# intel/QAT-ZSTD-Plugin

Measured on AMD Instinct MI355X. Metric: input MB/s via ZSTD_compress2 L1 128KiB blocks @1/2/4/8 GPU; ratio vs sw zstd, higher is better.
Workload: dtype u8

## Files before the change

### include/qzstd_hip.h

```cpp
#ifndef QZSTD_HIP_H
#define QZSTD_HIP_H

#include <stddef.h>
#include <stdint.h>

#if defined(__cplusplus)
extern "C" {
#endif

#define QZSTD_HIP_BLOCK_MAX (1u << 17)
#define QZSTD_HIP_NSEQ_ERROR 0xFFFFFFFFu
#define QZSTD_HIP_SRC_ALIGN 16u

typedef struct {
    uint32_t tableSize;
    uint32_t tileLog;
    uint32_t capLen;
    uint32_t minMatch;
    uint32_t farLog1;
    uint32_t farLog2;
    uint32_t lazy;
    uint32_t backExt;
    uint32_t nearTab;
    uint32_t window;
    uint32_t hashBytes;
    uint32_t extLog;
    uint32_t longSize;
    uint32_t repWin;
    uint32_t chainDepth;
    uint32_t subTileLog;
    uint32_t segLog;
} qzstd_hip_profile_t;

typedef struct {
    uint64_t srcOff;
    uint64_t seqOff;
    uint32_t srcLen;
    uint32_t seqCap;
    uint32_t parseFrom;
    uint32_t mark;
} qzstd_hip_block_t;

#define QZSTD_HIP_MARK_COMPACT 0x80000000u
#define QZSTD_HIP_PACK(off, lit, ml, tag) ((uint64_t)(off) | ((uint64_t)(lit) << 17) | ((uint64_t)(ml) << 35) | ((uint64_t)(tag) << 52))
#define QZSTD_HIP_PACKED_OFF(v) ((uint32_t)((v) & 0x1FFFFu))
#define QZSTD_HIP_PACKED_LIT(v) ((uint32_t)(((v) >> 17) & 0x3FFFFu))
#define QZSTD_HIP_PACKED_ML(v) ((uint32_t)(((v) >> 35) & 0x1FFFFu))
#define QZSTD_HIP_PACKED_TAG(v) ((uint32_t)((v) >> 52))

const char *qzstd_hip_last_error(void);

#define QZSTD_HIP_LEVEL_REPCODES 0x100

int qzstd_hip_profile_for_level(int level, size_t blockSize, qzstd_hip_profile_t *out);
size_t qzstd_hip_sequence_bound(size_t srcSize);
size_t qzstd_hip_lds_bytes(int level, uint32_t maxBlockLen);

#ifndef QZ_RING
#define QZ_RING 32768u
#endif
#define QZSTD_HIP_RING_MIRROR 128u
#ifndef QZ_CHAIN_TABLE
#define QZ_CHAIN_TABLE 5888u
#endif
#define QZSTD_HIP_LDS_BASE 16u
#define QZSTD_HIP_LDS_CTRL 64u
#define QZSTD_HIP_LDS_SVC 96u
#define QZSTD_HIP_LDS_MAX 163840u

int qzstd_hip_device_count(void);
int qzstd_hip_device_name(int device, char *buf, size_t bufLen);
void *qzstd_hip_malloc(int device, size_t bytes);
void qzstd_hip_free(int device, void *dptr);
void *qzstd_hip_host_alloc(size_t bytes);
void *qzstd_hip_host_device_ptr(void *hptr);
void qzstd_hip_host_free(void *hptr);
void *qzstd_hip_stream_create(int device);
void qzstd_hip_stream_destroy(int device, void *stream);
int qzstd_hip_stream_sync(int device, void *stream);
int qzstd_hip_stream_query(int device, void *stream);
int qzstd_hip_stream_wait(int device, void *stream, unsigned timeoutMs);
int qzstd_hip_memcpy_h2d(int device, void *stream, void *dst, const void *src, size_t bytes);
int qzstd_hip_copy_in(int device, void *stream, void *dst, const void *src_dev, size_t bytes);
int qzstd_hip_memcpy_d2h(int device, void *stream, void *dst, const void *src, size_t bytes);
int qzstd_hip_memset(int device, void *stream, void *dst, int value, size_t bytes);
int qzstd_hip_memcpy2d_d2h(int device, void *stream, void *dst, size_t dpitch, const void *src, size_t spitch,
                           size_t width, size_t height);

size_t qzstd_hip_workspace_bytes(int level, uint32_t nBlocks, uint32_t maxBlockLen);
int qzstd_hip_find_sequences(int device, void *stream, int level, const void *d_src,
                             const qzstd_hip_block_t *d_blocks, uint32_t nBlocks,
                             uint32_t maxBlockLen, void *d_seqs, uint32_t *d_nseq,
                             void *d_work, size_t workBytes);

int qzstd_hip_occupancy(int device, int level);

#define QZSTD_HIP_NSEQ_REJECTED 0xFFFFFFFEu
#define QZSTD_HIP_NSEQ_STAGING 0xFFFFFFFCu
int qzstd_hip_service_progressive(int device);
#define QZSTD_HIP_SVC_MAX_ITEMS 32u
#define QZSTD_HIP_SVC_MAX_SLOTS 1024u
typedef struct {
    const void *hSrc;
    void *dSrc;
    void *hSeqs;
    uint32_t *hCount;
    uint32_t srcLen, itemBytes, nItems, seqCapPerItem;
    uint32_t slot;
    uint32_t epoch;
    void *dWork;
} qzstd_hip_svc_req_t;
#ifndef QZSTD_HIP_CHAIN_ENTRY_LINKS
#define QZSTD_HIP_CHAIN_ENTRY_LINKS 4u
#endif
#define QZSTD_HIP_SVC_WORK_BYTES ((size_t)QZSTD_HIP_BLOCK_MAX * (8u * QZSTD_HIP_CHAIN_ENTRY_LINKS + 4u) + (size_t)QZSTD_HIP_SVC_MAX_ITEMS * QZ_CHAIN_TABLE * 4u)
int qzstd_hip_service_submit(int device, int level, const qzstd_hip_svc_req_t *req);
int qzstd_hip_service_stop(int device);
int qzstd_hip_service_poke(int device, int level);
void qzstd_hip_service_mark_broken(int device);
int qzstd_hip_service_info(int device, unsigned long out[8]);
int qzstd_hip_service_debug(int device, unsigned long out[8]);
void *qzstd_hip_host_alloc_coherent(size_t bytes);

int qzstd_hip_device_numa_node(int device);
void *qzstd_hip_host_alloc_on_node(size_t bytes, int node, int coherent);
int qzstd_hip_host_node_of(const void *hptr);

#if defined(__cplusplus)
}
#endif
#include "qzstd_hip_device.h"
#endif
```

### qat-zstd-plugin_amd/csrc/qzstd_hip_internal.h

```cpp
#ifndef QZSTD_HIP_INTERNAL_H
#define QZSTD_HIP_INTERNAL_H

#include <hip/hip_runtime.h>

#pragma GCC visibility push(hidden)

int fail(const char *what, hipError_t e);
int fail_msg(const char *what);

#define QZ_CHECK(call, what)                       \
    do {                                           \
        hipError_t e_ = (call);                    \
        if (e_ != hipSuccess) return fail(what, e_); \
    } while (0)

int phys(int device);
extern int g_devReplicas;

#define QZ_SET_DEVICE(device)                                            \
    do {                                                                 \
        const int pd_ = phys(device);                                    \
        if (pd_ < 0) return fail_msg("device index out of range");       \
        QZ_CHECK(hipSetDevice(pd_), "hipSetDevice");                     \
    } while (0)

int probe_lds_order(int device, int physDev);

struct SvcFreeze { SvcFreeze(); ~SvcFreeze(); };

#pragma GCC visibility pop

#endif
```

### qat-zstd-plugin_amd/csrc/qzstd_kernels.hip

```cpp
#include <hip/hip_runtime.h>

#include <stdint.h>
#include <stdio.h>
#include <stdlib.h>
#include <string.h>

#include <atomic>
#include <mutex>
#include <sched.h>
#include <time.h>

#include "qzstd_hip.h"
#include "qzstd_hip_internal.h"

#define QZ_PRIO(n) do { if (!CHAIN) __builtin_amdgcn_s_setprio(n); } while (0)

#ifndef QZ_PARSE_SPLIT
#define QZ_PARSE_SPLIT 3
#endif
#ifndef QZ_LINKS_PER_STEP
#define QZ_LINKS_PER_STEP 4
#endif
#ifndef QZ_WAVES_PER_EU
#define QZ_WAVES_PER_EU 5
#endif
#define QZ_OCCUPANCY __attribute__((amdgpu_waves_per_eu(QZ_WAVES_PER_EU)))

#ifdef QZ_DEBUG_DUMP
#define QZ_PLAP(acc) { const u64 tN = __builtin_amdgcn_s_memtime(); acc += tN - tQ; tQ = tN; }
#define QZ_LAP(acc) { const u64 tN = __builtin_amdgcn_s_memtime(); acc += tN - tP; tP = tN; }
#define QZ_CLAP(k) { const u64 tN = __builtin_amdgcn_s_memtime(); dC[k] += tN - tC; tC = tN; }
#else
#define QZ_PLAP(acc)
#define QZ_LAP(acc)
#define QZ_CLAP(k)
#endif

namespace {

constexpr int kMatchWaves = 8;
constexpr int kMatchThreads = kMatchWaves * 64;
constexpr int kThreads = kMatchThreads + 64;
constexpr uint32_t kTileLog = 9;
constexpr uint32_t kTile = 1u << kTileLog;
constexpr uint32_t kWin = kTile >> 6;
constexpr uint32_t kTagBits = 14;
constexpr uint32_t kTagMask = (1u << kTagBits) - 1u;
constexpr uint32_t kPrime1 = 2654435761u;
constexpr uint32_t kPrime2 = 0x85EBCA77u;
constexpr uint32_t kNone = 0xFFFFFFFFu;
constexpr uint32_t kRing = QZ_RING;
constexpr uint32_t kRingMask = kRing - 1u;
constexpr uint32_t kMirror = QZSTD_HIP_RING_MIRROR;
constexpr uint32_t kLook = 4608u;
constexpr uint32_t kNear = kRing - kLook - 3u * kTile - 1024u;
static_assert((kRing & kRingMask) == 0u && kRing >= 16384u, "the ring is a power of two of at least 16 KiB");
constexpr size_t kLdsPerCu = QZSTD_HIP_LDS_MAX;
constexpr uint32_t kEL = QZSTD_HIP_CHAIN_ENTRY_LINKS;
constexpr uint32_t kEQ = QZSTD_HIP_CHAIN_ENTRY_LINKS / 4u;
static_assert(kEL == 4u || kEL == 8u, "chain entries hold four or eight links");
constexpr uint32_t kLdsBase = QZSTD_HIP_LDS_BASE;
constexpr uint32_t kLagT = 2u;

struct LaunchArgs {
    const uint8_t *src;
    const qzstd_hip_block_t *blocks;
    uint4 *seqs;
    uint32_t *nseq;
    qzstd_hip_profile_t prof;
    uint4 *chain;
    uint32_t chainStride;
    uint32_t chainEntries;
    uint32_t pwWords;
    uint32_t orderedLds;
#ifdef QZ_DEBUG_DUMP
    uint32_t dbg;
#endif
};

typedef unsigned long long u64;

#ifdef QZ_DEBUG_DUMP
#define QZ_ABLATED(bit) (args.dbg & (bit))
#define QZ_DBG args.dbg
#else
#define QZ_ABLATED(bit) false
#define QZ_DBG 0u
#endif

#define QZ_BARRIER_LDS() asm volatile("s_waitcnt lgkmcnt(0)\n\ts_barrier" ::: "memory")

#define QZ_RLX_AGENT __ATOMIC_RELAXED, __HIP_MEMORY_SCOPE_AGENT
#define QZ_RLX_SYSTEM __ATOMIC_RELAXED, __HIP_MEMORY_SCOPE_SYSTEM

__device__ __forceinline__ uint32_t rdlane(uint32_t v, uint32_t l) { return (uint32_t)__builtin_amdgcn_readlane((int)v, (int)l); }
__device__ __forceinline__ uint32_t rdfirst(uint32_t v) { return (uint32_t)__builtin_amdgcn_readfirstlane((int)v); }
__device__ __forceinline__ u64 below(uint32_t c) { return c >= 64u ? ~0ull : ((1ull << c) - 1ull); }
__device__ __forceinline__ uint32_t umin(uint32_t a, uint32_t b) { return a < b ? a : b; }
__device__ __forceinline__ uint32_t umax(uint32_t a, uint32_t b) { return a > b ? a : b; }
__device__ __forceinline__ uint32_t umax3(uint32_t a, uint32_t b, uint32_t c) { return umax(umax(a, b), c); }

typedef const __attribute__((address_space(3))) uint32_t *LdsWords;
typedef const __attribute__((address_space(1))) uint32_t *HbmWords;
struct Src {
    LdsWords ring;
    HbmWords g;
    uint32_t nearLimit;
};

__device__ __forceinline__ uint32_t ring_dw(uint32_t a)
{
    return (a & kRingMask) >> 2;
}

__device__ __forceinline__ uint32_t ring_fwd(uint32_t r, uint32_t d) { return (r + d) & kRingMask; }
__device__ __forceinline__ uint32_t ring_back(uint32_t r, uint32_t d) { return (r - d) & kRingMask; }

template <int N>
__device__ __forceinline__ void load_dw_r(const Src &s, uint32_t a, uint32_t r, bool far, uint32_t (&D)[N])
{
    if (far) {
        const uint32_t d = a >> 2;
#pragma unroll
        for (int i = 0; i < N; i++) D[i] = s.g[d + i];
    } else {
        const uint32_t d = r >> 2;
#pragma unroll
        for (int i = 0; i < N; i++) D[i] = s.ring[d + i];
    }
}

template <int N>
__device__ __forceinline__ void load_dw(const Src &s, uint32_t a, bool far, uint32_t (&D)[N])
{
    if (far) {
        const uint32_t d = a >> 2;
#pragma unroll
        for (int i = 0; i < N; i++) D[i] = s.g[d + i];
    } else {
        const uint32_t d = ring_dw(a);
#pragma unroll
        for (int i = 0; i < N; i++) D[i] = s.ring[d + i];
    }
}

__device__ __forceinline__ uint32_t first_diff_bit(uint32_t x)
{
    uint32_t r;
    asm("v_ffbl_b32 %0, %1" : "=v"(r) : "v"(x));
    return r;
}

__device__ __forceinline__ uint32_t rd32u(const Src &s, uint32_t a, bool far)
{
    uint32_t D[2];
    load_dw<2>(s, a, far, D);
    return __builtin_amdgcn_alignbyte(D[1], D[0], a & 3u);
}

__device__ __forceinline__ uint32_t rd32_r(const Src &s, uint32_t a, uint32_t r, bool far)
{
    uint32_t D[2];
    load_dw_r<2>(s, a, r, far, D);
    return __builtin_amdgcn_alignbyte(D[1], D[0], a & 3u);
}

__device__ __forceinline__ uint32_t chunk_len(const Src &s, uint32_t p, uint32_t rp, uint32_t off, bool far)
{
    const uint32_t q = p - off, ps = p & 3u, qs = q & 3u;
    uint32_t P[9], Q[9];
    load_dw_r<9>(s, p, rp, false, P);
    load_dw_r<9>(s, q, ring_back(rp, off), far, Q);
    uint32_t B = 256u;
#pragma unroll
    for (int i = 0; i < 8; i++) {
        const uint32_t x = __builtin_amdgcn_alignbyte(P[i + 1], P[i], ps) ^ __builtin_amdgcn_alignbyte(Q[i + 1], Q[i], qs);
        B = umin(B, first_diff_bit(x) | (32u * (uint32_t)i));
    }
    return B >> 3;
}

__device__ __forceinline__ uint32_t head_len(const Src &s, const uint32_t (&oa)[4], uint32_t q, uint32_t rq, bool far)
{
    const uint32_t qs = q & 3u;
    uint32_t Q[5];
    load_dw_r<5>(s, q, rq, far, Q);
    uint32_t B = 128u;
#pragma unroll
    for (int i = 0; i < 4; i++) {
        const uint32_t x = oa[i] ^ __builtin_amdgcn_alignbyte(Q[i + 1], Q[i], qs);
        B = umin(B, first_diff_bit(x) | (32u * (uint32_t)i));
    }
    return B >> 3;
}

__device__ __forceinline__ uint32_t head_cmp(const uint32_t (&oa)[4], const uint32_t (&Q)[5], uint32_t qs)
{
    uint32_t B = 128u;
#pragma unroll
    for (int i = 0; i < 4; i++) {
        const uint32_t x = oa[i] ^ __builtin_amdgcn_alignbyte(Q[i + 1], Q[i], qs);
        B = umin(B, first_diff_bit(x) | (32u * (uint32_t)i));
    }
    return B >> 3;
}

__device__ __forceinline__ __attribute__((unused)) uint32_t tail_cmp(const uint32_t (&pa)[8], const uint32_t (&Q)[9], uint32_t qs)
{
    uint32_t B = 256u;
#pragma unroll
    for (int i = 0; i < 8; i++) {
        const uint32_t x = pa[i] ^ __builtin_amdgcn_alignbyte(Q[i + 1], Q[i], qs);
        B = umin(B, first_diff_bit(x) | (32u * (uint32_t)i));
    }
    return B >> 3;
}

__device__ __forceinline__ uint32_t tail_len(const Src &s, const uint32_t (&pa)[8], uint32_t q, uint32_t rq, bool far)
{
    const uint32_t qs = q & 3u;
    uint32_t Q[9];
    load_dw_r<9>(s, q, rq, far, Q);
    uint32_t B = 256u;
#pragma unroll
    for (int i = 0; i < 8; i++) {
        const uint32_t x = pa[i] ^ __builtin_amdgcn_alignbyte(Q[i + 1], Q[i], qs);
        B = umin(B, first_diff_bit(x) | (32u * (uint32_t)i));
    }
    return B >> 3;
}

__device__ __forceinline__ uint32_t seg_end(const qzstd_hip_profile_t &pf, uint32_t p, uint32_t n)
{
    return pf.segLog ? umin(n, ((p >> pf.segLog) + 1u) << pf.segLog) : n;
}

__device__ __forceinline__ uint32_t min_len(const qzstd_hip_profile_t &pf, uint32_t off)
{
    return pf.minMatch + ((off >> pf.farLog1) ? 1u : 0u) + ((off >> pf.farLog2) ? 1u : 0u);
}

template <bool AFAR = false>
__device__ __forceinline__ uint32_t extend_match_from(const Src &s, uint32_t p, uint32_t off, uint32_t L, uint32_t lim,
                                                      uint32_t lane, const bool far ,
                                                      const uint32_t lastDw = 0xFFFFFFFFu )
{
    for (;;) {
        const uint32_t a = p + L + 16u * lane;
        uint32_t ok = 0;
        if (a < lim) {
            const uint32_t b = a - off, as = a & 3u, bs = b & 3u;
            uint32_t A[5], B[5];
            if constexpr (AFAR) {
#pragma unroll
                for (int i = 0; i < 5; i++) { A[i] = s.g[umin((a >> 2) + (uint32_t)i, lastDw)]; B[i] = s.g[umin((b >> 2) + (uint32_t)i, lastDw)]; }
            } else {
                load_dw<5>(s, a, false, A);
                if (far) {
#pragma unroll
                    for (int i = 0; i < 5; i++) B[i] = s.g[umin((b >> 2) + (uint32_t)i, lastDw)];
                } else load_dw<5>(s, b, false, B);
            }
            ok = 16u;
#pragma unroll
            for (int i = 3; i >= 0; i--) {
                const uint32_t x = __builtin_amdgcn_alignbyte(A[i + 1], A[i], as) ^ __builtin_amdgcn_alignbyte(B[i + 1], B[i], bs);
                if (x) ok = 4u * (uint32_t)i + ((uint32_t)__builtin_ctz(x) >> 3);
            }
            ok = umin(ok, lim - a);
        }
        const u64 bad = __ballot(ok < 16u);
        if (bad) {
            const uint32_t f = (uint32_t)__builtin_ctzll(bad);
            return L + 16u * f + rdlane(ok, f);
        }
        L += 1024u;
    }
}

__device__ __forceinline__ uint32_t extend_match(const Src &s, uint32_t p, uint32_t off, uint32_t L, uint32_t lim, uint32_t lane)
{
    return extend_match_from(s, p, off, L, lim, lane, off > s.nearLimit);
}

struct ParseState {
    uint32_t cur;
    uint32_t anchor;
    uint32_t nseq;
};

constexpr uint32_t kSrecWords = 8;
constexpr uint32_t kPvStride = kTile + 8u;
constexpr uint32_t kNxCapped = 255u;

__device__ __forceinline__ uint32_t pack_pos(uint32_t nx, uint32_t ns, uint32_t payload)
{
    return nx | (ns << 8) | (payload << 15);
}

template <uint32_t L>
__device__ __forceinline__ uint32_t wrlane(uint32_t vec, uint32_t val)
{
    asm("v_writelane_b32 %0, %1, %2" : "+v"(vec) : "s"(val), "n"(L));
    return vec;
}

#define QZ_CHASE(c)                                                                   \
    asm volatile("v_readlane_b32 %[j], %[wd], %[cc]\n"                               \
                 "s_movk_i32 %[jn], 64\n"                                            \
                 "s_bfe_u32 %[j], %[j], 0x70008\n"                                   \
                 "s_cmp_gt_u32 %[j], 63\n"                                           \
                 "s_cbranch_scc1 2f\n"                                               \
                 "1:\n"                                                              \
                 "s_bitset1_b64 %[ch], %[j]\n"                                       \
                 "v_readlane_b32 %[jn], %[nx], %[j]\n"                               \
                 "s_cmp_lt_u32 %[jn], 64\n"                                          \
                 "s_cselect_b32 %[j], %[jn], %[j]\n"                                 \
                 "s_cbranch_scc1 1b\n"                                               \
                 "v_readlane_b32 %[pl], %[wd], %[j]\n"                               \
                 "s_lshr_b32 %[pl], %[pl], 15\n"                                     \
                 "2:\n"                                                              \
                 : [ch] "+s"(chosen), [j] "=&s"(j), [jn] "=&s"(jn), [pl] "=&s"(pl)    \
                 : [nx] "v"(nx), [wd] "v"(wordW), [cc] "s"(c)                         \
                 : "scc");

struct ParseRecs {
    uint32_t r0, r1, r2, r3, r4, r5;
};

template <uint32_t W>
__device__ __forceinline__ void parse_window(const qzstd_hip_profile_t &pf, const Src &src, const uint32_t wordW,
                                             uint32_t base, uint32_t n, uint32_t lane, ParseState &st, ParseRecs &r)
{
    constexpr uint32_t w = W;
    const uint32_t w0 = base + 64u * w;
    const uint32_t anchorIn = st.anchor, seqBase = st.nseq;
    u64 chosen = 0;
    uint32_t ext0 = 0, ext1 = 0;
    const uint32_t c0 = st.cur - w0;
    if (c0 < 64u) {
        const uint32_t nx = wordW & 0xFFu;
        uint32_t j, jn, pl;
        QZ_CHASE(c0)
        uint32_t cEnd = jn, eEnd = j < 64u ? j + pl : st.anchor - w0;
        if (__builtin_expect(jn == kNxCapped, 0)) {
            for (;;) {
                const uint32_t pj = w0 + j;
                const uint32_t lim = umin(seg_end(pf, pj, n), ((pj >> pf.extLog) + 2u) << pf.extLog);
                const uint32_t xl = extend_match(src, pj, pl, pf.capLen, lim, lane);
                if (!ext0) ext0 = (j << 24) | xl; else ext1 = (j << 24) | xl;
                cEnd = eEnd = j + xl;
                if (cEnd >= 64u) break;
                QZ_CHASE(cEnd)
                if (j >= 64u) { cEnd = 64u; break; }
                cEnd = jn; eEnd = j + pl;
                if (jn != kNxCapped) break;
            }
        }
        st.nseq += (uint32_t)__popcll(chosen);
        st.cur = w0 + cEnd;
        st.anchor = w0 + eEnd;
    }
    r.r0 = wrlane<W>(r.r0, (uint32_t)chosen);
    r.r1 = wrlane<W>(r.r1, (uint32_t)(chosen >> 32));
    r.r2 = wrlane<W>(r.r2, anchorIn);
    r.r3 = wrlane<W>(r.r3, seqBase);
    if (ext0) {
        r.r4 = wrlane<W>(r.r4, ext0);
        r.r5 = wrlane<W>(r.r5, ext1);
    }
}

template <uint32_t W, uint32_t W_END>
__device__ __forceinline__ void parse_windows(const qzstd_hip_profile_t &pf, const Src &src, const uint32_t (&word)[kWin],
                                              uint32_t base, uint32_t n, uint32_t lane, ParseState &st, ParseRecs &r)
{
    if constexpr (W < W_END) {
        parse_window<W>(pf, src, word[W], base, n, lane, st, r);
        parse_windows<W + 1u, W_END>(pf, src, word, base, n, lane, st, r);
    }
}

template <uint32_t W_BEGIN, uint32_t W_END>
__device__ __forceinline__ void parse_tile(const qzstd_hip_profile_t &pf, const Src &src, const uint32_t *pv,
                                           uint32_t *srecOut, uint32_t base, uint32_t n, uint32_t lane, ParseState &st)
{
    uint32_t word[kWin];
#pragma unroll
    for (uint32_t w = W_BEGIN; w < W_END; w++) word[w] = pv[64u * w + lane];
#pragma unroll
    for (uint32_t w = W_BEGIN; w < W_END; w++) asm volatile("" : "+v"(word[w]));
    ParseRecs r = { 0u, 0u, 0u, 0u, 0u, 0u };
    parse_windows<W_BEGIN, W_END>(pf, src, word, base, n, lane, st, r);
    if (lane >= W_BEGIN && lane < W_END) {
        *reinterpret_cast<uint4 *>(srecOut + lane * kSrecWords) = make_uint4(r.r0, r.r1, r.r2, r.r3);
        srecOut[lane * kSrecWords + 4u] = r.r4;
        srecOut[lane * kSrecWords + 5u] = r.r5;
    }
}

struct RepState {
    uint32_t cur, anchor, nseq;
    uint32_t rep1, rep2;
    uint32_t tileSeq;
    uint32_t seg;
};
constexpr uint32_t kRepCap = 32u, kRepMin = 3u;
constexpr uint32_t kLenCapped = 127u;
constexpr uint32_t kChosenBit = 0x80000000u;

__device__ __forceinline__ uint32_t ring_byte(const Src &s, uint32_t x, bool far)
{
    if (far) return reinterpret_cast<const __attribute__((address_space(1))) uint8_t *>(s.g)[x];
    return reinterpret_cast<const __attribute__((address_space(3))) uint8_t *>(s.ring)[x & kRingMask];
}

__device__ __forceinline__ u64 rep_bitmap(const Src &src, uint32_t cur, uint32_t rp, uint32_t n, uint32_t lane, uint32_t ringFrom = 0u)
{
    const uint32_t bpos = cur + lane;
    bool eq = false;
    if (rp != 0u && bpos < n) eq = ring_byte(src, bpos, false) == ring_byte(src, bpos - rp, rp > src.nearLimit || bpos - rp < ringFrom);
    return __ballot(eq);
}

__device__ __forceinline__ u64 rep_record(uint32_t q, uint32_t off, uint32_t L, uint32_t lit)
{
    return (u64)q | ((u64)off << 17) | ((u64)L << 34) | ((u64)lit << 47);
}

__device__ __forceinline__ uint32_t ring_off_s(uint32_t a)
{
    return a & kRingMask;
}

template <bool DEF>
__device__ __forceinline__ void parse_rep_span(const qzstd_hip_profile_t &pf, const Src &src, uint32_t *pvT,
                                               uint32_t base, uint32_t limit, uint32_t n, uint32_t nh, uint32_t lane,
                                               RepState &st, const uint32_t ringFrom = 0u, u64 *recG = nullptr)
{
    const uint32_t segEnd = seg_end(pf, base, n);
    const uint32_t startEnd = segEnd - pf.hashBytes + 1u;
    const uint32_t tileLim = umin(base + kTile, startEnd), stop = umin(limit, startEnd);
    if (st.cur < base) st.cur = base;
    if (st.cur >= stop) return;
    if (pf.segLog && (base >> pf.segLog) != st.seg) {
        st.rep1 = st.rep2 = 0u;
        st.seg = base >> pf.segLog;
    }
    uint32_t rc = rdfirst(ring_off_s(st.cur));
    const __attribute__((address_space(3))) uint8_t *rb = reinterpret_cast<const __attribute__((address_space(3))) uint8_t *>(src.ring);
    while (st.cur < stop) {
        const uint32_t rem = tileLim - st.cur;
        const uint32_t W = umin(pf.repWin, rem), V = umin(W + 2u, rem);
        const uint32_t curIn = st.cur;
        uint32_t wd = 0;
        if (lane < V) wd = pvT[st.cur + lane - base];
        u64 M1, M2;
        if (DEF ? (st.cur - st.rep1 >= ringFrom && st.cur - st.rep2 >= ringFrom)
                : (st.rep1 <= src.nearLimit && st.rep2 <= src.nearLimit)) {
            const uint32_t t1 = rc - st.rep1, t2 = rc - st.rep2;
            const uint32_t r1 = t1 & kRingMask, r2 = t2 & kRingMask;
            const uint32_t A = rb[rc + lane], B1 = rb[r1 + lane], B2 = rb[r2 + lane];
            const u64 in = below(segEnd - st.cur);
            M1 = st.rep1 ? __ballot(A == B1) & in : 0ull;
            M2 = st.rep2 ? __ballot(A == B2) & in : 0ull;
        } else {
            M1 = rep_bitmap(src, st.cur, st.rep1, segEnd, lane, ringFrom);
            M2 = rep_bitmap(src, st.cur, st.rep2, segEnd, lane, ringFrom);
        }
        const uint32_t x1 = __builtin_amdgcn_alignbit((uint32_t)(M1 >> 32), (uint32_t)M1, lane);
        const uint32_t x2 = __builtin_amdgcn_alignbit((uint32_t)(M2 >> 32), (uint32_t)M2, lane);
        const uint32_t rl1 = umin(first_diff_bit(~x1), kRepCap), rl2 = umin(first_diff_bit(~x2), kRepCap);
        const uint32_t rg1 = rl1 < kRepMin ? 0u : (rl1 >= kRepCap ? 1000u : 4u * rl1 + 36u);
        const uint32_t rg2 = rl2 < kRepMin ? 0u : (rl2 >= kRepCap ? 999u : 4u * rl2 + 35u);
        const uint32_t Gh = wd & 0x3FFu;
        const uint32_t G = lane < V ? umax3(Gh, rg1, rg2) : 0u;
        const uint32_t G1 = (uint32_t)__builtin_amdgcn_update_dpp(0, (int)G, 0x130, 0xF, 0xF, true);
        const uint32_t G2 = (uint32_t)__builtin_amdgcn_update_dpp(0, (int)G1, 0x130, 0xF, 0xF, true);
        const bool ok = lane < W && G != 0u && !(G1 > G + 4u) && !(G2 > G + 11u);
        const u64 m = __ballot(ok);
        if (!m) {
            st.cur += W;
            rc = ring_fwd(rc, W);
            continue;
        }
        const uint32_t ks = (uint32_t)__builtin_ctzll(m);
        const uint32_t gh = rdlane(Gh, ks), g1 = rdlane(rg1, ks), g2 = rdlane(rg2, ks);
        const uint32_t q = st.cur + ks;
        uint32_t off, L, from;
        if (g1 <= gh && g2 <= gh) {
            off = rdlane(wd, ks) >> 10;
            L = (gh - 32u + (31u - (uint32_t)__builtin_clz(off + 1u))) >> 2;
            from = pf.capLen;
        } else if (g2 > umax(gh, g1)) {
            off = st.rep2;
            L = rdlane(rl2, ks);
            from = kRepCap;
        } else {
            off = st.rep1;
            L = rdlane(rl1, ks);
            from = kRepCap;
        }
        if (L == from) L = extend_match_from(src, q, off, from, umin(segEnd, ((q >> pf.extLog) + 2u) << pf.extLog), lane,
                                             DEF ? q - off < ringFrom : off > src.nearLimit,
                                             DEF ? (((n + 15u) & ~15u) >> 2) - 1u : 0xFFFFFFFFu);
        if (DEF) {
            if (lane == 0u) recG[st.nseq] = rep_record(q, off, L, q - st.anchor);
        } else if (lane == 0u) {
            uint32_t *r = pvT + (q - base);
            r[0] = kChosenBit | off;
            r[1] = L | ((st.nseq - st.tileSeq) << 17);
            r[2] = st.anchor;
        }
        st.nseq++;
        if (off != st.rep1) {
            st.rep2 = st.rep1;
            st.rep1 = off;
        }
        st.cur = st.anchor = q + L;
        rc = rdfirst(ring_off_s(st.cur));
        (void)curIn;
    }
}

struct PlainParse {
    uint32_t cur, cnt, endA;
};
template <uint32_t W0, uint32_t W1>
__device__ __forceinline__ void parse_plain_windows(const qzstd_hip_profile_t &pf, const Src &src, u64 *recG, const uint32_t base, const uint32_t n,
                                                    const uint32_t lastDw, const uint32_t lane, const uint32_t (&wds)[kWin], PlainParse &st)
{
    u64 smA[kWin], chA[kWin];
    uint32_t lenA[kWin];
#pragma unroll
    for (uint32_t w = W0; w < W1; w++) {
        smA[w] = __ballot((wds[w] & kChosenBit) != 0u);
        lenA[w] = (wds[w] >> 17) & 127u;
    }
#pragma unroll
    for (uint32_t w = W0; w < W1; w++) {
        const uint32_t w0 = base + 64u * w;
        const u64 sm = smA[w];
        uint32_t c = rdfirst(st.cur - w0);
        u64 chosen = 0ull;
        uint32_t lenF = lenA[w];
        uint32_t e = 0u, j = 0u, L = 0u;
        auto chase = [&]() {
            u64 m;
            uint32_t t;
            asm volatile("s_cmp_lt_u32 %[c], 64\n"
                         "s_cbranch_scc0 3f\n"
                         "1:\n"
                         "s_lshr_b64 %[m], %[sm], %[c]\n"
                         "s_cbranch_scc0 2f\n"
                         "s_ff1_i32_b64 %[t], %[m]\n"
                         "s_add_u32 %[j], %[c], %[t]\n"
                         "s_bitset1_b64 %[ch], %[j]\n"
                         "v_readlane_b32 %[L], %[len], %[j]\n"
                         "s_add_u32 %[c], %[j], %[L]\n"
                         "s_cmp_lt_u32 %[c], 64\n"
                         "s_cbranch_scc1 1b\n"
                         "s_mov_b32 %[e], %[c]\n"
                         "s_branch 3f\n"
                         "2:\n"
                         "s_mov_b32 %[e], %[c]\n"
                         "s_movk_i32 %[c], 64\n"
                         "s_mov_b32 %[L], 0\n"
                         "3:\n"
                         : [m] "=&s"(m), [t] "=&s"(t), [j] "+s"(j), [ch] "+s"(chosen), [L] "+s"(L), [c] "+s"(c), [e] "+s"(e)
                         : [sm] "s"(sm), [len] "v"(lenF)
                         : "scc");
        };
        chase();
        while (__builtin_expect(L == kLenCapped, 0)) {
            const uint32_t pj = w0 + j, offj = rdlane(wds[w], j) & 0x1FFFFu;
            L = extend_match_from<true>(src, pj, offj, pf.capLen, umin(seg_end(pf, pj, n), ((pj >> pf.extLog) + 2u) << pf.extLog), lane, true, lastDw);
            if (lane == j) lenF = L;
            c = e = j + L;
            L = 0u;
            chase();
        }
        lenA[w] = lenF;
        st.cur = w0 + c;
        if (chosen) st.endA = w0 + e;
        chA[w] = chosen;
    }
#pragma unroll
    for (uint32_t w = W0; w < W1; w++) {
        const u64 chosen = chA[w];
        const uint32_t rank = __builtin_amdgcn_mbcnt_hi((uint32_t)(chosen >> 32), __builtin_amdgcn_mbcnt_lo((uint32_t)chosen, 0u));
        if ((chosen >> lane) & 1ull) recG[st.cnt + rank] = rep_record(base + 64u * w + lane, wds[w] & 0x1FFFFu, lenA[w], 0u);
        st.cnt += (uint32_t)__popcll(chosen);
    }
}

__device__ __forceinline__ void store_entry(uint4 *out, uint32_t idx, uint32_t off, uint32_t lit, uint32_t ml, uint32_t mark)
{
    if (mark & QZSTD_HIP_MARK_COMPACT)
        reinterpret_cast<u64 *>(out)[idx] = QZSTD_HIP_PACK(off, lit, ml, mark & 0xFFFu);
    else
        out[idx] = make_uint4(off, lit, ml, mark);
}

template <bool REP>
__device__ __forceinline__ void emit_window(const qzstd_hip_profile_t &pf, const Src &src, const uint32_t *srec,
                                            const uint32_t *pvW, uint32_t off, uint32_t len, uint32_t w0, uint32_t rpE,
                                            uint32_t lane, uint4 *out, uint32_t seqCap, uint32_t tileSeq, uint32_t mark)
{
    bool ch;
    uint32_t prevEnd, idx;
    if (REP) {
        const uint32_t r0 = pvW[lane];
        ch = (r0 & kChosenBit) != 0u;
        if (!__ballot(ch)) return;
        const uint32_t r1 = pvW[lane + 1u];
        prevEnd = pvW[lane + 2u];
        off = r0 & 0x1FFFFu;
        len = r1 & 0x1FFFFu;
        idx = tileSeq + (r1 >> 17);
    } else {
        const uint4 rec = *reinterpret_cast<const uint4 *>(srec);
        const u64 chosen = (u64)rec.x | ((u64)rec.y << 32);
        if (!chosen) return;
        const uint32_t anchorIn = rec.z, seqBase = rec.w;
        const uint32_t ext0 = rdfirst(srec[4]);
        if (ext0) {
            const uint32_t ext1 = srec[5];
            if ((ext0 >> 24) == lane) len = ext0 & 0xFFFFFFu;
            if (ext1 && (ext1 >> 24) == lane) len = ext1 & 0xFFFFFFu;
        }
        ch = (chosen >> lane) & 1ull;
        const u64 lower = chosen & below(lane);
        const uint32_t myEnd = w0 + lane + len;
        const int jprev = lower ? 63 - __builtin_clzll(lower) : 0;
        prevEnd = __shfl(myEnd, jprev);
        if (!lower) prevEnd = anchorIn;
        idx = seqBase + __builtin_amdgcn_mbcnt_hi((uint32_t)(chosen >> 32), __builtin_amdgcn_mbcnt_lo((uint32_t)chosen, 0u));
    }
    if (ch) {
        const uint32_t p = w0 + lane, q = p - off;
        const uint32_t lit = p - prevEnd;
        const uint32_t maxb = umin(umin(umin(pf.backExt, lit), q), pf.segLog ? (p & ((1u << pf.segLog) - 1u)) : p);
        uint32_t b = 0;
        if (maxb) {
            const bool far = off > src.nearLimit;
            const uint32_t rp4 = ring_back(rpE, 4u);
            const uint32_t pb = rd32_r(src, p - 4u, rp4, false);
            uint32_t qb;
            if (far) qb = q >= 4u ? rd32u(src, q - 4u, true) : rd32u(src, 0u, true) << (8u * (4u - q));
            else qb = rd32_r(src, q - 4u, ring_back(rp4, off), false);
            const uint32_t x = pb ^ qb;
            b = umin(x ? (uint32_t)__builtin_clz(x) >> 3 : 4u, maxb);
        }
        if (idx < seqCap) store_entry(out, idx, off, lit - b, len + b, mark);
    }
}

__device__ __forceinline__ uint32_t chain_insert_window(uint32_t *tbl, uint32_t st, uint32_t mine, uint32_t lane, bool ordered)
{
    const bool vk = st != kNone;
    const uint32_t slotK = st & 0xFFFFu;
    if (ordered) return vk ? atomicMax(&tbl[slotK], mine) : 0u;
    uint32_t prd = 0u, fin = mine;
    if (vk) {
        uint32_t *e = &tbl[slotK];
        prd = __hip_atomic_load(e, __ATOMIC_RELAXED, __HIP_MEMORY_SCOPE_WORKGROUP);
        atomicMax(e, mine);
        fin = __hip_atomic_load(e, __ATOMIC_RELAXED, __HIP_MEMORY_SCOPE_WORKGROUP);
    }
    u64 rem = __ballot(fin != mine);
    uint32_t predLane = lane;
    while (rem) {
        const uint32_t s0 = rdlane(slotK, (uint32_t)__builtin_ctzll(rem));
        const bool in = vk && slotK == s0;
        const u64 grp = __ballot(in);
        const u64 lower = grp & below(lane);
        if (in && lower) predLane = 63u - (uint32_t)__builtin_clzll(lower);
        rem &= ~grp;
    }
    const uint32_t fromLane = (uint32_t)__shfl((int)mine, (int)predLane);
    return vk ? (predLane != lane ? fromLane : prd) : 0u;
}

__device__ __forceinline__ void chain_insert_tile(const qzstd_hip_profile_t &pf, const Src &src, uint32_t *tbl, uint32_t *P1, uint32_t t0,
                                                  uint32_t n, uint32_t nh, uint32_t lane, bool ordered)
{
    const uint32_t segE = rdfirst(seg_end(pf, t0, n));
    uint32_t stv[kWin];
#pragma unroll
    for (uint32_t k = 0; k < kWin; k++) {
        const uint32_t p = t0 + 64u * k + lane;
        const uint32_t mixH = rd32u(src, p, false) * kPrime1;
        stv[k] = (p < nh && p + 4u <= segE) ? (__umulhi(mixH, pf.tableSize) | (((mixH >> 3) & kTagMask) << 16)) : kNone;
    }
    if (ordered) {
#pragma unroll
        for (uint32_t k = 0; k < kWin; k++) {
            const uint32_t mineK = ((t0 + 64u * k + lane + 1u) << kTagBits) | (stv[k] >> 16);
            uint32_t pred = 0u;
            if (stv[k] != kNone) pred = atomicMax(&tbl[stv[k] & 0xFFFFu], mineK);
            P1[64u * k + lane] = pred;
        }
    } else {
#pragma unroll 1
        for (uint32_t k = 0; k < kWin; k++) {
            const uint32_t st = stv[k];
            const bool vk = st != kNone;
            const uint32_t slotK = st & 0xFFFFu;
            const uint32_t mineK = ((t0 + 64u * k + lane + 1u) << kTagBits) | (st >> 16);
            uint32_t prd = 0u, fin = mineK;
            if (vk) {
                uint32_t *e = &tbl[slotK];
                prd = __hip_atomic_load(e, __ATOMIC_RELAXED, __HIP_MEMORY_SCOPE_WORKGROUP);
                atomicMax(e, mineK);
                fin = __hip_atomic_load(e, __ATOMIC_RELAXED, __HIP_MEMORY_SCOPE_WORKGROUP);
            }
            u64 rem = __ballot(fin != mineK);
            uint32_t predLane = lane;
            while (rem) {
                const uint32_t s0 = rdlane(slotK, (uint32_t)__builtin_ctzll(rem));
                const bool in = vk && slotK == s0;
                const u64 grp = __ballot(in);
                const u64 lower = grp & below(lane);
                if (in && lower) predLane = 63u - (uint32_t)__builtin_clzll(lower);
                rem &= ~grp;
            }
            const uint32_t fromLane = (uint32_t)__shfl((int)mineK, (int)predLane);
            P1[64u * k + lane] = vk ? (predLane != lane ? fromLane : prd) : 0u;
        }
    }
}

struct HistShare {
    uint32_t *flags;
    uint32_t item;
    uint32_t epoch;
    uint32_t spinLimit;
    uint32_t nItems;
    uint32_t *tabFlags;
    uint32_t *linkFlags;
    uint32_t *tabs;
};
constexpr uint32_t kSvcTabStride = QZ_CHAIN_TABLE;
static_assert((uint32_t)kMatchWaves * kPvStride <= QZ_CHAIN_TABLE, "the deferred parse's eight windows of parse words must fit in the head table (QZ_CHAIN_TABLE)");

template <bool HAS_LONG, bool REP, bool CHAIN, bool TURNS, bool NEAR, bool DEFER = false>
__device__ __forceinline__ uint32_t qz_item(const LaunchArgs &args, const qzstd_hip_block_t &blk, const uint8_t *gsrc, uint4 *out,
                                            uint4 *chainB, uint32_t *p1B, const HistShare hsh)
{
    extern __shared__ __attribute__((aligned(16))) uint8_t smem[];
    const uint32_t tid = threadIdx.x;
    const uint32_t lane = tid & 63u;
    const uint32_t wave = rdfirst(tid >> 6);
    const bool matcher = wave < (uint32_t)kMatchWaves;
    const uint32_t n = blk.srcLen;
    const qzstd_hip_profile_t pf = args.prof;
    const uint32_t nh = n >= pf.hashBytes ? n - pf.hashBytes + 1u : 0u;
    const uint32_t nTiles = (nh + kTile - 1u) >> kTileLog;
    const uint32_t itEnd = (DEFER && !CHAIN) ? nTiles : nTiles + kLagT;
    static_assert(kNear + kLagT * kTile + 4u <= kRing - kLook, "the ring no longer holds a near source when its tile is parsed / emitted");
    const uint32_t tabShift = (uint32_t)__builtin_clz(pf.tableSize) + 1u, longShift = pf.longSize ? (uint32_t)__builtin_clz(pf.longSize) + 1u : 31u;
    const uint32_t firstTile = blk.parseFrom >> kTileLog;
    if (blk.parseFrom != 0u && (pf.segLog == 0u || (blk.parseFrom & ((1u << pf.segLog) - 1u)) != 0u || blk.parseFrom >= n)) {
        return QZSTD_HIP_NSEQ_ERROR;
    }
    if (NEAR && n > kRing) return QZSTD_HIP_NSEQ_ERROR;
    if (DEFER && args.pwWords != 0u && ((n + kTile - 1u) & ~(kTile - 1u)) > args.pwWords) return QZSTD_HIP_NSEQ_ERROR;
    if (DEFER && CHAIN && args.chainEntries != 0u && ((n + kTile - 1u) & ~(kTile - 1u)) * kEQ > args.chainEntries) return QZSTD_HIP_NSEQ_ERROR;

    uint8_t *smemI = (uint8_t *)(__attribute__((address_space(3))) uint8_t *)kLdsBase;
    if ((uint32_t)(uintptr_t)(__attribute__((address_space(3))) uint8_t *)smem != 0u) {
        return QZSTD_HIP_NSEQ_ERROR;
    }
    uint32_t *ring32 = reinterpret_cast<uint32_t *>(smemI);
    uint4 *ring128 = reinterpret_cast<uint4 *>(smemI);
    uint32_t *tbl = reinterpret_cast<uint32_t *>(smemI + kRing + kMirror);
    uint32_t *tblL = tbl + pf.tableSize;
    uint32_t *nearTab = tblL + pf.longSize;
    uint32_t *srec = nearTab + kTile;
    uint32_t *pv = srec + kLagT * kWin * kSrecWords;
    uint32_t *turnCtr = pv + kLagT * kPvStride;
    uint32_t *P1odd = turnCtr + QZSTD_HIP_LDS_CTRL / 4u;
    const uint4 *g128 = reinterpret_cast<const uint4 *>(gsrc);
    Src src;
    src.ring = (LdsWords)ring32;
    src.g = (HbmWords)reinterpret_cast<const uint32_t *>(gsrc);
    src.nearLimit = NEAR ? 0xFFFFFFFFu : kNear;
    const uint32_t nPad = (n + 15u) & ~15u;

    const uint32_t itBegin = firstTile;
    const uint32_t histEnd = itBegin << kTileLog;
    const uint32_t hi = umin(nPad, histEnd + kLook + (itBegin ? 0u : kTile));
    const uint32_t lo = hi > kRing ? (hi - kRing + 15u) & ~15u : 0u;
    constexpr uint32_t kStep = (uint32_t)kThreads * 16u;
    const uint32_t hashEnd = CHAIN ? 0u : histEnd;
    uint32_t fo = (hashEnd ? 0u : lo) + tid * 16u;
    uint4 fa0 = make_uint4(0u, 0u, 0u, 0u), fb0 = fa0, fa1 = fa0, fb1 = fa0;
    if (fo < hi) { fa0 = g128[fo >> 4]; if (fo < hashEnd) fb0 = g128[(fo >> 4) + 1u]; }
    if (fo + kStep < hi) { fa1 = g128[(fo + kStep) >> 4]; if (fo + kStep < hashEnd) fb1 = g128[((fo + kStep) >> 4) + 1u]; }
    for (uint32_t i = tid; i < pf.tableSize + pf.longSize; i += kThreads) tbl[i] = 0u;
    if (!(CHAIN && itBegin != 0u)) {
        for (uint32_t i = tid; i < kTile; i += kThreads) nearTab[i] = 0xFFFFFFFFu;
        for (uint32_t i = tid; i < kLagT * kWin * kSrecWords + kLagT * kPvStride + QZSTD_HIP_LDS_CTRL / 4u; i += kThreads) srec[i] = 0u;
    }
    const bool sharedHist = CHAIN && hsh.flags != nullptr && hsh.nItems > 1u && pf.tableSize <= kSvcTabStride;
    if (itBegin != 0u || sharedHist) __syncthreads();
    if (sharedHist) {
        constexpr uint32_t kGroup = 4096u;
        uint32_t *hist = ring32;
        uint32_t *link = ring32 + kGroup;
        const uint32_t a0 = blk.parseFrom, b0 = n, k = hsh.item;
        auto wait_for = [&](uint32_t *fl) -> bool {
            if (wave == 0u) {
                uint32_t spins = 0u, ok = 1u;
                for (;;) {
                    const bool there = lane >= k || __hip_atomic_load(&fl[lane], QZ_RLX_AGENT) == hsh.epoch;
                    if (__all(there)) break;
                    if (++spins > hsh.spinLimit) { ok = 0u; break; }
                    __builtin_amdgcn_s_sleep(2);
                }
                __builtin_amdgcn_fence(__ATOMIC_ACQUIRE, "agent");
                if (lane == 0u) turnCtr[2] = ok;
            }
            __syncthreads();
            const bool ok = rdfirst(turnCtr[2]) != 0u;
            __syncthreads();
            return ok;
        };
        auto hash_group = [&](uint32_t g0) {
            if (tid < 256u) {
                const uint32_t c = g0 + tid * 16u;
                uint4 ha = make_uint4(0u, 0u, 0u, 0u), hb = ha;
                if (c < b0) { ha = g128[c >> 4]; hb = g128[(c >> 4) + 1u]; }
                const uint32_t W[5] = { ha.x, ha.y, ha.z, ha.w, hb.x };
                const uint32_t segEc = seg_end(pf, c, n);
                uint32_t st16[16];
#pragma unroll
                for (uint32_t j = 0; j < 16u; j++) {
                    const uint32_t v = (j & 3u) ? __builtin_amdgcn_alignbyte(W[(j >> 2) + 1u], W[j >> 2], j & 3u) : W[j >> 2];
                    const uint32_t mixH = v * kPrime1;
                    const bool okp = c + j < nh && c + j + 4u <= segEc;
                    st16[j] = okp ? (__umulhi(mixH, pf.tableSize) | (((mixH >> 3) & kTagMask) << 16)) : kNone;
                }
#pragma unroll
                for (uint32_t j = 0; j < 4u; j++)
                    reinterpret_cast<uint4 *>(hist)[tid * 4u + j] = make_uint4(st16[4u * j], st16[4u * j + 1u], st16[4u * j + 2u], st16[4u * j + 3u]);
            }
        };
        for (uint32_t g0 = a0; g0 < b0; g0 += kGroup) {
            hash_group(g0);
            QZ_BARRIER_LDS();
            if (wave == 2u || wave == 3u) {
                const uint32_t nW = (umin(kGroup, b0 - g0) + 63u) >> 6;
                const uint32_t par = wave & 1u;
                for (uint32_t w0 = 0; w0 < nW; w0 += 16u) {
                    uint32_t st[16], pred[16];
#pragma unroll
                    for (uint32_t j = 0; j < 16u; j++) st[j] = w0 + j < nW ? hist[64u * (w0 + j) + lane] : kNone;
#pragma unroll
                    for (uint32_t j = 0; j < 16u; j++) {
                        const uint32_t pos = g0 + 64u * (w0 + j) + lane;
                        const bool mine = st[j] != kNone && (st[j] & 1u) == par;
                        pred[j] = 0u;
                        if (mine) pred[j] = args.orderedLds != 0u ? atomicMax(&tbl[st[j] & 0xFFFFu], ((pos + 1u) << kTagBits) | (st[j] >> 16))
                                                                   : chain_insert_window(tbl, st[j], ((pos + 1u) << kTagBits) | (st[j] >> 16), lane, false);
                        else if (args.orderedLds == 0u) (void)chain_insert_window(tbl, kNone, 0u, lane, false);
                    }
#pragma unroll
                    for (uint32_t j = 0; j < 16u; j++)
                        if (w0 + j < nW && (st[j] == kNone || (st[j] & 1u) == par)) link[64u * (w0 + j) + lane] = pred[j];
                }
            }
            QZ_BARRIER_LDS();
            if (tid < 512u) {
#pragma unroll
                for (uint32_t j = 0; j < 2u; j++)
                    if (g0 + (j * 512u + tid) * 4u < b0) reinterpret_cast<uint4 *>(p1B + g0)[j * 512u + tid] = reinterpret_cast<const uint4 *>(link)[j * 512u + tid];
            }
            QZ_BARRIER_LDS();
        }
        {
            uint32_t *mine = hsh.tabs + (size_t)k * kSvcTabStride;
            for (uint32_t i = tid; i < pf.tableSize; i += kThreads) __hip_atomic_store(&mine[i], tbl[i], QZ_RLX_AGENT);
            asm volatile("s_waitcnt vmcnt(0)" ::: "memory");
            __syncthreads();
            if (tid == 0u) __hip_atomic_store(&hsh.tabFlags[k], hsh.epoch, QZ_RLX_AGENT);
        }
        if (!wait_for(hsh.tabFlags)) return QZSTD_HIP_NSEQ_ERROR;
        for (uint32_t i = tid; i < pf.tableSize; i += kThreads) {
            uint32_t m = 0u;
            for (uint32_t j = 0; j < k; j++) m = umax(m, hsh.tabs[(size_t)j * kSvcTabStride + i]);
            tbl[i] = m;
        }
        __syncthreads();
        for (uint32_t g0 = a0; g0 < b0; g0 += kGroup) {
            hash_group(g0);
            QZ_BARRIER_LDS();
            if (tid < 512u) {
#pragma unroll
                for (uint32_t j = 0; j < 8u; j++) {
                    const uint32_t i = j * 512u + tid, pos = g0 + i;
                    if (pos < b0) {
                        uint32_t l1 = p1B[pos];
                        const uint32_t st = hist[i];
                        if (l1 == 0u && st != kNone) l1 = tbl[st & 0xFFFFu];
                        __hip_atomic_store(&p1B[pos], l1, QZ_RLX_AGENT);
                    }
                }
            }
            QZ_BARRIER_LDS();
        }
        asm volatile("s_waitcnt vmcnt(0)" ::: "memory");
        __syncthreads();
        if (tid == 0u) __hip_atomic_store(&hsh.linkFlags[k], hsh.epoch, QZ_RLX_AGENT);
        if (!wait_for(hsh.linkFlags)) return QZSTD_HIP_NSEQ_ERROR;
        constexpr uint32_t kCh = 16u / kEL;
        for (uint32_t p0 = a0 + tid; p0 < b0; p0 += kCh * (uint32_t)kThreads) {
            uint32_t e[kEL][kCh];
#pragma unroll
            for (uint32_t i = 0; i < kCh; i++) { const uint32_t pp = p0 + i * (uint32_t)kThreads; e[0][i] = pp < b0 ? __hip_atomic_load(&p1B[pp], QZ_RLX_AGENT) : 0u; }
#pragma unroll
            for (uint32_t d = 1; d < kEL; d++)
#pragma unroll
                for (uint32_t i = 0; i < kCh; i++) e[d][i] = e[d - 1u][i] ? __hip_atomic_load(&p1B[(e[d - 1u][i] >> kTagBits) - 1u], QZ_RLX_AGENT) : 0u;
#pragma unroll
            for (uint32_t i = 0; i < kCh; i++) {
                const uint32_t pp = p0 + i * (uint32_t)kThreads;
                if (pp < b0) {
                    u64 *w = reinterpret_cast<u64 *>(chainB + (size_t)pp * kEQ);
#pragma unroll
                    for (uint32_t d = 0; d < kEL; d += 2u) __hip_atomic_store(w + d / 2u, (u64)e[d][i] | ((u64)e[d + 1u][i] << 32), QZ_RLX_AGENT);
                }
            }
        }
        asm volatile("s_waitcnt vmcnt(0)" ::: "memory");
        __syncthreads();
        if (tid == 0u) __hip_atomic_store(&hsh.flags[k], hsh.epoch, QZ_RLX_AGENT);
        if (!wait_for(hsh.flags)) return QZSTD_HIP_NSEQ_ERROR;
        for (uint32_t i = tid; i < kTile; i += kThreads) nearTab[i] = 0xFFFFFFFFu;
        for (uint32_t i = tid; i < kLagT * kWin * kSrecWords + kLagT * kPvStride + QZSTD_HIP_LDS_CTRL / 4u; i += kThreads) srec[i] = 0u;
    } else if (CHAIN && itBegin != 0u) {
        constexpr uint32_t kGroup = 4096u;
        static_assert(kGroup * 8u <= kRing, "two words per position of a group in the ring's LDS");
        uint32_t *hist = ring32;
        uint32_t *link = ring32 + kGroup;
        const uint32_t nGroups = (histEnd + kGroup - 1u) / kGroup;
        uint4 ha = make_uint4(0u, 0u, 0u, 0u), hb = ha;
        if (tid < 256u && tid * 16u < histEnd) { ha = g128[tid]; hb = g128[tid + 1u]; }
        for (uint32_t g = 0; g < nGroups && !QZ_ABLATED(2048u); g++) {
            const uint32_t g0 = g * kGroup;
            if (tid < 256u) {
                const uint32_t c = g0 + tid * 16u;
                const uint32_t W[5] = { ha.x, ha.y, ha.z, ha.w, hb.x };
                const uint32_t segEc = seg_end(pf, c, n);
                uint32_t st16[16];
#pragma unroll
                for (uint32_t k = 0; k < 16u; k++) {
                    const uint32_t v = (k & 3u) ? __builtin_amdgcn_alignbyte(W[(k >> 2) + 1u], W[k >> 2], k & 3u) : W[k >> 2];
                    const uint32_t mixH = v * kPrime1;
                    const bool ok = c + k < histEnd && c + k + 4u <= segEc;
                    st16[k] = ok ? (__umulhi(mixH, pf.tableSize) | (((mixH >> 3) & kTagMask) << 16)) : kNone;
                }
#pragma unroll
                for (uint32_t k = 0; k < 4u; k++)
                    reinterpret_cast<uint4 *>(hist)[tid * 4u + k] = make_uint4(st16[4u * k], st16[4u * k + 1u], st16[4u * k + 2u], st16[4u * k + 3u]);
                const uint32_t cn = c + kGroup;
                ha = hb = make_uint4(0u, 0u, 0u, 0u);
                if (cn < histEnd) { ha = g128[cn >> 4]; hb = g128[(cn >> 4) + 1u]; }
            }
            QZ_BARRIER_LDS();
            if (wave == 2u || wave == 3u) {
                const uint32_t nW = umin(kGroup, histEnd - g0) >> 6;
                const uint32_t par = wave & 1u;
                if (args.orderedLds != 0u) {
                    for (uint32_t w0 = 0; w0 < nW; w0 += 16u) {
                        uint32_t st[16], pred[16];
#pragma unroll
                        for (uint32_t k = 0; k < 16u; k++) st[k] = hist[64u * (w0 + k) + lane];
#pragma unroll
                        for (uint32_t k = 0; k < 16u; k++) {
                            const uint32_t pos = g0 + 64u * (w0 + k) + lane;
                            pred[k] = 0u;
                            if (st[k] != kNone && (st[k] & 1u) == par) pred[k] = atomicMax(&tbl[st[k] & 0xFFFFu], ((pos + 1u) << kTagBits) | (st[k] >> 16));
                        }
#pragma unroll
                        for (uint32_t k = 0; k < 16u; k++)
                            if (st[k] == kNone || (st[k] & 1u) == par) link[64u * (w0 + k) + lane] = pred[k];
                    }
                } else {
                    for (uint32_t w = 0; w < nW; w++) {
                        const uint32_t st = hist[64u * w + lane];
                        const uint32_t pos = g0 + 64u * w + lane;
                        const bool mine = st != kNone && (st & 1u) == par;
                        const uint32_t pred = chain_insert_window(tbl, mine ? st : kNone, ((pos + 1u) << kTagBits) | (st >> 16), lane, false);
                        if (mine || st == kNone) link[64u * w + lane] = pred;
                    }
                }
            }
            QZ_BARRIER_LDS();
            if (tid < 512u && !QZ_ABLATED(1024u)) {
#pragma unroll
                for (uint32_t k = 0; k < 2u; k++)
                    if (g0 + (k * 512u + tid) * 4u < histEnd) reinterpret_cast<uint4 *>(p1B + g0)[k * 512u + tid] = reinterpret_cast<const uint4 *>(link)[k * 512u + tid];
            }
            QZ_BARRIER_LDS();
        }
        constexpr uint32_t kChase = 32u / kEL;
        const uint32_t chaseFrom = hsh.flags ? histEnd - histEnd / hsh.item : 0u;
        for (uint32_t p0 = chaseFrom + tid; p0 < histEnd && !QZ_ABLATED(512u); p0 += kChase * (uint32_t)kThreads) {
            uint32_t e[kEL][kChase];
#pragma unroll
            for (uint32_t i = 0; i < kChase; i++) { const uint32_t pp = p0 + i * (uint32_t)kThreads; e[0][i] = pp < histEnd ? p1B[pp] : 0u; }
#pragma unroll
            for (uint32_t d = 1; d < kEL; d++)
#pragma unroll
                for (uint32_t i = 0; i < kChase; i++) e[d][i] = e[d - 1u][i] ? p1B[(e[d - 1u][i] >> kTagBits) - 1u] : 0u;
#pragma unroll
            for (uint32_t i = 0; i < kChase; i++) {
                const uint32_t pp = p0 + i * (uint32_t)kThreads;
                if (pp < histEnd) {
                    if (hsh.flags) {
                        u64 *w = reinterpret_cast<u64 *>(chainB + (size_t)pp * kEQ);
#pragma unroll
                        for (uint32_t d = 0; d < kEL; d += 2u) __hip_atomic_store(w + d / 2u, (u64)e[d][i] | ((u64)e[d + 1u][i] << 32), QZ_RLX_AGENT);
                    } else {
#pragma unroll
                        for (uint32_t j = 0; j < kEL / 4u; j++) chainB[(size_t)pp * kEQ + j] = make_uint4(e[4u * j][i], e[4u * j + 1u][i], e[4u * j + 2u][i], e[4u * j + 3u][i]);
                    }
                }
            }
        }
        if (hsh.flags) {
            asm volatile("s_waitcnt vmcnt(0)" ::: "memory");
            __syncthreads();
            if (wave == 0u) {
                if (lane == 0u) __hip_atomic_store(&hsh.flags[hsh.item], hsh.epoch, QZ_RLX_AGENT);
                uint32_t spins = 0u, ok = 1u;
                for (;;) {
                    const bool there = lane == 0u || lane >= hsh.item || __hip_atomic_load(&hsh.flags[lane], QZ_RLX_AGENT) == hsh.epoch;
                    if (__all(there)) break;
                    if (++spins > hsh.spinLimit) { ok = 0u; break; }
                    __builtin_amdgcn_s_sleep(2);
                }
                __builtin_amdgcn_fence(__ATOMIC_ACQUIRE, "agent");
                if (lane == 0u) turnCtr[2] = ok;
            }
            __syncthreads();
            if (rdfirst(turnCtr[2]) == 0u) return QZSTD_HIP_NSEQ_ERROR;
        }
        __syncthreads();
        for (uint32_t i = tid; i < kTile; i += kThreads) nearTab[i] = 0xFFFFFFFFu;
        for (uint32_t i = tid; i < kLagT * kWin * kSrecWords + kLagT * kPvStride + QZSTD_HIP_LDS_CTRL / 4u; i += kThreads) srec[i] = 0u;
    }
    {
        const uint32_t hiMaskH = pf.hashBytes >= 8 ? 0xFFFFFFFFu : ((1u << (8u * (pf.hashBytes - 4u))) - 1u);
        for (; fo < hi; fo += kStep) {
            uint4 fa2 = make_uint4(0u, 0u, 0u, 0u), fb2 = fa2;
            const uint32_t o2 = fo + 2u * kStep;
            if (o2 < hi) { fa2 = g128[o2 >> 4]; if (o2 < hashEnd) fb2 = g128[(o2 >> 4) + 1u]; }
            if (fo >= lo) {
                const uint32_t r = ring_dw(fo) << 2;
                ring128[r >> 4] = fa0;
                if (r < kMirror) ring128[(kRing + r) >> 4] = fa0;
            }
            if (fo < hashEnd) {
                const uint32_t W[6] = { fa0.x, fa0.y, fa0.z, fa0.w, fb0.x, fb0.y };
                const uint32_t segEc = seg_end(pf, fo, n);
#pragma unroll
                for (uint32_t k = 0; k < 16u; k++) {
                    const uint32_t p = fo + k;
                    if (p + pf.hashBytes <= segEc) {
                        const uint32_t v = __builtin_amdgcn_alignbyte(W[(k >> 2) + 1u], W[k >> 2], k & 3u);
                        const uint32_t w = __builtin_amdgcn_alignbyte(W[(k >> 2) + 2u], W[(k >> 2) + 1u], k & 3u);
                        const uint32_t mixH = (v * kPrime1) ^ __umul24(pf.hashBytes > 4 ? w & hiMaskH : 0u, kPrime2 & 0xFFFFFFu);
                        atomicMax(&tbl[mixH >> tabShift], ((p + 1u) << kTagBits) | ((mixH >> 3) & kTagMask));
                        if (HAS_LONG && p + 8u <= segEc) {
                            const uint32_t m8 = (v * kPrime1) ^ (w * kPrime2);
                            atomicMax(&tblL[m8 >> longShift], ((p + 1u) << kTagBits) | ((m8 >> 3) & kTagMask));
                        }
                    }
                }
            }
            fa0 = fa1; fb0 = fb1; fa1 = fa2; fb1 = fb2;
        }
        if (itBegin != 0u && TURNS && !CHAIN && tid == 0u) *turnCtr = itBegin * (uint32_t)kMatchWaves;
        if (itBegin == 0u)
            for (uint32_t o = hi + tid * 16u; o < kTile + kLook; o += kThreads * 16u) {
                ring128[o >> 4] = make_uint4(0u, 0u, 0u, 0u);
                if (o < kMirror) ring128[(kRing + o) >> 4] = make_uint4(0u, 0u, 0u, 0u);
            }
    }
    __syncthreads();

    if (DEFER && !matcher) __builtin_amdgcn_endpgm();
    if (!matcher) {
        if (!QZ_ABLATED(32u)) __builtin_amdgcn_s_setprio(3);
        constexpr uint32_t kSplit = QZ_PARSE_SPLIT;
#ifdef QZ_DEBUG_DUMP
        u64 pI1 = 0, pW1 = 0, pI2 = 0, pW2 = 0, tQ = __builtin_amdgcn_s_memtime();
#endif
        uint32_t nseqEnd, anchorEnd;
        if (REP) {
            RepState st = { blk.parseFrom, blk.parseFrom, 0u, 0u, 0u, 0u, pf.segLog ? blk.parseFrom >> pf.segLog : 0u };
            for (uint32_t it = itBegin; it < itEnd; it++) {
                const bool work = it >= 1u && it - 1u < nTiles && it - 1u >= firstTile && !QZ_ABLATED(1u);
                const uint32_t k = it - 1u, base = k << kTileLog;
                uint32_t *pvT = pv + (k % kLagT) * kPvStride, *srecT = srec + (k % kLagT) * kWin * kSrecWords;
                if (work) {
                    st.tileSeq = st.nseq;
                    if (lane == 0u) srecT[0] = st.nseq;
                    if (!CHAIN) parse_rep_span<false>(pf, src, pvT, base, base + 64u * kSplit, n, nh, lane, st);
                }
                if (CHAIN && it == itBegin && it < nTiles) chain_insert_tile(pf, src, tbl, (it & 1u) ? P1odd : nearTab, it << kTileLog, n, nh, lane, args.orderedLds != 0u);
                QZ_PLAP(pI1)
                __syncthreads();
                QZ_PLAP(pW1)
                if (work) parse_rep_span<false>(pf, src, pvT, base, base + kTile, n, nh, lane, st);
                if (CHAIN && it + 1u < nTiles) chain_insert_tile(pf, src, tbl, ((it + 1u) & 1u) ? P1odd : nearTab, (it + 1u) << kTileLog, n, nh, lane, args.orderedLds != 0u);
                QZ_PLAP(pI2)
                __syncthreads();
                QZ_PLAP(pW2)
            }
            nseqEnd = st.nseq;
            anchorEnd = st.anchor;
        } else {
            ParseState st = { blk.parseFrom, blk.parseFrom, 0u };
            for (uint32_t it = itBegin; it < itEnd; it++) {
                const bool work = it >= 1u && it - 1u < nTiles && it - 1u >= firstTile && !QZ_ABLATED(1u);
                const uint32_t k = it - 1u;
                if (work && !CHAIN)
                    parse_tile<0, kSplit>(pf, src, pv + (k % kLagT) * kPvStride, srec + (k % kLagT) * kWin * kSrecWords,
                                          k << kTileLog, n, lane, st);
                if (CHAIN && it == itBegin && it < nTiles) chain_insert_tile(pf, src, tbl, (it & 1u) ? P1odd : nearTab, it << kTileLog, n, nh, lane, args.orderedLds != 0u);
                QZ_PLAP(pI1)
                __syncthreads();
                QZ_PLAP(pW1)
                if (work) {
                    if (CHAIN)
                        parse_tile<0, kWin>(pf, src, pv + (k % kLagT) * kPvStride, srec + (k % kLagT) * kWin * kSrecWords, k << kTileLog, n, lane, st);
                    else
                        parse_tile<kSplit, kWin>(pf, src, pv + (k % kLagT) * kPvStride, srec + (k % kLagT) * kWin * kSrecWords,
                                                 k << kTileLog, n, lane, st);
                }
                if (CHAIN && it + 1u < nTiles) chain_insert_tile(pf, src, tbl, ((it + 1u) & 1u) ? P1odd : nearTab, (it + 1u) << kTileLog, n, nh, lane, args.orderedLds != 0u);
                QZ_PLAP(pI2)
                __syncthreads();
                QZ_PLAP(pW2)
            }
            nseqEnd = st.nseq;
            anchorEnd = st.anchor;
        }
#ifdef QZ_DEBUG_DUMP
        if (lane == 0 && !(blk.mark & QZSTD_HIP_MARK_COMPACT)) out[blk.seqCap - 2u] = make_uint4((uint32_t)pI1, (uint32_t)pW1, (uint32_t)pI2, (uint32_t)pW2);
        if (lane == 0 && !(blk.mark & QZSTD_HIP_MARK_COMPACT)) out[blk.seqCap - 12u - wave] = make_uint4(__builtin_amdgcn_s_getreg((4 << 0) | (0 << 6) | (31 << 11)), 0u, 0u, 0u);
#endif
        uint32_t count = nseqEnd + 1u;
        if (lane == 0 && nseqEnd < blk.seqCap) store_entry(out, nseqEnd, 0u, n - anchorEnd, 0u, blk.mark);
        if (count + 1u >= blk.seqCap) count = QZSTD_HIP_NSEQ_ERROR;
        return count;
    }

    if (matcher) {
    uint4 *const ownB = (CHAIN && hsh.flags) ? chainB + (size_t)QZSTD_HIP_BLOCK_MAX * kEQ : chainB;
    const uint32_t ownFrom = blk.parseFrom;
    auto entryOf = [&](uint32_t q, uint32_t (&D)[kEL]) {
        const uint4 *b = (q >= ownFrom ? ownB : chainB) + (size_t)q * kEQ;
#pragma unroll
        for (uint32_t j = 0; j < kEL / 4u; j++) { const uint4 v = b[j]; D[4u * j] = v.x; D[4u * j + 1u] = v.y; D[4u * j + 2u] = v.z; D[4u * j + 3u] = v.w; }
    };
    const uint32_t hiMask = pf.hashBytes >= 8 ? 0xFFFFFFFFu : ((1u << (8u * (pf.hashBytes - 4u))) - 1u);
    const uint32_t nearShift = 32u - kTileLog;
    const uint32_t stampShift = kTileLog + kTagBits;
    const uint32_t nTilesMax = QZSTD_HIP_BLOCK_MAX >> kTileLog;

    uint32_t offH[kLagT], lenH[kLagT];
#pragma unroll
    for (uint32_t i = 0; i < kLagT; i++) offH[i] = lenH[i] = 0u;
    uint32_t rp = ring_dw((itBegin << kTileLog) + tid) << 2 | (tid & 3u);
#ifdef QZ_DEBUG_DUMP
    u64 dI1 = 0, dW1 = 0, dI2 = 0, dW2 = 0, tP = __builtin_amdgcn_s_memtime();
    u64 dC[6] = { 0, 0, 0, 0, 0, 0 }, tC = 0;
#endif

    auto write_flags = [&](uint32_t tileIdx, uint32_t cl, uint32_t off) {
            const bool take = cl != 0u && cl >= min_len(pf, off);
            bool defer1, defer2, defer3 = false;
            if (pf.lazy >= 4u) {
                const uint32_t G = take ? 4u * cl + 32u - (31u - (uint32_t)__builtin_clz(off + 1u)) : 0u;
                const uint32_t G1 = (uint32_t)__builtin_amdgcn_update_dpp(0, (int)G, 0x130, 0xF, 0xF, true);
                const uint32_t G2 = (uint32_t)__builtin_amdgcn_update_dpp(0, (int)G1, 0x130, 0xF, 0xF, true);
                defer1 = lane < 63u && G1 > G + 4u;
                defer2 = lane < 62u && G2 > G + 7u;
            } else {
                const uint32_t tl = take ? cl : 0u;
                const uint32_t tl1 = (uint32_t)__builtin_amdgcn_update_dpp(0, (int)tl, 0x130, 0xF, 0xF, true);
                const uint32_t tl2 = (uint32_t)__builtin_amdgcn_update_dpp(0, (int)tl1, 0x130, 0xF, 0xF, true);
                const uint32_t tl3 = (uint32_t)__builtin_amdgcn_update_dpp(0, (int)tl2, 0x130, 0xF, 0xF, true);
                defer1 = pf.lazy >= 1u && lane < 63u && tl1 > cl;
                defer2 = pf.lazy >= 2u && lane < 62u && tl2 > cl;
                defer3 = pf.lazy >= 3u && lane < 61u && tl3 > cl + 2u;
            }
            const bool start = take && !defer1 && !defer2 && !defer3;
            if constexpr (DEFER && !REP) {
                p1B[(tileIdx << kTileLog) + tid] = off | ((cl == pf.capLen ? kLenCapped : cl) << 17) | (start ? kChosenBit : 0u);
                return;
            }
            const u64 startMask = __ballot(start);
            const uint32_t smLo = (uint32_t)startMask, smHi = (uint32_t)(startMask >> 32);
            const uint32_t keepLo = lane < 32u ? smLo & (0xFFFFFFFFu << (lane & 31u)) : 0u;
            const uint32_t keepHi = lane < 32u ? smHi : smHi & (0xFFFFFFFFu << (lane & 31u));
            const uint32_t ns = umin(umin(first_diff_bit(keepLo), first_diff_bit(keepHi) | 32u), 64u);
            const bool capped = cl == pf.capLen;
            const uint32_t endj = lane + cl;
            const uint32_t nsEnd = (uint32_t)__shfl((int)ns, (int)(endj & 63u));
            uint32_t nx = endj >= 64u ? endj : nsEnd;
            nx = capped ? kNxCapped : nx;
            const uint32_t gRep = take ? 4u * cl + 32u - (31u - (uint32_t)__builtin_clz(off + 1u)) : 0u;
            if (DEFER) p1B[(tileIdx << kTileLog) + tid] = gRep | (off << 10);
            else pv[(tileIdx % kLagT) * kPvStride + tid] = REP ? (gRep | (off << 10)) : pack_pos(nx, ns, capped ? off : cl);
    };
    for (uint32_t it = itBegin; it < itEnd; it++) {
        const uint32_t t0 = it << kTileLog;
        const uint32_t p = t0 + tid;
        const uint32_t stamp = (nTilesMax - 1u - (it & (nTilesMax - 1u))) << stampShift;
        uint32_t mix = 0, old = 0;
        const uint32_t segE = rdfirst(seg_end(pf, t0, n));
        const bool valid = it < nTiles && p < nh && p + pf.hashBytes <= segE;
        const bool history = it < firstTile;

        QZ_PRIO(2);
        if (CHAIN && DEFER && wave == 0u && it == itBegin && it < nTiles)
            chain_insert_tile(pf, src, tbl, (it & 1u) ? P1odd : nearTab, it << kTileLog, n, nh, lane, args.orderedLds != 0u);
        uint32_t own[5];
        load_dw_r<5>(src, p, rp, false, own);
        uint4 fresh;
        asm volatile("" : "=v"(fresh.x), "=v"(fresh.y), "=v"(fresh.z), "=v"(fresh.w));
        const uint32_t fpos = t0 + kLook + (tid - 64u) * 16u;
        const bool refill = wave == 1u && it >= 1u && lane < kTile / 16u && fpos < nPad;
        if (refill) fresh = g128[fpos >> 4];
        if (!DEFER && it >= kLagT + firstTile && !QZ_ABLATED(8u))
            emit_window<REP>(pf, src, srec + ((it % kLagT) * kWin + wave) * kSrecWords, pv + (it % kLagT) * kPvStride + 64u * wave,
                             offH[kLagT - 1u], lenH[kLagT - 1u], t0 - kLagT * kTile + 64u * wave, ring_back(rp, kLagT * kTile), lane, out, blk.seqCap,
                             REP ? srec[(it % kLagT) * kWin * kSrecWords] : 0u, blk.mark);
        QZ_PRIO(1);
        uint32_t slot = 0, nslot = 0, slotL = 0, oldL = 0, tagL = 0;
        const bool validL = HAS_LONG && valid && p + 8u <= segE;
        uint32_t oa[4];
#pragma unroll
        for (int i = 0; i < 4; i++) oa[i] = __builtin_amdgcn_alignbyte(own[i + 1], own[i], p & 3u);
        if (valid) {
            const uint32_t v = oa[0];
            uint32_t hi = 0;
            if (pf.hashBytes > 4) hi = oa[1] & hiMask;
            mix = (v * kPrime1) ^ __umul24(hi, kPrime2 & 0xFFFFFFu);
            slot = CHAIN ? __umulhi(mix, pf.tableSize) : mix >> tabShift;
            nslot = mix >> nearShift;
            if (!TURNS) old = tbl[slot];
            if (pf.nearTab && !history) atomicMin(&nearTab[nslot], stamp | (tid << kTagBits) | ((mix >> 3) & kTagMask));
            if (validL) {
                const uint32_t m8 = (v * kPrime1) ^ (oa[1] * kPrime2);
                slotL = m8 >> longShift;
                tagL = (m8 >> 3) & kTagMask;
                if (!TURNS) oldL = tblL[slotL];
            }
        }
        uint32_t pre[kEL];
#pragma unroll
        for (uint32_t j = 0; j < kEL; j++) pre[j] = 0u;
        if (CHAIN && it != itBegin) {
            old = valid ? ((it & 1u) ? P1odd : nearTab)[tid] : 0u;
            if (old != 0u && (old >> kTagBits) - 1u < t0) entryOf((old >> kTagBits) - 1u, pre);
        }
        if (CHAIN && it > itBegin && it - 1u < nTiles && it - 1u >= firstTile && !QZ_ABLATED(4u)) write_flags(it - 1u, lenH[0], offH[0]);
        QZ_LAP(dI1)
        __syncthreads();
        QZ_LAP(dW1)

        QZ_PRIO(2);
        if (CHAIN && DEFER && wave == 0u && it + 1u < nTiles)
            chain_insert_tile(pf, src, tbl, ((it + 1u) & 1u) ? P1odd : nearTab, (it + 1u) << kTileLog, n, nh, lane, args.orderedLds != 0u);
        if (refill) {
            const uint32_t o = ring_dw(fpos) << 2;
            ring128[o >> 4] = fresh;
            if (o < kMirror) ring128[(kRing + o) >> 4] = fresh;
        }
        uint32_t cl = 0, off = 0;
        if (CHAIN) {
            const uint32_t *P1T = (it & 1u) ? P1odd : nearTab;
            const uint32_t tag = (mix >> 3) & kTagMask;
#ifdef QZ_DEBUG_DUMP
            tC = __builtin_amdgcn_s_memtime();
#endif
            uint32_t E[kEL];
#pragma unroll
            for (uint32_t j = 0; j < kEL; j++) E[j] = 0u;
            if (valid) {
                E[0] = P1T[tid];
                if (E[0] != 0u && (E[0] >> kTagBits) - 1u < t0) {
                    if (it == itBegin) entryOf((E[0] >> kTagBits) - 1u, pre);
#pragma unroll
                    for (uint32_t i = 1; i < kEL; i++) E[i] = pre[i - 1u];
                } else {
#pragma unroll
                    for (uint32_t i = 1; i < kEL; i++) {
                        const uint32_t q = (E[i - 1u] >> kTagBits) - 1u;
                        if (E[i - 1u] == 0u || q < t0) break;
                        E[i] = P1T[q - t0];
                    }
                }
#pragma unroll
                for (uint32_t j = 0; j < kEL / 4u; j++) ownB[(size_t)p * kEQ + j] = make_uint4(E[4u * j], E[4u * j + 1u], E[4u * j + 2u], E[4u * j + 3u]);
            }
            const uint32_t cap = valid ? umin(umin(pf.capLen, 48u), segE - p) : 0u;
            uint32_t walked = 0;
            if (history) E[0] = 0u;
            int bg = 0;
            QZ_CLAP(0)
            while (__ballot(E[0] != 0u)) {
                uint32_t N[kEL];
#pragma unroll
                for (uint32_t j = 0; j < kEL; j++) N[j] = 0u;
                if (E[0] != 0u) {
                    uint32_t last = E[0], cnt = 1u;
#pragma unroll
                    for (uint32_t j = 1; j < kEL; j++) { if (E[j] != 0u) { last = E[j]; cnt = j + 1u; } }
                    const uint32_t ql = (last >> kTagBits) - 1u;
                    if (walked + cnt < pf.chainDepth) {
                        if (ql < t0) {
                            entryOf(ql, N);
                        } else {
                            N[0] = P1T[ql - t0];
#pragma unroll
                            for (uint32_t i = 1; i < kEL; i++) {
                                const uint32_t q = (N[i - 1u] >> kTagBits) - 1u;
                                if (N[i - 1u] == 0u || q < t0) break;
                                N[i] = P1T[q - t0];
                            }
                        }
                    }
                    constexpr int kG = QZ_LINKS_PER_STEP;
                    QZ_CLAP(1)
#pragma unroll
                    for (int kk = 0; kk < (int)kEL; kk += kG) {
                        uint32_t q[kG], rq[kG];
                        bool far[kG], m[kG];
#pragma unroll
                        for (int g = 0; g < kG; g++) {
                            const uint32_t l = E[kk + g];
                            q[g] = (l >> kTagBits) - 1u;
                            far[g] = p - q[g] > src.nearLimit;
                            m[g] = l != 0u && walked + (uint32_t)(kk + g) < pf.chainDepth && (l & kTagMask) == tag && (pf.window == 0u || p - q[g] <= pf.window) &&
                                   !QZ_ABLATED(2u) && !(QZ_ABLATED(64u) && far[g]);
                            rq[g] = ring_back(rp, p - q[g]);
                        }
                        bool any = false;
#pragma unroll
                        for (int g = 0; g < kG; g++) any = any || m[g];
                        if (any && cl != 0u) {
                            uint32_t v[kG];
#pragma unroll
                            for (int g = 0; g < kG; g++) {
                                m[g] = m[g] && cl < cap;
                                v[g] = 0u;
                                if (m[g]) v[g] = rd32_r(src, q[g] + cl - 3u, ring_fwd(rq[g], cl - 3u), far[g]);
                            }
                            const uint32_t pw = rd32_r(src, p + cl - 3u, ring_fwd(rp, cl - 3u), false);
#pragma unroll
                            for (int g = 0; g < kG; g++) m[g] = m[g] && v[g] == pw;
                        }
                        QZ_CLAP(2)
                        uint32_t Q[kG][5];
#pragma unroll
                        for (int g = 0; g < kG; g++) {
#pragma unroll
                            for (int i = 0; i < 5; i++) Q[g][i] = 0u;
                            if (m[g]) load_dw_r<5>(src, q[g], rq[g], far[g], Q[g]);
                        }
#pragma unroll
                        for (int g = 0; g < kG; g++) {
                            if (m[g] && cl < cap) {
                                uint32_t l = head_cmp(oa, Q[g], q[g] & 3u);
                                if (l == 16u && cap > 16u) l += chunk_len(src, p + 16u, ring_fwd(rp, 16u), p - q[g], far[g]);
                                l = umin(l, cap);
                                const int gn = (int)(4u * l) - (int)(31u - (uint32_t)__builtin_clz(p - q[g] + 1u));
                                if (l >= 4u && (cl == 0u || gn > bg)) { cl = l; off = p - q[g]; bg = gn; }
                            }
                        }
                    }
                    walked += cnt;
                }
                QZ_CLAP(3)
#ifdef QZ_DEBUG_DUMP
                asm volatile("s_waitcnt vmcnt(0)" ::: "memory");
                dC[5] += 1;
#endif
                const bool full = cl != 0u && cl >= cap;
#pragma unroll
                for (uint32_t j = 0; j < kEL; j++) E[j] = full ? 0u : N[j];
                QZ_CLAP(4)
            }
        } else {
        if (TURNS) {
            const uint32_t turn = it * (uint32_t)kMatchWaves + wave;
            uint32_t spins = 0;
            while (__hip_atomic_load(turnCtr, __ATOMIC_ACQUIRE, __HIP_MEMORY_SCOPE_WORKGROUP) != turn && ++spins < (1u << 22))
                __builtin_amdgcn_s_sleep(1);
            if (valid) {
                old = tbl[slot];
                if (validL) oldL = tblL[slotL];
                atomicMax(&tbl[slot], ((p + 1u) << kTagBits) | ((mix >> 3) & kTagMask));
                if (validL) atomicMax(&tblL[slotL], ((p + 1u) << kTagBits) | tagL);
            }
            if (lane == 0u) __hip_atomic_store(turnCtr, turn + 1u, __ATOMIC_RELEASE, __HIP_MEMORY_SCOPE_WORKGROUP);
        }
        if (valid) {
            const uint32_t tag = (mix >> 3) & kTagMask;
            const uint32_t en = pf.nearTab ? nearTab[nslot] : 0xFFFFFFFFu;
            if (!TURNS) {
                atomicMax(&tbl[slot], ((p + 1u) << kTagBits) | tag);
                if (validL) atomicMax(&tblL[slotL], ((p + 1u) << kTagBits) | tagL);
            }
            if (!history) {
            const uint32_t cap = umin(pf.capLen, segE - p);
            uint32_t q1 = kNone, q2 = kNone;
            if (old != 0u && (old & kTagMask) == tag) {
                const uint32_t q = (old >> kTagBits) - 1u;
                if (pf.window == 0u || p - q <= pf.window) q1 = q;
            }
            if (QZ_ABLATED(2u)) q1 = kNone;
            if (QZ_ABLATED(64u) && q1 != kNone && p - q1 > src.nearLimit) q1 = kNone;
            uint32_t l1 = 0, l2 = 0, l3 = 0;
            const bool far1 = q1 != kNone && p - q1 > src.nearLimit;
            if (q1 != kNone) l1 = head_len(src, oa, q1, ring_back(rp, p - q1), far1);
            uint32_t q3 = kNone;
            if (HAS_LONG && validL && oldL != 0u && (oldL & kTagMask) == tagL && !QZ_ABLATED(2u)) q3 = (oldL >> kTagBits) - 1u;
            const bool far3 = q3 != kNone && p - q3 > src.nearLimit;
            if (q3 != kNone) l3 = head_len(src, oa, q3, ring_back(rp, p - q3), far3);
            if (pf.nearTab && (en >> stampShift) == (stamp >> stampShift) && (en & kTagMask) == tag) {
                const uint32_t q = t0 + ((en >> kTagBits) & (kTile - 1u));
                if (q < p && !QZ_ABLATED(2u | 256u)) q2 = q;
            }
            if (q2 != kNone) l2 = head_len(src, oa, q2, ring_back(rp, p - q2), false);
            bool need1 = l1 == 16u && cap > 16u, need2 = l2 == 16u && cap > 16u, need3 = HAS_LONG && l3 == 16u && cap > 16u;
            if (QZ_ABLATED(128u)) need1 = need2 = need3 = false;
            QZ_PRIO(1);
            if (need1 || need2 || need3) {
                const uint32_t rp16 = ring_fwd(rp, 16u);
                uint32_t P[9], pa[8];
                load_dw_r<9>(src, p + 16u, rp16, false, P);
#pragma unroll
                for (int i = 0; i < 8; i++) pa[i] = __builtin_amdgcn_alignbyte(P[i + 1], P[i], p & 3u);
                if (need1) { const uint32_t l = tail_len(src, pa, q1 + 16u, ring_back(rp16, p - q1), far1); l1 = 16u + l; need1 = l == 32u && 48u < cap; }
                if (HAS_LONG && need3) { const uint32_t l = tail_len(src, pa, q3 + 16u, ring_back(rp16, p - q3), far3); l3 = 16u + l; need3 = l == 32u && 48u < cap; }
                if (need2) { const uint32_t l = tail_len(src, pa, q2 + 16u, ring_back(rp16, p - q2), false); l2 = 16u + l; need2 = l == 32u && 48u < cap; }
            }
            while (need1 || need2 || need3) {
                const int which = need1 ? 1 : (need3 ? 3 : 2);
                const uint32_t q = which == 1 ? q1 : (which == 3 ? q3 : q2);
                const uint32_t L = which == 1 ? l1 : (which == 3 ? l3 : l2);
                const uint32_t l = chunk_len(src, p + L, ring_fwd(rp, L), p - q, which == 1 ? far1 : (which == 3 ? far3 : false));
                const bool more = l == 32u && L + 32u < cap;
                if (which == 1) { l1 = L + l; need1 = more; }
                else if (which == 3) { l3 = L + l; need3 = more; }
                else { l2 = L + l; need2 = more; }
            }
            QZ_PRIO(0);
            l1 = umin(l1, cap); l2 = umin(l2, cap); l3 = umin(l3, cap);
            if (l1 >= 4u) { cl = l1; off = p - q1; }
            if (l3 >= 4u && l3 > cl) { cl = l3; off = p - q3; }
            if (l2 >= 4u && l2 >= cl) { cl = l2; off = p - q2; }
            }
        }
        }
        if (!CHAIN && it < nTiles && !history && !QZ_ABLATED(4u)) write_flags(it, cl, off);
#pragma unroll
        for (uint32_t i = kLagT - 1u; i > 0u; i--) { offH[i] = offH[i - 1u]; lenH[i] = lenH[i - 1u]; }
        offH[0] = off;
        lenH[0] = cl;
        rp = ring_fwd(rp, kTile);
        QZ_LAP(dI2)
        if (DEFER && !CHAIN) QZ_BARRIER_LDS(); else __syncthreads();
        QZ_LAP(dW2)
    }
#ifdef QZ_DEBUG_DUMP
    if (!(blk.mark & QZSTD_HIP_MARK_COMPACT)) {
    if (lane == 0) out[blk.seqCap - 3u - wave] = make_uint4((uint32_t)dI1, (uint32_t)dW1, (uint32_t)dI2, (uint32_t)dW2);
    if (lane == 0) out[blk.seqCap - 24u - 2u * wave] = make_uint4((uint32_t)(dC[0] >> 4), (uint32_t)(dC[1] >> 4), (uint32_t)(dC[2] >> 4), (uint32_t)(dC[3] >> 4));
    if (lane == 0) out[blk.seqCap - 25u - 2u * wave] = make_uint4((uint32_t)(dC[4] >> 4), (uint32_t)dC[5], 0u, 0u);
    if (lane == 0) out[blk.seqCap - 12u - wave] = make_uint4(__builtin_amdgcn_s_getreg((4 << 0) | (0 << 6) | (31 << 11)), 0u, 0u, 0u);
    }
#endif
    if constexpr (!DEFER) return 0u;
    }

    if constexpr (DEFER && !REP) {
        constexpr uint32_t kSegLog = 12u, kSeg = 1u << kSegLog, kMaxSegs = QZSTD_HIP_BLOCK_MAX >> kSegLog;
        static_assert(kMaxSegs <= 64u, "one lane per segment in the prefix step");
        constexpr uint32_t kNoAnchor = 0xFFFFFFFFu;
        uint32_t *segCnt = srec, *segEndA = srec + kMaxSegs;
        const uint32_t firstSeg = blk.parseFrom >> kSegLog, nSegs = (nh + kSeg - 1u) >> kSegLog;
#ifdef QZ_DEBUG_DUMP
        const u64 tD0 = __builtin_amdgcn_s_memtime();
#endif
        if (wave == 0u && lane == 0u) segCnt[2u * kMaxSegs] = firstSeg;
        __syncthreads();
#ifdef QZ_DEBUG_DUMP
        const u64 tD1 = __builtin_amdgcn_s_memtime();
#endif
        {
            const uint32_t S0 = rdfirst(segCnt[2u * kMaxSegs]);
            const uint32_t lastDw = (nPad >> 2) - 1u;
            auto load_tile = [&](uint32_t tb, uint32_t (&dst)[kWin]) {
#pragma unroll
                for (uint32_t j = 0; j < kWin; j++) dst[j] = p1B[tb + 64u * j + lane];
            };
            uint32_t nxt[kWin];
            uint32_t sgN = S0 + wave;
            if (sgN < nSegs) load_tile(sgN << kSegLog, nxt);
            while (sgN < nSegs) {
                const uint32_t sg = sgN;
                sgN = sg + (uint32_t)kMatchWaves;
                const uint32_t segStart = sg << kSegLog;
                u64 *recG = reinterpret_cast<u64 *>(p1B + segStart);
                const uint32_t tEnd = umin(segStart + kSeg, nTiles << kTileLog);
                PlainParse st = { segStart, 0u, kNoAnchor };
                for (uint32_t base = segStart; base < tEnd; base += kTile) {
                    uint32_t wds[kWin];
#pragma unroll
                    for (uint32_t j = 0; j < kWin; j++) wds[j] = nxt[j];
                    const uint32_t nb = base + kTile < tEnd ? base + kTile : sgN << kSegLog;
                    if (base + kTile < tEnd || sgN < nSegs) load_tile(nb, nxt);
                    parse_plain_windows<0, kWin>(pf, src, recG, base, n, lastDw, lane, wds, st);
                }
                if (lane == 0u) { segCnt[sg] = st.cnt; segEndA[sg] = st.endA; }
            }
        }
#ifdef QZ_DEBUG_DUMP
        const u64 tD2 = __builtin_amdgcn_s_memtime();
#endif
        __syncthreads();
#ifdef QZ_DEBUG_DUMP
        const u64 tD3 = __builtin_amdgcn_s_memtime();
#endif
        const bool mine = lane >= firstSeg && lane < nSegs;
        const uint32_t cv = mine ? segCnt[lane] : 0u, ev = mine ? segEndA[lane] : kNoAnchor;
        uint32_t incl = cv, last = ev;
#pragma unroll
        for (uint32_t d = 1; d < kMaxSegs; d <<= 1) {
            const uint32_t ci = (uint32_t)__shfl_up((int)incl, d), li = (uint32_t)__shfl_up((int)last, d);
            if (lane >= d) { incl += ci; if (last == kNoAnchor) last = li; }
        }
        const uint32_t total = rdlane(incl, kMaxSegs - 1u), lastAll = rdlane(last, kMaxSegs - 1u);
        const uint32_t anchorEndAll = lastAll == kNoAnchor ? blk.parseFrom : lastAll;
        {
            for (uint32_t sg = firstSeg + wave; sg < nSegs; sg += (uint32_t)kMatchWaves) {
                const u64 *recG = reinterpret_cast<const u64 *>(p1B + (sg << kSegLog));
                const uint32_t cnt = rdlane(cv, sg), first = rdlane(incl, sg) - cnt;
                uint32_t anchorIn = blk.parseFrom;
                if (sg > 0u) { const uint32_t a = rdlane(last, sg - 1u); if (a != kNoAnchor) anchorIn = a; }
                constexpr uint32_t kU = 4u;
                for (uint32_t k0 = 0; k0 < cnt; k0 += 64u * kU) {
                    u64 r[kU], rp1[kU];
#pragma unroll
                    for (uint32_t u = 0; u < kU; u++) {
                        const uint32_t k = k0 + 64u * u + lane;
                        r[u] = k < cnt ? recG[k] : 0ull;
                        rp1[u] = (k < cnt && k) ? recG[k - 1u] : 0ull;
                    }
                    uint32_t P0[kU], P1[kU], Q0[kU], Q1[kU], lit[kU], maxb[kU];
#pragma unroll
                    for (uint32_t u = 0; u < kU; u++) {
                        const uint32_t k = k0 + 64u * u + lane;
                        const uint32_t pm = (uint32_t)r[u] & 0x1FFFFu, off = (uint32_t)(r[u] >> 17) & 0x1FFFFu;
                        lit[u] = k ? pm - (((uint32_t)rp1[u] & 0x1FFFFu) + ((uint32_t)(rp1[u] >> 34) & 0x1FFFu))
                                   : pm - anchorIn;
                        const uint32_t q = pm - off;
                        maxb[u] = k < cnt ? umin(umin(umin(pf.backExt, lit[u]), q), pm & (kSeg - 1u)) : 0u;
                        P0[u] = P1[u] = Q0[u] = Q1[u] = 0u;
                        if (maxb[u]) {
                            const uint32_t pa = pm >= 4u ? pm - 4u : 0u, qa = q >= 4u ? q - 4u : 0u;
                            P0[u] = src.g[pa >> 2]; P1[u] = src.g[(pa >> 2) + 1u];
                            Q0[u] = src.g[qa >> 2]; Q1[u] = src.g[(qa >> 2) + 1u];
                        }
                    }
#pragma unroll
                    for (uint32_t u = 0; u < kU; u++) {
                        const uint32_t k = k0 + 64u * u + lane;
                        if (k < cnt) {
                            const uint32_t pm = (uint32_t)r[u] & 0x1FFFFu, off = (uint32_t)(r[u] >> 17) & 0x1FFFFu, len = (uint32_t)(r[u] >> 34) & 0x1FFFu;
                            const uint32_t q = pm - off;
                            uint32_t b = 0;
                            if (maxb[u]) {
                                const uint32_t pa = pm >= 4u ? pm - 4u : 0u, qa = q >= 4u ? q - 4u : 0u;
                                uint32_t pb = __builtin_amdgcn_alignbyte(P1[u], P0[u], pa & 3u), qb = __builtin_amdgcn_alignbyte(Q1[u], Q0[u], qa & 3u);
                                if (pm < 4u) pb <<= 8u * (4u - pm);
                                if (q < 4u) qb <<= 8u * (4u - q);
                                const uint32_t x = pb ^ qb;
                                b = umin(x ? (uint32_t)__builtin_clz(x) >> 3 : 4u, maxb[u]);
                            }
                            const uint32_t idx = first + k;
                            if (idx < blk.seqCap) store_entry(out, idx, off, lit[u] - b, len + b, blk.mark);
                        }
                    }
                }
            }
#ifdef QZ_DEBUG_DUMP
            if (lane == 0 && !(blk.mark & QZSTD_HIP_MARK_COMPACT))
                out[blk.seqCap - 44u - wave] = make_uint4((uint32_t)(tD1 - tD0), (uint32_t)(tD2 - tD1), (uint32_t)(tD3 - tD2), (uint32_t)(__builtin_amdgcn_s_memtime() - tD3));
#endif
        }
        if (wave != 0u) return 0u;
        uint32_t count = total + 1u;
        if (lane == 0 && total < blk.seqCap) store_entry(out, total, 0u, n - anchorEndAll, 0u, blk.mark);
        if (count + 1u >= blk.seqCap) count = QZSTD_HIP_NSEQ_ERROR;
        return count;
    }

    if constexpr (DEFER && REP) {
        constexpr uint32_t kSegLog = 12u, kSeg = 1u << kSegLog, kSegsPerQ = kRing >> kSegLog;
        static_assert(kSegsPerQ == (uint32_t)kMatchWaves, "one wave per segment of a quarter");
        constexpr uint32_t kNoAnchor = 0xFFFFFFFFu;
        __syncthreads();
        uint32_t *pvW = tbl + wave * kPvStride;
        uint32_t *ctl = srec;
        const uint32_t firstSeg = blk.parseFrom >> kSegLog, nSegs = (nh + kSeg - 1u) >> kSegLog;
        uint32_t total = 0u, anchorCarry = blk.parseFrom;
        for (uint32_t Q = firstSeg / kSegsPerQ; Q * kSegsPerQ < nSegs; Q++) {
            const uint32_t qs = Q * kRing;
            for (uint32_t o = qs + tid * 16u; o < umin(qs + kRing, nPad); o += (uint32_t)kMatchThreads * 16u) {
                const uint4 v = g128[o >> 4];
                ring128[(o & kRingMask) >> 4] = v;
                if ((o & kRingMask) < kMirror) ring128[(kRing + (o & kRingMask)) >> 4] = v;
            }
            __syncthreads();
            const uint32_t sg = Q * kSegsPerQ + wave;
            const uint32_t segStart = sg << kSegLog;
            u64 *recG = reinterpret_cast<u64 *>(p1B + segStart);
            uint32_t cnt = 0u, endA = kNoAnchor;
            if (sg >= firstSeg && sg < nSegs) {
                const uint32_t tEnd = umin(segStart + kSeg, nTiles << kTileLog);
                uint32_t nxt[kWin];
#pragma unroll
                for (uint32_t j = 0; j < kWin; j++) nxt[j] = p1B[segStart + 64u * j + lane];
                {
                    RepState st = { segStart, segStart, 0u, 0u, 0u, 0u, sg };
                    for (uint32_t base = segStart; base < tEnd; base += kTile) {
#pragma unroll
                        for (uint32_t j = 0; j < kWin; j++) pvW[64u * j + lane] = nxt[j];
                        if (base + kTile < tEnd) {
#pragma unroll
                            for (uint32_t j = 0; j < kWin; j++) nxt[j] = p1B[base + kTile + 64u * j + lane];
                        }
                        parse_rep_span<true>(pf, src, pvW, base, base + kTile, n, nh, lane, st, qs, recG);
                    }
                    cnt = st.nseq;
                    if (cnt) endA = st.anchor;
                }
            }
            if (lane == 0u) { ctl[wave] = cnt; ctl[kSegsPerQ + wave] = endA; }
            __syncthreads();
            {
                const uint32_t cv = lane < 2u * kSegsPerQ ? ctl[lane] : 0u;
                uint32_t before = 0u, all = 0u, anchorIn = anchorCarry, anchorOut = anchorCarry;
#pragma unroll
                for (uint32_t j = 0; j < kSegsPerQ; j++) {
                    const uint32_t c = rdlane(cv, j), a = rdlane(cv, kSegsPerQ + j);
                    if (j < wave) { before += c; if (a != kNoAnchor) anchorIn = a; }
                    all += c;
                    if (a != kNoAnchor) anchorOut = a;
                }
                const uint32_t cnt = rdlane(cv, wave);
                for (uint32_t k0 = 0; k0 < cnt; k0 += 64u) {
                    const uint32_t k = k0 + lane;
                    if (k < cnt) {
                        const u64 r = recG[k];
                        const uint32_t pm = (uint32_t)r & 0x1FFFFu, off = (uint32_t)(r >> 17) & 0x1FFFFu, len = (uint32_t)(r >> 34) & 0x1FFFu;
                        uint32_t lit = pm - anchorIn;
                        if (k) lit = (uint32_t)(r >> 47) & 0x1FFFu;
                        const uint32_t q = pm - off;
                        const uint32_t maxb = umin(umin(umin(pf.backExt, lit), q), pm & (kSeg - 1u));
                        uint32_t b = 0;
                        if (maxb) {
                            const uint32_t pb = rd32u(src, pm - 4u, false);
                            uint32_t qb;
                            if (q < qs + 4u) qb = q >= 4u ? rd32u(src, q - 4u, true) : rd32u(src, 0u, true) << (8u * (4u - q));
                            else qb = rd32u(src, q - 4u, false);
                            const uint32_t x = pb ^ qb;
                            b = umin(x ? (uint32_t)__builtin_clz(x) >> 3 : 4u, maxb);
                        }
                        const uint32_t idx = total + before + k;
                        if (idx < blk.seqCap) store_entry(out, idx, off, lit - b, len + b, blk.mark);
                    }
                }
                total += all;
                anchorCarry = anchorOut;
            }
            __syncthreads();
        }
        if (wave != 0u) return 0u;
        uint32_t count = total + 1u;
        if (lane == 0 && total < blk.seqCap) store_entry(out, total, 0u, n - anchorCarry, 0u, blk.mark);
        if (count + 1u >= blk.seqCap) count = QZSTD_HIP_NSEQ_ERROR;
        return count;
    }
    return 0u;
}

template <bool HAS_LONG, bool REP, bool CHAIN, bool TURNS, bool NEAR>
__global__ __launch_bounds__(kThreads) QZ_OCCUPANCY void qzstd_find_sequences_kernel(LaunchArgs args)
{
    const qzstd_hip_block_t blk = args.blocks[blockIdx.x];
    const uint32_t count = qz_item<HAS_LONG, REP, CHAIN, TURNS, NEAR, true>(args, blk, args.src + blk.srcOff, args.seqs + blk.seqOff,
                                                              CHAIN ? args.chain + (size_t)blockIdx.x * args.chainStride : nullptr,
                                                              reinterpret_cast<uint32_t *>(args.chain + (size_t)blockIdx.x * args.chainStride + args.chainEntries),
                                                              HistShare{ nullptr, 0u, 0u, 0u, 0u, nullptr, nullptr, nullptr });
    asm volatile("s_waitcnt vmcnt(0)" ::: "memory");
    __syncthreads();
    if (threadIdx.x == 0u)
        __hip_atomic_store(args.nseq + blockIdx.x, count, __ATOMIC_RELEASE, __HIP_MEMORY_SCOPE_SYSTEM);
}

constexpr uint32_t kSvcQueue = 4096u;
constexpr uint32_t kSvcRing = 256u;
constexpr uint32_t kSvcMaxItems = 32u;
constexpr uint32_t kSvcSlots = 1024u;
constexpr uint32_t kSvcRejected = 0xFFFFFFFEu;

struct SvcDev {
    u64 items[kSvcQueue][8];
    uint32_t head;
    uint32_t done;
    uint32_t quit;
    uint32_t spinFails;
    uint32_t started;
    uint32_t taken;
    uint32_t pad[2];
    uint32_t sliceFlag[kSvcSlots][kSvcMaxItems];
    uint32_t histFlag[kSvcSlots][kSvcMaxItems];
    uint32_t tabFlag[kSvcSlots][kSvcMaxItems];
    uint32_t linkFlag[kSvcSlots][kSvcMaxItems];
};

struct SvcHost {
    u64 ring[kSvcRing][8];
    uint32_t state;
    uint32_t quitReq;
    u64 consumed;
    u64 itemsDone;
    uint32_t spinFails;
    uint32_t pad;
    u64 dbg[8];
};

typedef __attribute__((address_space(1))) u64 *gu64p;
typedef __attribute__((address_space(1))) uint32_t *gu32p;

__device__ __forceinline__ u64 svc_tag(u64 n, uint32_t entries) { return (n / entries) % 255ull + 1ull; }
__device__ __forceinline__ u64 svc_payload(u64 g) { return g & 0x00FFFFFFFFFFFFFFull; }


constexpr uint32_t kSvcProfiles = 24u;
__device__ __forceinline__ uint32_t svc_profile_index(uint32_t levelByte) { return ((levelByte & 0x7Fu) - 1u) + ((levelByte & 0x80u) ? 12u : 0u); }

template <bool HAS_LONG, bool REP, bool CHAIN, bool TURNS, bool MULTI>
__global__ __launch_bounds__(kThreads) void qzstd_service_worker(LaunchArgs args, SvcDev *sv, uint32_t ctlOff, uint32_t spinLimit, const qzstd_hip_profile_t *profs)
{
    const uint32_t tid = threadIdx.x, lane = tid & 63u;
    const uint32_t wave = rdfirst(tid >> 6);
    uint32_t *ctl = (uint32_t *)(__attribute__((address_space(3))) uint32_t *)(size_t)(kLdsBase + ctlOff);
    if (tid == 0u) (void)__hip_atomic_fetch_add(&sv->started, 1u, QZ_RLX_AGENT);
    for (;;) {
        if (wave == 0u) {
            uint32_t t = 0u;
            if (lane == 0u) t = __hip_atomic_fetch_add(&sv->head, 1u, QZ_RLX_AGENT);
            t = rdfirst(t);
            const u64 want = svc_tag(t, kSvcQueue);
            const u64 *slot = sv->items[t & (kSvcQueue - 1u)];
            u64 g = 0;
            uint32_t got = 0u;
            for (;;) {
                if (lane < 8u) g = __hip_atomic_load(slot + lane, QZ_RLX_AGENT);
                else if (lane == 8u) g = (u64)__hip_atomic_load(&sv->quit, QZ_RLX_AGENT);
                const bool mine = lane >= 8u || (g >> 56) == want;
                if (__all(mine)) { got = 1u; break; }
                if (rdlane((uint32_t)g, 8u) != 0u) break;
                __builtin_amdgcn_s_sleep(4);
            }
            if (lane < 8u) { ctl[2u * lane] = (uint32_t)g; ctl[2u * lane + 1u] = (uint32_t)(svc_payload(g) >> 32); }
            if (lane == 8u) ctl[16] = got;
            if (lane == 0u && got) (void)__hip_atomic_fetch_add(&sv->taken, 1u, QZ_RLX_AGENT);
        }
        __syncthreads();
        if (rdfirst(ctl[16]) == 0u) return;
        const u64 q0 = rdfirst(ctl[0]) | ((u64)rdfirst(ctl[1]) << 32), q1 = rdfirst(ctl[2]) | ((u64)rdfirst(ctl[3]) << 32),
                  q2 = rdfirst(ctl[4]) | ((u64)rdfirst(ctl[5]) << 32), q3 = rdfirst(ctl[6]) | ((u64)rdfirst(ctl[7]) << 32),
                  q4 = rdfirst(ctl[8]) | ((u64)rdfirst(ctl[9]) << 32), q5 = rdfirst(ctl[10]), q6 = rdfirst(ctl[12]),
                  q7 = rdfirst(ctl[14]) | ((u64)rdfirst(ctl[15]) << 32);
        const uint8_t *hSrc = (const uint8_t *)q0;
        uint8_t *dSrc = (uint8_t *)q1;
        uint4 *out = (uint4 *)q2;
        uint32_t *countWord = (uint32_t *)q3;
        qzstd_hip_block_t blk;
        blk.srcOff = 0; blk.seqOff = 0;
        blk.srcLen = (uint32_t)q4 & 0x3FFFFu;
        blk.parseFrom = (uint32_t)(q4 >> 18) & 0x3FFFFu;
        blk.seqCap = (uint32_t)q5 & 0xFFFFFFu;
        const uint32_t nItemsReq = (uint32_t)(q5 >> 24) & 63u;
        const uint32_t k = (uint32_t)(q4 >> 36) & 63u, slotIdx = (uint32_t)(q4 >> 42) & (kSvcSlots - 1u);
        const uint32_t epoch = (uint32_t)q6 & 0xFFFFFFu;
        blk.mark = epoch;
        {
            const uint32_t end = (blk.srcLen + 15u) & ~15u;
            if (wave == 0u) {
                uint32_t spins = 0u, okS = 1u;
                while (__hip_atomic_load(countWord, QZ_RLX_SYSTEM) == QZSTD_HIP_NSEQ_STAGING) {
                    if (++spins > spinLimit) { okS = 0u; break; }
                    __builtin_amdgcn_s_sleep(8);
                }
                __builtin_amdgcn_fence(__ATOMIC_ACQUIRE, "");
                if (lane == 0u) ctl[18] = okS;
            }
            __syncthreads();
            const bool staged = rdfirst(ctl[18]) != 0u;
            for (uint32_t o = blk.parseFrom + tid * 16u; o < end && staged; o += (uint32_t)kThreads * 16u) {
                const u64 a = __hip_atomic_load((const u64 *)(hSrc + o), QZ_RLX_SYSTEM);
                const u64 b = __hip_atomic_load((const u64 *)(hSrc + o + 8u), QZ_RLX_SYSTEM);
                __hip_atomic_store((u64 *)(dSrc + o), a, QZ_RLX_AGENT);
                __hip_atomic_store((u64 *)(dSrc + o + 8u), b, QZ_RLX_AGENT);
            }
            asm volatile("s_waitcnt vmcnt(0)" ::: "memory");
            __syncthreads();
            if (wave == 0u) {
                if (lane == 0u && staged) __hip_atomic_store(&sv->sliceFlag[slotIdx][k], epoch, QZ_RLX_AGENT);
                uint32_t spins = 0u, ok = 1u;
                for (;;) {
                    const bool there = lane >= k || __hip_atomic_load(&sv->sliceFlag[slotIdx][lane], QZ_RLX_AGENT) == epoch;
                    if (__all(there)) break;
                    if (++spins > spinLimit) { ok = 0u; break; }
                    __builtin_amdgcn_s_sleep(2);
                }
                __builtin_amdgcn_fence(__ATOMIC_ACQUIRE, "agent");
                if (lane == 0u) ctl[17] = staged ? ok : 0u;
            }
            __syncthreads();
        }
        uint32_t count = QZSTD_HIP_NSEQ_ERROR;
#define QZ_SVC_ITEM(A, L, R, C, T)                                                                                                            \
    qz_item<L, R, C, T, false>(A, blk, dSrc, out, (C) ? (uint4 *)q7 : nullptr, (C) ? (uint32_t *)(q7 + (u64)QZSTD_HIP_BLOCK_MAX * (8ull * QZSTD_HIP_CHAIN_ENTRY_LINKS)) : nullptr, \
                               HistShare{ (C) ? &sv->histFlag[slotIdx][0] : nullptr, k, epoch, spinLimit, nItemsReq, &sv->tabFlag[slotIdx][0],   \
                                          &sv->linkFlag[slotIdx][0], (C) ? (uint32_t *)(q7 + (u64)QZSTD_HIP_BLOCK_MAX * (8ull * QZSTD_HIP_CHAIN_ENTRY_LINKS + 4ull)) : nullptr })
        if (rdfirst(ctl[17]) != 0u) {
            if (MULTI) {
                LaunchArgs a2 = args;
                const uint32_t pi = rdfirst(svc_profile_index((uint32_t)(q6 >> 24) & 0xFFu));
                a2.prof = profs[pi < kSvcProfiles ? pi : 0u];
                const bool chain = a2.prof.chainDepth != 0u, rpt = a2.prof.repWin != 0u, turns = a2.prof.subTileLog != 0u;
                if (chain) count = rpt ? QZ_SVC_ITEM(a2, false, true, true, true) : QZ_SVC_ITEM(a2, false, false, true, true);
                else if (turns) count = rpt ? QZ_SVC_ITEM(a2, false, true, false, true) : QZ_SVC_ITEM(a2, false, false, false, true);
                else count = rpt ? QZ_SVC_ITEM(a2, false, true, false, false) : QZ_SVC_ITEM(a2, false, false, false, false);
            } else {
                count = QZ_SVC_ITEM(args, HAS_LONG, REP, CHAIN, TURNS);
            }
        } else if (tid == 0u) (void)__hip_atomic_fetch_add(&sv->spinFails, 1u, QZ_RLX_AGENT);
#undef QZ_SVC_ITEM
        asm volatile("s_waitcnt vmcnt(0)" ::: "memory");
        __syncthreads();
        if (tid == (uint32_t)kMatchThreads) {
            __hip_atomic_store(countWord, count, __ATOMIC_RELEASE, __HIP_MEMORY_SCOPE_SYSTEM);
            (void)__hip_atomic_fetch_add(&sv->done, 1u, QZ_RLX_AGENT);
        }
    }
}

__global__ __launch_bounds__(64) void qzstd_service_dispatcher(SvcHost *hs, SvcDev *sv, uint32_t served, uint32_t idleUs, uint32_t drainUs)
{
    const uint32_t lane = threadIdx.x;
    u64 head = __hip_atomic_load(&hs->consumed, QZ_RLX_SYSTEM);
    uint32_t tail = 0u;
    u64 lastWork = __builtin_amdgcn_s_memrealtime();
    u64 polls = 0, seen = 0;
    for (;;) {
        u64 g = 0;
        if ((++polls & 255u) == 0u && lane < 6u) {
            const u64 v = lane == 0u ? polls : lane == 1u ? seen : lane == 2u ? (u64)tail : lane == 3u ? (u64)__hip_atomic_load(&sv->started, QZ_RLX_AGENT)
                        : lane == 4u ? (u64)__hip_atomic_load(&sv->taken, QZ_RLX_AGENT) : (u64)__hip_atomic_load(&sv->done, QZ_RLX_AGENT);
            __hip_atomic_store(&hs->dbg[lane], v, QZ_RLX_SYSTEM);
        }
        if (lane < 8u) g = __hip_atomic_load(&hs->ring[head & (kSvcRing - 1u)][lane], QZ_RLX_SYSTEM);
        else if (lane == 8u) g = (u64)__hip_atomic_load(&hs->quitReq, QZ_RLX_SYSTEM);
        const bool mine = lane >= 8u || (g >> 56) == svc_tag(head, kSvcRing);
        const bool quitReq = rdlane((uint32_t)g, 8u) != 0u;
        if (__all(mine) && !quitReq) {
            const u64 r0 = svc_payload(__shfl(g, 0)), r1 = svc_payload(__shfl(g, 1)), r2 = svc_payload(__shfl(g, 2)),
                      r3 = svc_payload(__shfl(g, 3)), r4 = svc_payload(__shfl(g, 4)), r5 = svc_payload(__shfl(g, 5)),
                      r6 = svc_payload(__shfl(g, 6)), r7 = svc_payload(__shfl(g, 7));
            const uint32_t srcLen = (uint32_t)r4 & 0x3FFFFu, itemBytes = (uint32_t)(r4 >> 18) & 0x3FFFFu;
            const uint32_t nItems = (uint32_t)(r4 >> 36) & 63u, slotIdx = (uint32_t)(r4 >> 42) & (kSvcSlots - 1u);
            const uint32_t cap = (uint32_t)r5 & 0xFFFFFFu, epoch = (uint32_t)r6 & 0xFFFFFFu, lv = (uint32_t)(r6 >> 24) & 0xFFu;
            const bool sane = nItems >= 1u && nItems <= kSvcMaxItems && itemBytes != 0u && srcLen != 0u && srcLen <= QZSTD_HIP_BLOCK_MAX &&
                              (u64)(nItems - 1u) * itemBytes < srcLen && (lv & 0x7Fu) >= 1u && (lv & 0x7Fu) <= 12u &&
                              ((served >> svc_profile_index(lv)) & 1u) != 0u;
            if (!sane) {
                if (lane < umin(nItems, kSvcMaxItems)) __hip_atomic_store((uint32_t *)r3 + lane, kSvcRejected, __ATOMIC_RELEASE, __HIP_MEMORY_SCOPE_SYSTEM);
            } else {
                uint32_t spins = 0u;
                while (tail + nItems - __hip_atomic_load(&sv->done, QZ_RLX_AGENT) > kSvcQueue && ++spins < (1u << 24)) __builtin_amdgcn_s_sleep(8);
                if (lane < nItems) {
                    const u64 t = (u64)tail + lane, tg = svc_tag(t, kSvcQueue) << 56;
                    u64 *e = sv->items[t & (kSvcQueue - 1u)];
                    const uint32_t from = lane * itemBytes;
                    const uint32_t upTo = umin(srcLen, from + itemBytes);
                    __hip_atomic_store(e + 0, tg | r0, QZ_RLX_AGENT);
                    __hip_atomic_store(e + 1, tg | r1, QZ_RLX_AGENT);
                    __hip_atomic_store(e + 2, tg | (r2 + (u64)lane * cap * 16ull), QZ_RLX_AGENT);
                    __hip_atomic_store(e + 3, tg | (r3 + 4ull * lane), QZ_RLX_AGENT);
                    __hip_atomic_store(e + 4, tg | upTo | ((u64)from << 18) | ((u64)lane << 36) | ((u64)slotIdx << 42), QZ_RLX_AGENT);
                    __hip_atomic_store(e + 5, tg | cap | ((u64)nItems << 24), QZ_RLX_AGENT);
                    __hip_atomic_store(e + 6, tg | epoch | ((u64)lv << 24), QZ_RLX_AGENT);
                    __hip_atomic_store(e + 7, tg | r7, QZ_RLX_AGENT);
                }
                tail += nItems;
            }
            head++;
            seen++;
            if (lane == 0u) __hip_atomic_store(&hs->consumed, head, QZ_RLX_SYSTEM);
            lastWork = __builtin_amdgcn_s_memrealtime();
            continue;
        }
        const u64 now = __builtin_amdgcn_s_memrealtime();
        const bool drained = __hip_atomic_load(&sv->done, QZ_RLX_AGENT) == tail;
        if (quitReq || (drained && now - lastWork > (u64)idleUs * 100ull)) {
            if (!quitReq) {
                if (lane == 0u) __hip_atomic_store(&hs->state, 2u, __ATOMIC_RELEASE, __HIP_MEMORY_SCOPE_SYSTEM);
                u64 g2 = 0;
                if (lane < 8u) g2 = __hip_atomic_load(&hs->ring[head & (kSvcRing - 1u)][lane], QZ_RLX_SYSTEM);
                if (__all(lane >= 8u || (g2 >> 56) == svc_tag(head, kSvcRing))) {
                    if (lane == 0u) __hip_atomic_store(&hs->state, 1u, __ATOMIC_RELEASE, __HIP_MEMORY_SCOPE_SYSTEM);
                    lastWork = now;
                    continue;
                }
            }
            const u64 t0 = __builtin_amdgcn_s_memrealtime();
            while (__hip_atomic_load(&sv->done, QZ_RLX_AGENT) != tail && __builtin_amdgcn_s_memrealtime() - t0 < (u64)drainUs * 100ull)
                __builtin_amdgcn_s_sleep(16);
            if (lane == 0u) {
                __hip_atomic_store(&sv->quit, 1u, QZ_RLX_AGENT);
                __hip_atomic_store(&hs->itemsDone, hs->itemsDone + __hip_atomic_load(&sv->done, QZ_RLX_AGENT), QZ_RLX_SYSTEM);
                __hip_atomic_store(&hs->spinFails, hs->spinFails + __hip_atomic_load(&sv->spinFails, QZ_RLX_AGENT), QZ_RLX_SYSTEM);
                __hip_atomic_store(&hs->state, 0u, __ATOMIC_RELEASE, __HIP_MEMORY_SCOPE_SYSTEM);
            }
            return;
        }
        __builtin_amdgcn_s_sleep(2);
    }
}

__global__ __launch_bounds__(kThreads) void qzstd_probe_lds_order(uint32_t *bad)
{
    __shared__ uint32_t slots[64];
    __shared__ uint32_t noise[4096];
    const uint32_t tid = threadIdx.x, lane = tid & 63u, wave = tid >> 6;
    uint32_t wrong = 0;
    for (uint32_t i = tid; i < 4096u; i += kThreads) noise[i] = 0u;
    for (uint32_t round = 0; round < 64u; round++) {
        if (wave == 0u) slots[lane] = 0u;
        __syncthreads();
        if (wave == 0u) {
            uint32_t slot;
            switch (round & 7u) {
            case 0: slot = 0u; break;
            case 1: slot = lane & 1u; break;
            case 2: slot = lane >> 3; break;
            case 3: slot = lane % 7u; break;
            case 4: slot = (lane * 2654435761u + round) >> 28; break;
            case 5: slot = (lane * 0x85EBCA77u + round) >> 26; break;
            case 6: slot = lane < 32u ? 5u : lane & 3u; break;
            default: slot = (lane ^ (lane >> 2)) & 31u; break;
            }
            const uint32_t mine = (round << 8) + lane + 1u;
            const uint32_t got = atomicMax(&slots[slot], mine);
            uint32_t want = 0u;
            for (uint32_t l = 0; l < 64u; l++) {
                const uint32_t sl = (uint32_t)__shfl((int)slot, (int)l);
                if (l < lane && sl == slot) want = (round << 8) + l + 1u;
            }
            if (got != want) wrong++;
        } else {
            uint32_t acc = 0u;
            for (uint32_t k = 0; k < 24u; k++) {
                const uint32_t a = (tid * 2654435761u + k * 40503u + round * 977u) >> 20;
                acc += atomicMax(&noise[a], tid + k);
                atomicMin(&noise[(a * 33u + 7u) & 4095u], acc);
                acc ^= noise[(a + 64u * k) & 4095u];
                noise[(a ^ 1u) & 4095u] = acc;
            }
            if (acc == 0xDEADBEEFu) wrong += 0u * acc;
        }
        __syncthreads();
    }
    if (wrong) atomicAdd(bad, wrong);
}

struct Service {
    std::mutex mu;
    SvcHost *hs = nullptr;
    SvcDev *dv = nullptr;
    hipStream_t sWork = nullptr, sDisp = nullptr;
    hipEvent_t ev = nullptr;
    int level = 0;
    uint32_t served = 0;
    qzstd_hip_profile_t *dProfs = nullptr;
    int workers = 0;
    int broken = 0;
    std::atomic<unsigned long long> reserve{0};
    unsigned long launches = 0, requests = 0, refused = 0;
    static constexpr int kBig = 64;
    hipEvent_t bigEv[kBig] = {};
    bool bigUsed[kBig] = {};
    size_t bigLds[kBig] = {};
    int bigNext = 0;
    size_t lds = 0;
    long long launchNs = 0;
    bool sawWorkers = false;
    bool wide = false;
};
Service g_svc[64];
std::atomic<int> g_svcFreeze{0};

struct SvcConfig { int enabled, workers, idleUs, spinLimit; };
const SvcConfig &svc_config()
{
    static const SvcConfig c = [] {
        SvcConfig k;
        const char *e = getenv("QZSTD_HIP_SERVICE"), *w = getenv("QZSTD_HIP_SERVICE_WORKERS"), *i = getenv("QZSTD_HIP_SERVICE_IDLE_US");
        k.enabled = e ? atoi(e) : 1;
        k.workers = w ? atoi(w) : 0;
        k.idleUs = i ? atoi(i) : 20000;
        if (k.idleUs < 100) k.idleUs = 100;
        k.spinLimit = 1 << 20;
        return k;
    }();
    return c;
}

int svc_stop_locked(Service &s, unsigned waitMs)
{
    if (!s.hs) return 0;
    if (__atomic_load_n(&s.hs->state, __ATOMIC_ACQUIRE) != 0u) {
        __atomic_store_n(&s.hs->quitReq, 1u, __ATOMIC_RELEASE);
        struct timespec t0, t;
        clock_gettime(CLOCK_MONOTONIC, &t0);
        while (__atomic_load_n(&s.hs->state, __ATOMIC_ACQUIRE) != 0u) {
            clock_gettime(CLOCK_MONOTONIC, &t);
            if ((t.tv_sec - t0.tv_sec) * 1000ll + (t.tv_nsec - t0.tv_nsec) / 1000000ll > (long long)waitMs) { s.broken = 1; return 1; }
            sched_yield();
        }
    }
    return 0;
}

#define QZ_SEARCHES(X, last)                                                                                    \
    X(false, false, false, false, last), X(false, true, false, false, last),        \
    X(false, false, false, true, last), X(false, true, false, true, last),                \
    X(false, false, true, true, last), X(false, true, true, true, last),      \
    X(true, false, false, false, last), X(true, true, false, false, last)
#define QZ_K(L, R, C, T, N) reinterpret_cast<const void *>(qzstd_find_sequences_kernel<L, R, C, T, N>)
#define QZ_W(L, R, C, T, M) reinterpret_cast<const void *>(qzstd_service_worker<L, R, C, T, M>)
const void *const kLaunchKernels[16] = { QZ_SEARCHES(QZ_K, false), QZ_SEARCHES(QZ_K, true) };
const void *const kWorkers[8] = { QZ_SEARCHES(QZ_W, false) };
#undef QZ_K
#undef QZ_W
#undef QZ_SEARCHES

int variant_index(const qzstd_hip_profile_t &p, bool nearK)
{
    const int search = p.chainDepth ? 2 : (p.longSize ? 3 : (p.subTileLog ? 1 : 0));
    return (nearK ? 8 : 0) + 2 * search + (p.repWin ? 1 : 0);
}

}

SvcFreeze::SvcFreeze()
{
    g_svcFreeze.fetch_add(1);
    for (int d = 0; d < 64; d++) {
        Service &s = g_svc[d];
        if (!s.hs) continue;
        std::lock_guard<std::mutex> g(s.mu);
        (void)svc_stop_locked(s, 2000);
    }
}
SvcFreeze::~SvcFreeze() { g_svcFreeze.fetch_sub(1); }

static int g_ldsOrdered[64];
static std::mutex g_probeMu;

int probe_lds_order(int device, int physDev)
{
    {
        const int known = __atomic_load_n(&g_ldsOrdered[device], __ATOMIC_ACQUIRE);
        if (known > 0) return known - 1;
    }
    std::lock_guard<std::mutex> g(g_probeMu);
    if (g_ldsOrdered[device] > 0) return g_ldsOrdered[device] - 1;
    int verdict = 0;
    const char *force = getenv("QZSTD_HIP_ORDERED_LDS");
    uint32_t *dBad = nullptr, hBad = 1u;
    if (!(force && atoi(force) == 0) && hipSetDevice(physDev) == hipSuccess && hipMalloc(&dBad, sizeof(uint32_t)) == hipSuccess) {
        if (hipMemset(dBad, 0, sizeof(uint32_t)) == hipSuccess) {
            hipLaunchKernelGGL(qzstd_probe_lds_order, dim3(512), dim3(kThreads), 0, 0, dBad);
            if (hipGetLastError() == hipSuccess && hipMemcpy(&hBad, dBad, sizeof(uint32_t), hipMemcpyDeviceToHost) == hipSuccess)
                verdict = hBad == 0u;
        }
        (void)hipFree(dBad);
    }
    (void)hipGetLastError();
    __atomic_store_n(&g_ldsOrdered[device], verdict + 1, __ATOMIC_RELEASE);
    return verdict;
}

extern "C" {

int qzstd_hip_find_sequences(int device, void *stream, int level, const void *d_src,
                             const qzstd_hip_block_t *d_blocks, uint32_t nBlocks, uint32_t maxBlockLen,
                             void *d_seqs, uint32_t *d_nseq, void *d_work, size_t workBytes)
{
    LaunchArgs a;
    if (nBlocks == 0) return 0;
    if (!d_src || !d_blocks || !d_seqs || !d_nseq) return fail_msg("qzstd_hip_find_sequences: null pointer");
    if (maxBlockLen > QZSTD_HIP_BLOCK_MAX) return fail_msg("qzstd_hip_find_sequences: block larger than 128 KiB");
    if (qzstd_hip_profile_for_level(level, maxBlockLen, &a.prof))
        return fail_msg("qzstd_hip_find_sequences: level outside 1..12 (optionally | QZSTD_HIP_LEVEL_REPCODES)");
    if (a.prof.tileLog != kTileLog || a.prof.extLog < 8 || a.prof.extLog > 15 || a.prof.capLen > 48 || a.prof.capLen < 32 ||
        a.prof.minMatch < 4 || a.prof.hashBytes < 4 || a.prof.hashBytes > 8 || a.prof.repWin > 16 || a.prof.chainDepth > 64 ||
        a.prof.lazy > 4 || (a.prof.subTileLog != 0u && a.prof.subTileLog != 6u) || (a.prof.segLog != 0u && (a.prof.segLog < kTileLog || a.prof.segLog > 17u)) ||
        (a.prof.chainDepth && (a.prof.subTileLog != 6u || a.prof.longSize || a.prof.nearTab)) || (a.prof.longSize && a.prof.subTileLog))
        return fail_msg("qzstd_hip_find_sequences: unsupported profile");
    const size_t lds = qzstd_hip_lds_bytes(level, maxBlockLen);
    if (lds == 0) return fail_msg("qzstd_hip_find_sequences: LDS budget exceeded");
    QZ_SET_DEVICE(device);
    bool big = lds + qzstd_hip_lds_bytes(1, QZSTD_HIP_BLOCK_MAX) > kLdsPerCu;
    std::unique_lock<std::mutex> bigLock;
    if (device >= 0 && device < 64) {
        Service &sv = g_svc[device];
        bigLock = std::unique_lock<std::mutex>(sv.mu);
        big = big || sv.wide;
        if (sv.hs && __atomic_load_n(&sv.hs->state, __ATOMIC_ACQUIRE) != 0u && lds + sv.lds > kLdsPerCu) (void)svc_stop_locked(sv, 2000);
    }
    {
        static std::mutex attrMu;
        static bool attrDone[64];
        std::lock_guard<std::mutex> g(attrMu);
        if (phys(device) < 0) return fail_msg("qzstd_hip_find_sequences: device index out of range");
        if (!attrDone[device]) {
            size_t most = 0;
            for (int l = 1; l <= 12; l++) {
                const size_t b = qzstd_hip_lds_bytes(l, QZSTD_HIP_BLOCK_MAX);
                if (b > most) most = b;
            }
            for (const void *f : kLaunchKernels)
                QZ_CHECK(hipFuncSetAttribute(f, hipFuncAttributeMaxDynamicSharedMemorySize, (int)most),
                         "hipFuncSetAttribute(MaxDynamicSharedMemorySize)");
            attrDone[device] = true;
        }
    }
    a.chain = nullptr;
    a.pwWords = 0;
    a.chainStride = 0;
    a.chainEntries = 0;
    a.orderedLds = 0;
    if (a.prof.chainDepth) {
        a.orderedLds = (uint32_t)probe_lds_order(device, phys(device));
        const size_t need = qzstd_hip_workspace_bytes(level, nBlocks, maxBlockLen);
        if (!d_work || workBytes < need) return fail_msg("qzstd_hip_find_sequences: workspace missing or too small (qzstd_hip_workspace_bytes)");
        a.chain = static_cast<uint4 *>(d_work);
        a.chainStride = (uint32_t)(need / nBlocks / sizeof(uint4));
        a.chainEntries = (uint32_t)(need / nBlocks / (4u * QZSTD_HIP_CHAIN_ENTRY_LINKS + 4u)) * kEQ;
    } else {
        const size_t need = qzstd_hip_workspace_bytes(level, nBlocks, maxBlockLen);
        if (!d_work || workBytes < need || need == 0) return fail_msg("qzstd_hip_find_sequences: workspace missing or too small (qzstd_hip_workspace_bytes)");
        a.chain = static_cast<uint4 *>(d_work);
        a.chainStride = (uint32_t)(need / nBlocks / sizeof(uint4));
        a.pwWords = (uint32_t)(need / nBlocks / 33u * 8u);
    }
    if (a.prof.segLog != 12u) return fail_msg("qzstd_hip_find_sequences: unsupported profile (the deferred parse of a launch works on 4 KiB segments)");
    a.src = static_cast<const uint8_t *>(d_src);
    a.blocks = d_blocks;
    a.seqs = static_cast<uint4 *>(d_seqs);
    a.nseq = d_nseq;
#ifdef QZ_DEBUG_DUMP
    { const char *ab = getenv("QZSTD_HIP_ABLATE"); a.dbg = ab ? (uint32_t)atoi(ab) : 0u; }
#endif
#ifdef QZ_DEBUG_DUMP
    size_t ldsLaunch = lds;
    { const char *pad = getenv("QZSTD_HIP_LDS_PAD"); if (pad) ldsLaunch += (size_t)atoi(pad); }
#else
    const size_t ldsLaunch = lds;
#endif
    const dim3 grid(nBlocks), wg(kThreads);
    const void *kernel = kLaunchKernels[variant_index(a.prof, maxBlockLen <= kRing)];
    void *kargs[1] = { &a };
    if (!a.prof.chainDepth && ((a.prof.tableSize & (a.prof.tableSize - 1u)) != 0u || (a.prof.longSize & (a.prof.longSize - 1u)) != 0u || a.prof.hashBytes > 7u))
        return fail_msg("qzstd_hip_find_sequences: unsupported profile (tables below the chain levels are powers of two, hashBytes <= 7)");
    QZ_CHECK(hipLaunchKernel(kernel, grid, wg, kargs, ldsLaunch, (hipStream_t)stream), "launch qzstd_find_sequences_kernel");
    QZ_CHECK(hipGetLastError(), "launch qzstd_find_sequences_kernel");
    if (big && bigLock.owns_lock()) {
        Service &sv = g_svc[device];
        int k = sv.bigNext;
        for (int tries = 0; tries < Service::kBig && sv.bigUsed[k]; tries++) {
            if (hipEventQuery(sv.bigEv[k]) != hipErrorNotReady) { (void)hipGetLastError(); sv.bigUsed[k] = false; break; }
            k = (k + 1) % Service::kBig;
        }
        if (sv.bigUsed[k]) { (void)hipEventSynchronize(sv.bigEv[k]); (void)hipGetLastError(); }
        sv.bigNext = (k + 1) % Service::kBig;
        if (!sv.bigEv[k] && hipEventCreateWithFlags(&sv.bigEv[k], hipEventDisableTiming) != hipSuccess) { sv.bigEv[k] = nullptr; (void)hipGetLastError(); }
        if (sv.bigEv[k] && hipEventRecord(sv.bigEv[k], (hipStream_t)stream) == hipSuccess) { sv.bigUsed[k] = true; sv.bigLds[k] = lds; }
        else (void)hipGetLastError();
    }
    return 0;
}

int qzstd_hip_occupancy(int device, int level)
{
    qzstd_hip_profile_t p;
    if (qzstd_hip_profile_for_level(level, QZSTD_HIP_BLOCK_MAX, &p)) return fail_msg("qzstd_hip_occupancy: bad level");
    const size_t lds = qzstd_hip_lds_bytes(level, QZSTD_HIP_BLOCK_MAX);
    QZ_SET_DEVICE(device);
    const void *k = kLaunchKernels[variant_index(p, false)];
    (void)hipFuncSetAttribute(k, hipFuncAttributeMaxDynamicSharedMemorySize, (int)lds);
    int n = 0;
    QZ_CHECK(hipOccupancyMaxActiveBlocksPerMultiprocessor(&n, k, kThreads, lds), "hipOccupancyMaxActiveBlocksPerMultiprocessor");
    return n;
}

}

namespace {

const void *svc_worker_variant(const qzstd_hip_profile_t &p) { return kWorkers[variant_index(p, false)]; }

int svc_level_index(int level)
{
    const int l = level & ~QZSTD_HIP_LEVEL_REPCODES;
    return (l >= 1 && l <= 12) ? (l - 1) + ((level & QZSTD_HIP_LEVEL_REPCODES) ? 12 : 0) : -1;
}

int svc_launch_locked(int device, Service &s, int level)
{
    const SvcConfig &cfg = svc_config();
    LaunchArgs a;
    memset(&a, 0, sizeof(a));
    if (qzstd_hip_profile_for_level(level, QZSTD_HIP_BLOCK_MAX, &a.prof)) return fail_msg("service: bad level");
    static const bool multiOn = [] { const char *v = getenv("QZSTD_HIP_SERVICE_MULTI"); return !(v && atoi(v) == 0); }();
    const bool multi = multiOn && a.prof.longSize == 0u;
    const void *worker = multi ? reinterpret_cast<const void *>(qzstd_service_worker<false, false, false, false, true>) : svc_worker_variant(a.prof);
    size_t lds = qzstd_hip_lds_bytes(level, QZSTD_HIP_BLOCK_MAX);
    uint32_t served = 0u;
    qzstd_hip_profile_t profs[kSvcProfiles];
    memset(profs, 0, sizeof(profs));
    for (int l = 1; l <= 12; l++)
        for (int r = 0; r < 2; r++) {
            const int lv = l | (r ? QZSTD_HIP_LEVEL_REPCODES : 0), ix = svc_level_index(lv);
            qzstd_hip_profile_t p;
            if (ix < 0 || qzstd_hip_profile_for_level(lv, QZSTD_HIP_BLOCK_MAX, &p)) continue;
            profs[ix] = p;
            if (multi ? p.longSize == 0u : lv == level) {
                served |= 1u << ix;
                if (multi && qzstd_hip_lds_bytes(lv, QZSTD_HIP_BLOCK_MAX) > lds) lds = qzstd_hip_lds_bytes(lv, QZSTD_HIP_BLOCK_MAX);
            }
        }
    if (!worker || lds == 0) return fail_msg("service: level not served");
    if (a.prof.chainDepth || multi) a.orderedLds = (uint32_t)probe_lds_order(device, phys(device));
    QZ_SET_DEVICE(device);
    for (int k = 0; k < Service::kBig; k++) {
        if (!s.bigUsed[k]) continue;
        const hipError_t q = hipEventQuery(s.bigEv[k]);
        if (q == hipErrorNotReady) {
            if (s.bigLds[k] + lds > kLdsPerCu) return fail_msg("service: a launch that cannot share a CU with its workers is in flight");
            continue;
        }
        (void)hipGetLastError();
        s.bigUsed[k] = false;
    }
    if (lds + qzstd_hip_lds_bytes(1, QZSTD_HIP_BLOCK_MAX) > kLdsPerCu && !s.wide) {
        s.wide = true;
        QZ_CHECK(hipDeviceSynchronize(), "hipDeviceSynchronize(before the first service of levels 3-4)");
    }
    if (!s.hs) {
        hipDeviceProp_t prop;
        QZ_CHECK(hipGetDeviceProperties(&prop, phys(device)), "hipGetDeviceProperties");
        s.workers = cfg.workers > 0 ? cfg.workers : (prop.multiProcessorCount / g_devReplicas > 0 ? prop.multiProcessorCount / g_devReplicas : 1);
        if (s.workers > 1024) s.workers = 1024;
        void *h = nullptr, *d = nullptr;
        {
            const char *nm = getenv("QZSTD_HIP_NUMA");
            h = qzstd_hip_host_alloc_on_node(sizeof(SvcHost), (nm && atoi(nm) == 0) ? -1 : qzstd_hip_device_numa_node(device), 1);
            if (!h) return fail_msg("service: no pinned memory for the request ring");
            QZ_SET_DEVICE(device);
        }
        memset(h, 0, sizeof(SvcHost));
        int prLeast = 0, prGreatest = 0;
        (void)hipDeviceGetStreamPriorityRange(&prLeast, &prGreatest);
        if (hipMalloc(&d, sizeof(SvcDev)) != hipSuccess || hipStreamCreateWithPriority(&s.sWork, hipStreamNonBlocking, prGreatest) != hipSuccess ||
            hipStreamCreateWithPriority(&s.sDisp, hipStreamNonBlocking, prGreatest) != hipSuccess || hipEventCreateWithFlags(&s.ev, hipEventDisableTiming) != hipSuccess) {
            (void)hipGetLastError();
            if (d) (void)hipFree(d);
            (void)hipHostFree(h);
            s.broken = 1;
            return fail_msg("service: set-up failed");
        }
        s.hs = static_cast<SvcHost *>(h);
        s.dv = static_cast<SvcDev *>(d);
        static std::once_flag once;
        std::call_once(once, [] {
            atexit([] {
                for (int dvc = 0; dvc < 64; dvc++) {
                    Service &sv = g_svc[dvc];
                    if (!sv.hs) continue;
                    std::lock_guard<std::mutex> g(sv.mu);
                    (void)svc_stop_locked(sv, 500);
                }
            });
        });
    }
    QZ_CHECK(hipFuncSetAttribute(worker, hipFuncAttributeMaxDynamicSharedMemorySize, (int)lds), "hipFuncSetAttribute(service worker)");
    QZ_CHECK(hipStreamSynchronize(s.sDisp), "hipStreamSynchronize(service dispatcher stream)");
    QZ_CHECK(hipMemsetAsync(s.dv, 0, sizeof(SvcDev), s.sWork), "hipMemsetAsync(service queue)");
    QZ_CHECK(hipStreamSynchronize(s.sWork), "hipStreamSynchronize(service worker stream)");
    __atomic_store_n(&s.hs->quitReq, 0u, __ATOMIC_RELEASE);
    __atomic_store_n(&s.hs->dbg[3], 0ull, __ATOMIC_RELAXED);
    s.sawWorkers = false;
    {
        struct timespec t;
        clock_gettime(CLOCK_MONOTONIC, &t);
        __atomic_store_n(&s.launchNs, (long long)t.tv_sec * 1000000000ll + t.tv_nsec, __ATOMIC_RELAXED);
    }
    if (!s.dProfs && hipMalloc(reinterpret_cast<void **>(&s.dProfs), sizeof(profs)) != hipSuccess) { (void)hipGetLastError(); s.dProfs = nullptr; return fail_msg("service: no memory for the profile table"); }
    QZ_CHECK(hipMemcpyAsync(s.dProfs, profs, sizeof(profs), hipMemcpyHostToDevice, s.sWork), "hipMemcpyAsync(service profiles)");
    QZ_CHECK(hipStreamSynchronize(s.sWork), "hipStreamSynchronize(service worker stream)");
    __atomic_store_n(&s.hs->state, 1u, __ATOMIC_RELEASE);
    s.level = level;
    s.served = served;
    s.lds = lds;
    SvcHost *hsDev = nullptr;
    QZ_CHECK(hipHostGetDevicePointer(reinterpret_cast<void **>(&hsDev), s.hs, 0), "hipHostGetDevicePointer");
    uint32_t ctlOff = (uint32_t)(lds - QZSTD_HIP_LDS_SVC - kLdsBase), spin = (uint32_t)cfg.spinLimit;
    void *wargs[5] = { &a, &s.dv, &ctlOff, &spin, &s.dProfs };
    uint32_t idle = (uint32_t)cfg.idleUs, drain = 1000000u;
    void *dargs[5] = { &hsDev, &s.dv, &served, &idle, &drain };
    hipError_t e = hipLaunchKernel(reinterpret_cast<const void *>(qzstd_service_dispatcher), dim3(1), dim3(64), dargs, 0, s.sDisp);
    if (e != hipSuccess) {
        __atomic_store_n(&s.hs->state, 0u, __ATOMIC_RELEASE);
        s.broken = 1;
        return fail("launch of the service dispatcher", e);
    }
    e = hipLaunchKernel(worker, dim3((unsigned)s.workers), dim3(kThreads), wargs, lds, s.sWork);
    if (e != hipSuccess) {
        __atomic_store_n(&s.hs->quitReq, 1u, __ATOMIC_RELEASE);
        s.broken = 1;
        return fail("launch of the service workers", e);
    }
    s.launches++;
    return 0;
}

}

extern "C" {

int qzstd_hip_service_submit(int device, int level, const qzstd_hip_svc_req_t *r)
{
    const SvcConfig &cfg = svc_config();
    if (!cfg.enabled || g_svcFreeze.load() > 0 || device < 0 || device >= 64 || phys(device) < 0 || !r) return 1;
    Service &s = g_svc[device];
    if (s.broken) return 1;
    {
        qzstd_hip_profile_t p;
        if (qzstd_hip_profile_for_level(level, QZSTD_HIP_BLOCK_MAX, &p) || !svc_worker_variant(p)) return 1;
        if (p.chainDepth && !r->dWork) return fail_msg("qzstd_hip_service_submit: the chain levels need dWork");
    }
    if (r->nItems < 1u || r->nItems > kSvcMaxItems || r->slot >= kSvcSlots || r->srcLen == 0u || r->srcLen > QZSTD_HIP_BLOCK_MAX ||
        r->itemBytes == 0u || (size_t)(r->nItems - 1u) * r->itemBytes >= r->srcLen || (r->itemBytes & 15u) || !r->hSrc || !r->dSrc ||
        !r->hSeqs || !r->hCount || r->seqCapPerItem < 4u || r->seqCapPerItem > 0xFFFFFFu)
        return fail_msg("qzstd_hip_service_submit: bad request");
    if (!s.hs || __atomic_load_n(&s.hs->state, __ATOMIC_ACQUIRE) == 0u) {
        std::lock_guard<std::mutex> g(s.mu);
        if (s.broken || g_svcFreeze.load() > 0) return 1;
        if (!s.hs || __atomic_load_n(&s.hs->state, __ATOMIC_ACQUIRE) == 0u) {
            if (svc_launch_locked(device, s, level) != 0) return 1;
        }
    }
    {
        const int ix = svc_level_index(level);
        if (ix < 0 || !((s.served >> ix) & 1u)) { s.refused++; return 1; }
    }
    void *dvSrc = nullptr, *dvSeqs = nullptr, *dvCount = nullptr;
    if (hipHostGetDevicePointer(&dvSrc, const_cast<void *>(r->hSrc), 0) != hipSuccess || hipHostGetDevicePointer(&dvSeqs, r->hSeqs, 0) != hipSuccess ||
        hipHostGetDevicePointer(&dvCount, r->hCount, 0) != hipSuccess) {
        (void)hipGetLastError();
        return fail_msg("qzstd_hip_service_submit: the buffers are not pinned host memory");
    }
    const unsigned long long n = s.reserve.fetch_add(1);
    {
        struct timespec t0, t;
        clock_gettime(CLOCK_MONOTONIC, &t0);
        unsigned spins = 0;
        while (n - __atomic_load_n(&s.hs->consumed, __ATOMIC_ACQUIRE) >= kSvcRing) {
            if ((++spins & 1023u) == 0u) {
                clock_gettime(CLOCK_MONOTONIC, &t);
                if (t.tv_sec - t0.tv_sec >= 2) { s.broken = 1; return fail_msg("qzstd_hip_service_submit: the request ring stays full"); }
                sched_yield();
            }
        }
    }
    const u64 tg = ((n / kSvcRing) % 255ull + 1ull) << 56;
    const u64 lv = (u64)((unsigned)level & 0xFFu) | ((level & QZSTD_HIP_LEVEL_REPCODES) ? 0x80ull : 0ull);
    volatile u64 *e = s.hs->ring[n & (kSvcRing - 1u)];
    e[0] = tg | (u64)(uintptr_t)dvSrc;
    e[1] = tg | (u64)(uintptr_t)r->dSrc;
    e[2] = tg | (u64)(uintptr_t)dvSeqs;
    e[3] = tg | (u64)(uintptr_t)dvCount;
    e[4] = tg | (u64)r->srcLen | ((u64)r->itemBytes << 18) | ((u64)r->nItems << 36) | ((u64)r->slot << 42);
    e[5] = tg | (u64)r->seqCapPerItem;
    e[6] = tg | (u64)(r->epoch & 0xFFFFFFu) | (lv << 24);
    e[7] = tg | (u64)(uintptr_t)r->dWork;
    std::atomic_thread_fence(std::memory_order_seq_cst);
    uint32_t st;
    unsigned spins = 0;
    while ((st = __atomic_load_n(&s.hs->state, __ATOMIC_ACQUIRE)) == 2u && ++spins < (1u << 26)) {}
    if (st != 1u) {
        std::lock_guard<std::mutex> g(s.mu);
        if (__atomic_load_n(&s.hs->state, __ATOMIC_ACQUIRE) == 0u && !s.broken && g_svcFreeze.load() == 0) (void)svc_launch_locked(device, s, level);
    }
    __atomic_fetch_add(&s.requests, 1ul, __ATOMIC_RELAXED);
    return 0;
}

int qzstd_hip_service_progressive(int device)
{
    static int on = -1;
    (void)device;
    if (on < 0) { const char *v = getenv("QZSTD_HIP_SERVICE_EARLY"); on = !(v && *v && atoi(v) == 0); }
    return on;
}

int qzstd_hip_service_poke(int device, int level)
{
    if (device < 0 || device >= 64) return -1;
    Service &s = g_svc[device];
    if (!s.hs) return 1;
    if (__atomic_load_n(&s.hs->state, __ATOMIC_ACQUIRE) != 0u) {
        if (!s.sawWorkers) {
            if (__atomic_load_n(&s.hs->dbg[3], __ATOMIC_RELAXED) != 0ull) s.sawWorkers = true;
            else {
                struct timespec t;
                clock_gettime(CLOCK_MONOTONIC, &t);
                if ((long long)t.tv_sec * 1000000000ll + t.tv_nsec - s.launchNs > 200000000ll) {
                    s.broken = 1;
                    __atomic_store_n(&s.hs->quitReq, 1u, __ATOMIC_RELEASE);
                    return 2;
                }
            }
        }
        return 0;
    }
    if (s.broken) return 2;
    if (g_svcFreeze.load() > 0) return 1;
    std::lock_guard<std::mutex> g(s.mu);
    if (__atomic_load_n(&s.hs->state, __ATOMIC_ACQUIRE) != 0u) return 0;
    if (__atomic_load_n(&s.hs->consumed, __ATOMIC_ACQUIRE) >= s.reserve.load()) return 0;
    return svc_launch_locked(device, s, level) == 0 ? 0 : 1;
}

int qzstd_hip_service_stop(int device)
{
    if (device < 0 || device >= 64) return -1;
    Service &s = g_svc[device];
    std::lock_guard<std::mutex> g(s.mu);
    if (!s.hs) return 0;
    const int r = svc_stop_locked(s, 2000);
    if (r == 0 && phys(device) >= 0 && hipSetDevice(phys(device)) == hipSuccess) {
        (void)hipStreamSynchronize(s.sWork);
        (void)hipStreamSynchronize(s.sDisp);
    }
    __atomic_store_n(&s.hs->consumed, (u64)s.reserve.load(), __ATOMIC_RELEASE);
    return r;
}

void qzstd_hip_service_mark_broken(int device)
{
    if (device < 0 || device >= 64) return;
    Service &s = g_svc[device];
    s.broken = 1;
    if (s.hs) __atomic_store_n(&s.hs->quitReq, 1u, __ATOMIC_RELEASE);
}

int qzstd_hip_service_info(int device, unsigned long out[8])
{
    if (device < 0 || device >= 64 || !out) return -1;
    Service &s = g_svc[device];
    for (int k = 0; k < 8; k++) out[k] = 0;
    out[0] = s.launches;
    out[1] = s.requests;
    out[2] = s.refused;
    out[3] = (unsigned long)s.broken;
    if (s.hs) {
        out[4] = (unsigned long)__atomic_load_n(&s.hs->state, __ATOMIC_ACQUIRE);
        out[5] = (unsigned long)s.hs->itemsDone;
        out[6] = (unsigned long)s.hs->spinFails;
        out[7] = (unsigned long)s.workers;
    }
    return 0;
}

int qzstd_hip_service_debug(int device, unsigned long out[8])
{
    if (device < 0 || device >= 64 || !out) return -1;
    Service &s = g_svc[device];
    for (int k = 0; k < 8; k++) out[k] = 0;
    if (!s.hs) return 0;
    for (int k = 0; k < 6; k++) out[k] = (unsigned long)__atomic_load_n(&s.hs->dbg[k], __ATOMIC_RELAXED);
    out[6] = (unsigned long)__atomic_load_n(&s.hs->consumed, __ATOMIC_RELAXED);
    out[7] = (unsigned long)s.reserve.load() | ((unsigned long)__atomic_load_n(&s.hs->quitReq, __ATOMIC_RELAXED) << 62) |
             ((unsigned long)(g_svcFreeze.load() > 0) << 61);
    return 0;
}

}
```

### qat-zstd-plugin_amd/csrc/qzstd_profile.c

```c
#include "qzstd_hip.h"

#include <string.h>


int qzstd_hip_profile_for_level(int level, size_t blockSize, qzstd_hip_profile_t *out)
{
    const int repcodes = (level & QZSTD_HIP_LEVEL_REPCODES) != 0;
    level &= ~QZSTD_HIP_LEVEL_REPCODES;
    if (level < 1 || level > 12 || !out) return -1;
    memset(out, 0, sizeof(*out));
    (void)blockSize;
    {
        const int chains = level >= 5;
        out->tableSize = chains ? QZ_CHAIN_TABLE : (level >= 3 ? 16384u : 8192u);
        out->longSize = (!chains && level >= 3) ? 8192u : 0u;
        out->tileLog = 9;
#ifndef QZ_CAP_HI
#define QZ_CAP_HI 48u
#endif
#ifndef QZ_CAP_MID
#define QZ_CAP_MID 48u
#endif
#ifndef QZ_DEPTH_HI
#define QZ_DEPTH_HI 40u
#endif
        out->capLen = level >= 9 ? QZ_CAP_HI : (level >= 5 ? QZ_CAP_MID : 48u);
        out->minMatch = 4;
        out->farLog1 = 12;
        out->farLog2 = 16;
        out->lazy = chains ? 4u : 3u;
        out->backExt = 4;
        out->nearTab = chains ? 0u : 1u;
        out->window = 0;
        out->hashBytes = chains ? 4u : 5u;
        out->extLog = 11;
        out->repWin = (repcodes || level >= 10) ? 16u : 0u;
#ifndef QZ_DEPTH_6
#define QZ_DEPTH_6 12u
#endif
        out->chainDepth = level >= 10 ? QZ_DEPTH_HI : (level >= 9 ? 64u : (level >= 7 ? 32u : (level >= 6 ? QZ_DEPTH_6 : (level >= 5 ? 8u : 0u))));
        out->subTileLog = (chains || level == 2) ? 6u : 0u;
        out->segLog = 12u;
    }
    return 0;
}

size_t qzstd_hip_sequence_bound(size_t srcSize)
{
    return srcSize / 3 + 1 + srcSize / 1024 + 1;
}

size_t qzstd_hip_workspace_bytes(int level, uint32_t nBlocks, uint32_t maxBlockLen)
{
    qzstd_hip_profile_t p;
    if (maxBlockLen > QZSTD_HIP_BLOCK_MAX || qzstd_hip_profile_for_level(level, maxBlockLen, &p)) return 0;
    if (!p.chainDepth)
        return (size_t)nBlocks * ((((size_t)maxBlockLen + 511u) & ~(size_t)511u) / 8u * 33u);
    return (size_t)nBlocks * (((size_t)maxBlockLen + 511u) & ~(size_t)511u) * (4u * QZSTD_HIP_CHAIN_ENTRY_LINKS + 4u);
}

size_t qzstd_hip_lds_bytes(int level, uint32_t maxBlockLen)
{
    qzstd_hip_profile_t p;
    size_t need;
    const size_t lag = 2u;
    if (maxBlockLen > QZSTD_HIP_BLOCK_MAX || qzstd_hip_profile_for_level(level, maxBlockLen, &p)) return 0;
    need = (size_t)QZ_RING + QZSTD_HIP_RING_MIRROR
           + 4u * p.tableSize
           + 4u * p.longSize
           + (4u << p.tileLog)
           + lag * ((4u << p.tileLog) + 32u)
           + lag * ((1u << p.tileLog) >> 6) * 32u
           + (p.chainDepth ? (4u << p.tileLog) : 0u)
           + QZSTD_HIP_LDS_BASE + QZSTD_HIP_LDS_CTRL + QZSTD_HIP_LDS_SVC;
    return need <= QZSTD_HIP_LDS_MAX ? need : 0;
}
```

Baseline: 23630.

## Add small-ring, no-service-wave kernel variant for levels 1-2 to raise occupancy

Result: no change. 23410 (-0.9%).

```diff
diff --git a/include/qzstd_hip.h b/include/qzstd_hip.h
--- a/include/qzstd_hip.h
+++ b/include/qzstd_hip.h
@@ -59,6 +59,7 @@
 #ifndef QZ_RING
 #define QZ_RING 32768u
 #endif
+#define QZ_RING_SMALL 16384u
 #define QZSTD_HIP_RING_MIRROR 128u
 #ifndef QZ_CHAIN_TABLE
 #define QZ_CHAIN_TABLE 5888u
diff --git a/qat-zstd-plugin_amd/csrc/qzstd_hip_internal.h b/qat-zstd-plugin_amd/csrc/qzstd_hip_internal.h
--- a/qat-zstd-plugin_amd/csrc/qzstd_hip_internal.h
+++ b/qat-zstd-plugin_amd/csrc/qzstd_hip_internal.h
@@ -2,6 +2,9 @@
 #define QZSTD_HIP_INTERNAL_H
 
 #include <hip/hip_runtime.h>
+
+extern "C" size_t qzstd_hip_launch_lds_bytes(int level, uint32_t maxBlockLen, int flags);
+extern "C" int qzstd_hip_launch_residency(int device, int level, uint32_t maxBlockLen, unsigned long out[4]);
 
 #pragma GCC visibility push(hidden)
 
diff --git a/qat-zstd-plugin_amd/csrc/qzstd_kernels.hip b/qat-zstd-plugin_amd/csrc/qzstd_kernels.hip
--- a/qat-zstd-plugin_amd/csrc/qzstd_kernels.hip
+++ b/qat-zstd-plugin_amd/csrc/qzstd_kernels.hip
@@ -24,7 +24,6 @@
 #ifndef QZ_WAVES_PER_EU
 #define QZ_WAVES_PER_EU 5
 #endif
-#define QZ_OCCUPANCY __attribute__((amdgpu_waves_per_eu(QZ_WAVES_PER_EU)))
 
 #ifdef QZ_DEBUG_DUMP
 #define QZ_PLAP(acc) { const u64 tN = __builtin_amdgcn_s_memtime(); acc += tN - tQ; tQ = tN; }
@@ -41,6 +40,7 @@
 constexpr int kMatchWaves = 8;
 constexpr int kMatchThreads = kMatchWaves * 64;
 constexpr int kThreads = kMatchThreads + 64;
+constexpr int kSmallThreads = kMatchThreads;
 constexpr uint32_t kTileLog = 9;
 constexpr uint32_t kTile = 1u << kTileLog;
 constexpr uint32_t kWin = kTile >> 6;
@@ -49,12 +49,8 @@
 constexpr uint32_t kPrime1 = 2654435761u;
 constexpr uint32_t kPrime2 = 0x85EBCA77u;
 constexpr uint32_t kNone = 0xFFFFFFFFu;
-constexpr uint32_t kRing = QZ_RING;
-constexpr uint32_t kRingMask = kRing - 1u;
 constexpr uint32_t kMirror = QZSTD_HIP_RING_MIRROR;
 constexpr uint32_t kLook = 4608u;
-constexpr uint32_t kNear = kRing - kLook - 3u * kTile - 1024u;
-static_assert((kRing & kRingMask) == 0u && kRing >= 16384u, "the ring is a power of two of at least 16 KiB");
 constexpr size_t kLdsPerCu = QZSTD_HIP_LDS_MAX;
 constexpr uint32_t kEL = QZSTD_HIP_CHAIN_ENTRY_LINKS;
 constexpr uint32_t kEQ = QZSTD_HIP_CHAIN_ENTRY_LINKS / 4u;
@@ -102,22 +98,30 @@
 
 typedef const __attribute__((address_space(3))) uint32_t *LdsWords;
 typedef const __attribute__((address_space(1))) uint32_t *HbmWords;
-struct Src {
+template <uint32_t RING>
+struct SrcT {
+    static constexpr uint32_t kRing = RING;
+    static constexpr uint32_t kRingMask = RING - 1u;
+    static constexpr uint32_t kNear = RING - kLook - 3u * kTile - 1024u;
+    static_assert((RING & (RING - 1u)) == 0u && RING >= 16384u, "the ring is a power of two of at least 16 KiB");
     LdsWords ring;
     HbmWords g;
     uint32_t nearLimit;
 };
 
+template <uint32_t RING>
 __device__ __forceinline__ uint32_t ring_dw(uint32_t a)
 {
-    return (a & kRingMask) >> 2;
-}
-
-__device__ __forceinline__ uint32_t ring_fwd(uint32_t r, uint32_t d) { return (r + d) & kRingMask; }
-__device__ __forceinline__ uint32_t ring_back(uint32_t r, uint32_t d) { return (r - d) & kRingMask; }
-
-template <int N>
-__device__ __forceinline__ void load_dw_r(const Src &s, uint32_t a, uint32_t r, bool far, uint32_t (&D)[N])
+    return (a & (RING - 1u)) >> 2;
+}
+
+template <uint32_t RING>
+__device__ __forceinline__ uint32_t ring_fwd(uint32_t r, uint32_t d) { return (r + d) & (RING - 1u); }
+template <uint32_t RING>
+__device__ __forceinline__ uint32_t ring_back(uint32_t r, uint32_t d) { return (r - d) & (RING - 1u); }
+
+template <int N, class S>
+__device__ __forceinline__ void load_dw_r(const S &s, uint32_t a, uint32_t r, bool far, uint32_t (&D)[N])
 {
     if (far) {
         const uint32_t d = a >> 2;
@@ -130,15 +134,15 @@
     }
 }
 
-template <int N>
-__device__ __forceinline__ void load_dw(const Src &s, uint32_t a, bool far, uint32_t (&D)[N])
+template <int N, class S>
+__device__ __forceinline__ void load_dw(const S &s, uint32_t a, bool far, uint32_t (&D)[N])
 {
     if (far) {
         const uint32_t d = a >> 2;
 #pragma unroll
         for (int i = 0; i < N; i++) D[i] = s.g[d + i];
     } else {
-        const uint32_t d = ring_dw(a);
+        const uint32_t d = ring_dw<S::kRing>(a);
 #pragma unroll
         for (int i = 0; i < N; i++) D[i] = s.ring[d + i];
     }
@@ -151,26 +155,29 @@
     return r;
 }
 
-__device__ __forceinline__ uint32_t rd32u(const Src &s, uint32_t a, bool far)
+template <class S>
+__device__ __forceinline__ uint32_t rd32u(const S &s, uint32_t a, bool far)
 {
     uint32_t D[2];
     load_dw<2>(s, a, far, D);
     return __builtin_amdgcn_alignbyte(D[1], D[0], a & 3u);
 }
 
-__device__ __forceinline__ uint32_t rd32_r(const Src &s, uint32_t a, uint32_t r, bool far)
+template <class S>
+__device__ __forceinline__ uint32_t rd32_r(const S &s, uint32_t a, uint32_t r, bool far)
 {
     uint32_t D[2];
     load_dw_r<2>(s, a, r, far, D);
     return __builtin_amdgcn_alignbyte(D[1], D[0], a & 3u);
 }
 
-__device__ __forceinline__ uint32_t chunk_len(const Src &s, uint32_t p, uint32_t rp, uint32_t off, bool far)
+template <class S>
+__device__ __forceinline__ uint32_t chunk_len(const S &s, uint32_t p, uint32_t rp, uint32_t off, bool far)
 {
     const uint32_t q = p - off, ps = p & 3u, qs = q & 3u;
     uint32_t P[9], Q[9];
     load_dw_r<9>(s, p, rp, false, P);
-    load_dw_r<9>(s, q, ring_back(rp, off), far, Q);
+    load_dw_r<9>(s, q, ring_back<S::kRing>(rp, off), far, Q);
     uint32_t B = 256u;
 #pragma unroll
     for (int i = 0; i < 8; i++) {
@@ -180,7 +187,8 @@
     return B >> 3;
 }
 
-__device__ __forceinline__ uint32_t head_len(const Src &s, const uint32_t (&oa)[4], uint32_t q, uint32_t rq, bool far)
+template <class S>
+__device__ __forceinline__ uint32_t head_len(const S &s, const uint32_t (&oa)[4], uint32_t q, uint32_t rq, bool far)
 {
     const uint32_t qs = q & 3u;
     uint32_t Q[5];
@@ -216,7 +224,8 @@
     return B >> 3;
 }
 
-__device__ __forceinline__ uint32_t tail_len(const Src &s, const uint32_t (&pa)[8], uint32_t q, uint32_t rq, bool far)
+template <class S>
+__device__ __forceinline__ uint32_t tail_len(const S &s, const uint32_t (&pa)[8], uint32_t q, uint32_t rq, bool far)
 {
     const uint32_t qs = q & 3u;
     uint32_t Q[9];
@@ -240,8 +249,8 @@
     return pf.minMatch + ((off >> pf.farLog1) ? 1u : 0u) + ((off >> pf.farLog2) ? 1u : 0u);
 }
 
-template <bool AFAR = false>
-__device__ __forceinline__ uint32_t extend_match_from(const Src &s, uint32_t p, uint32_t off, uint32_t L, uint32_t lim,
+template <bool AFAR = false, class S>
+__device__ __forceinline__ uint32_t extend_match_from(const S &s, uint32_t p, uint32_t off, uint32_t L, uint32_t lim,
                                                       uint32_t lane, const bool far ,
                                                       const uint32_t lastDw = 0xFFFFFFFFu )
 {
@@ -278,7 +287,8 @@
     }
 }
 
-__device__ __forceinline__ uint32_t extend_match(const Src &s, uint32_t p, uint32_t off, uint32_t L, uint32_t lim, uint32_t lane)
+template <class S>
+__device__ __forceinline__ uint32_t extend_match(const S &s, uint32_t p, uint32_t off, uint32_t L, uint32_t lim, uint32_t lane)
 {
     return extend_match_from(s, p, off, L, lim, lane, off > s.nearLimit);
 }
@@ -328,8 +338,8 @@
     uint32_t r0, r1, r2, r3, r4, r5;
 };
 
-template <uint32_t W>
-__device__ __forceinline__ void parse_window(const qzstd_hip_profile_t &pf, const Src &src, const uint32_t wordW,
+template <uint32_t W, class S>
+__device__ __forceinline__ void parse_window(const qzstd_hip_profile_t &pf, const S &src, const uint32_t wordW,
                                              uint32_t base, uint32_t n, uint32_t lane, ParseState &st, ParseRecs &r)
 {
     constexpr uint32_t w = W;
@@ -371,8 +381,8 @@
     }
 }
 
-template <uint32_t W, uint32_t W_END>
-__device__ __forceinline__ void parse_windows(const qzstd_hip_profile_t &pf, const Src &src, const uint32_t (&word)[kWin],
+template <uint32_t W, uint32_t W_END, class S>
+__device__ __forceinline__ void parse_windows(const qzstd_hip_profile_t &pf, const S &src, const uint32_t (&word)[kWin],
                                               uint32_t base, uint32_t n, uint32_t lane, ParseState &st, ParseRecs &r)
 {
     if constexpr (W < W_END) {
@@ -381,8 +391,8 @@
     }
 }
 
-template <uint32_t W_BEGIN, uint32_t W_END>
-__device__ __forceinline__ void parse_tile(const qzstd_hip_profile_t &pf, const Src &src, const uint32_t *pv,
+template <uint32_t W_BEGIN, uint32_t W_END, class S>
+__device__ __forceinline__ void parse_tile(const qzstd_hip_profile_t &pf, const S &src, const uint32_t *pv,
                                            uint32_t *srecOut, uint32_t base, uint32_t n, uint32_t lane, ParseState &st)
 {
     uint32_t word[kWin];
@@ -409,13 +419,15 @@
 constexpr uint32_t kLenCapped = 127u;
 constexpr uint32_t kChosenBit = 0x80000000u;
 
-__device__ __forceinline__ uint32_t ring_byte(const Src &s, uint32_t x, bool far)
+template <class S>
+__device__ __forceinline__ uint32_t ring_byte(const S &s, uint32_t x, bool far)
 {
     if (far) return reinterpret_cast<const __attribute__((address_space(1))) uint8_t *>(s.g)[x];
-    return reinterpret_cast<const __attribute__((address_space(3))) uint8_t *>(s.ring)[x & kRingMask];
-}
-
-__device__ __forceinline__ u64 rep_bitmap(const Src &src, uint32_t cur, uint32_t rp, uint32_t n, uint32_t lane, uint32_t ringFrom = 0u)
+    return reinterpret_cast<const __attribute__((address_space(3))) uint8_t *>(s.ring)[x & S::kRingMask];
+}
+
+template <class S>
+__device__ __forceinline__ u64 rep_bitmap(const S &src, uint32_t cur, uint32_t rp, uint32_t n, uint32_t lane, uint32_t ringFrom = 0u)
 {
     const uint32_t bpos = cur + lane;
     bool eq = false;
@@ -428,13 +440,14 @@
     return (u64)q | ((u64)off << 17) | ((u64)L << 34) | ((u64)lit << 47);
 }
 
+template <uint32_t RING>
 __device__ __forceinline__ uint32_t ring_off_s(uint32_t a)
 {
-    return a & kRingMask;
-}
-
-template <bool DEF>
-__device__ __forceinline__ void parse_rep_span(const qzstd_hip_profile_t &pf, const Src &src, uint32_t *pvT,
+    return a & (RING - 1u);
+}
+
+template <bool DEF, class S>
+__device__ __forceinline__ void parse_rep_span(const qzstd_hip_profile_t &pf, const S &src, uint32_t *pvT,
                                                uint32_t base, uint32_t limit, uint32_t n, uint32_t nh, uint32_t lane,
                                                RepState &st, const uint32_t ringFrom = 0u, u64 *recG = nullptr)
 {
@@ -447,7 +460,7 @@
         st.rep1 = st.rep2 = 0u;
         st.seg = base >> pf.segLog;
     }
-    uint32_t rc = rdfirst(ring_off_s(st.cur));
+    uint32_t rc = rdfirst(ring_off_s<S::kRing>(st.cur));
     const __attribute__((address_space(3))) uint8_t *rb = reinterpret_cast<const __attribute__((address_space(3))) uint8_t *>(src.ring);
     while (st.cur < stop) {
         const uint32_t rem = tileLim - st.cur;
@@ -459,7 +472,7 @@
         if (DEF ? (st.cur - st.rep1 >= ringFrom && st.cur - st.rep2 >= ringFrom)
                 : (st.rep1 <= src.nearLimit && st.rep2 <= src.nearLimit)) {
             const uint32_t t1 = rc - st.rep1, t2 = rc - st.rep2;
-            const uint32_t r1 = t1 & kRingMask, r2 = t2 & kRingMask;
+            const uint32_t r1 = t1 & S::kRingMask, r2 = t2 & S::kRingMask;
             const uint32_t A = rb[rc + lane], B1 = rb[r1 + lane], B2 = rb[r2 + lane];
             const u64 in = below(segEnd - st.cur);
             M1 = st.rep1 ? __ballot(A == B1) & in : 0ull;
@@ -481,7 +494,7 @@
         const u64 m = __ballot(ok);
         if (!m) {
             st.cur += W;
-            rc = ring_fwd(rc, W);
+            rc = ring_fwd<S::kRing>(rc, W);
             continue;
         }
         const uint32_t ks = (uint32_t)__builtin_ctzll(m);
@@ -518,7 +531,7 @@
             st.rep1 = off;
         }
         st.cur = st.anchor = q + L;
-        rc = rdfirst(ring_off_s(st.cur));
+        rc = rdfirst(ring_off_s<S::kRing>(st.cur));
         (void)curIn;
     }
 }
@@ -526,8 +539,8 @@
 struct PlainParse {
     uint32_t cur, cnt, endA;
 };
-template <uint32_t W0, uint32_t W1>
-__device__ __forceinline__ void parse_plain_windows(const qzstd_hip_profile_t &pf, const Src &src, u64 *recG, const uint32_t base, const uint32_t n,
+template <uint32_t W0, uint32_t W1, class S>
+__device__ __forceinline__ void parse_plain_windows(const qzstd_hip_profile_t &pf, const S &src, u64 *recG, const uint32_t base, const uint32_t n,
                                                     const uint32_t lastDw, const uint32_t lane, const uint32_t (&wds)[kWin], PlainParse &st)
 {
     u64 smA[kWin], chA[kWin];
@@ -602,8 +615,8 @@
         out[idx] = make_uint4(off, lit, ml, mark);
 }
 
-template <bool REP>
-__device__ __forceinline__ void emit_window(const qzstd_hip_profile_t &pf, const Src &src, const uint32_t *srec,
+template <bool REP, class S>
+__device__ __forceinline__ void emit_window(const qzstd_hip_profile_t &pf, const S &src, const uint32_t *srec,
                                             const uint32_t *pvW, uint32_t off, uint32_t len, uint32_t w0, uint32_t rpE,
                                             uint32_t lane, uint4 *out, uint32_t seqCap, uint32_t tileSeq, uint32_t mark)
 {
@@ -644,11 +657,11 @@
         uint32_t b = 0;
         if (maxb) {
             const bool far = off > src.nearLimit;
-            const uint32_t rp4 = ring_back(rpE, 4u);
+            const uint32_t rp4 = ring_back<S::kRing>(rpE, 4u);
             const uint32_t pb = rd32_r(src, p - 4u, rp4, false);
             uint32_t qb;
             if (far) qb = q >= 4u ? rd32u(src, q - 4u, true) : rd32u(src, 0u, true) << (8u * (4u - q));
-            else qb = rd32_r(src, q - 4u, ring_back(rp4, off), false);
+            else qb = rd32_r(src, q - 4u, ring_back<S::kRing>(rp4, off), false);
             const uint32_t x = pb ^ qb;
             b = umin(x ? (uint32_t)__builtin_clz(x) >> 3 : 4u, maxb);
         }
@@ -682,7 +695,8 @@
     return vk ? (predLane != lane ? fromLane : prd) : 0u;
 }
 
-__device__ __forceinline__ void chain_insert_tile(const qzstd_hip_profile_t &pf, const Src &src, uint32_t *tbl, uint32_t *P1, uint32_t t0,
+template <class S>
+__device__ __forceinline__ void chain_insert_tile(const qzstd_hip_profile_t &pf, const S &src, uint32_t *tbl, uint32_t *P1, uint32_t t0,
                                                   uint32_t n, uint32_t nh, uint32_t lane, bool ordered)
 {
     const uint32_t segE = rdfirst(seg_end(pf, t0, n));
@@ -744,10 +758,15 @@
 constexpr uint32_t kSvcTabStride = QZ_CHAIN_TABLE;
 static_assert((uint32_t)kMatchWaves * kPvStride <= QZ_CHAIN_TABLE, "the deferred parse's eight windows of parse words must fit in the head table (QZ_CHAIN_TABLE)");
 
-template <bool HAS_LONG, bool REP, bool CHAIN, bool TURNS, bool NEAR, bool DEFER = false>
+template <bool HAS_LONG, bool REP, bool CHAIN, bool TURNS, bool NEAR, bool DEFER = false, bool SMALL = false>
 __device__ __forceinline__ uint32_t qz_item(const LaunchArgs &args, const qzstd_hip_block_t &blk, const uint8_t *gsrc, uint4 *out,
                                             uint4 *chainB, uint32_t *p1B, const HistShare hsh)
 {
+    static_assert(!SMALL || (DEFER && !REP && !CHAIN && !HAS_LONG && !NEAR), "the small-ring layout: a deferring plain-parse kernel of levels 1-2 (the deferred repeat-aware parse stages 32 KiB quarters in the ring)");
+    using S = SrcT<SMALL ? QZ_RING_SMALL : QZ_RING>;
+    using Src = S;
+    constexpr uint32_t kRing = S::kRing, kRingMask = S::kRingMask, kNear = S::kNear;
+    constexpr int kThr = SMALL ? kSmallThreads : kThreads;
     extern __shared__ __attribute__((aligned(16))) uint8_t smem[];
     const uint32_t tid = threadIdx.x;
     const uint32_t lane = tid & 63u;
@@ -779,7 +798,7 @@
     uint32_t *nearTab = tblL + pf.longSize;
     uint32_t *srec = nearTab + kTile;
     uint32_t *pv = srec + kLagT * kWin * kSrecWords;
-    uint32_t *turnCtr = pv + kLagT * kPvStride;
+    uint32_t *turnCtr = SMALL ? nearTab + kTile : pv + kLagT * kPvStride;
     uint32_t *P1odd = turnCtr + QZSTD_HIP_LDS_CTRL / 4u;
     const uint4 *g128 = reinterpret_cast<const uint4 *>(gsrc);
     Src src;
@@ -792,16 +811,17 @@
     const uint32_t histEnd = itBegin << kTileLog;
     const uint32_t hi = umin(nPad, histEnd + kLook + (itBegin ? 0u : kTile));
     const uint32_t lo = hi > kRing ? (hi - kRing + 15u) & ~15u : 0u;
-    constexpr uint32_t kStep = (uint32_t)kThreads * 16u;
+    constexpr uint32_t kStep = (uint32_t)kThr * 16u;
     const uint32_t hashEnd = CHAIN ? 0u : histEnd;
     uint32_t fo = (hashEnd ? 0u : lo) + tid * 16u;
     uint4 fa0 = make_uint4(0u, 0u, 0u, 0u), fb0 = fa0, fa1 = fa0, fb1 = fa0;
     if (fo < hi) { fa0 = g128[fo >> 4]; if (fo < hashEnd) fb0 = g128[(fo >> 4) + 1u]; }
     if (fo + kStep < hi) { fa1 = g128[(fo + kStep) >> 4]; if (fo + kStep < hashEnd) fb1 = g128[((fo + kStep) >> 4) + 1u]; }
-    for (uint32_t i = tid; i < pf.tableSize + pf.longSize; i += kThreads) tbl[i] = 0u;
+    for (uint32_t i = tid; i < pf.tableSize + pf.longSize; i += kThr) tbl[i] = 0u;
     if (!(CHAIN && itBegin != 0u)) {
-        for (uint32_t i = tid; i < kTile; i += kThreads) nearTab[i] = 0xFFFFFFFFu;
-        for (uint32_t i = tid; i < kLagT * kWin * kSrecWords + kLagT * kPvStride + QZSTD_HIP_LDS_CTRL / 4u; i += kThreads) srec[i] = 0u;
+        for (uint32_t i = tid; i < kTile; i += kThr) nearTab[i] = 0xFFFFFFFFu;
+        if constexpr (SMALL) { if (tid < QZSTD_HIP_LDS_CTRL / 4u) turnCtr[tid] = 0u; }
+        else for (uint32_t i = tid; i < kLagT * kWin * kSrecWords + kLagT * kPvStride + QZSTD_HIP_LDS_CTRL / 4u; i += kThr) srec[i] = 0u;
     }
     const bool sharedHist = CHAIN && hsh.flags != nullptr && hsh.nItems > 1u && pf.tableSize <= kSvcTabStride;
     if (itBegin != 0u || sharedHist) __syncthreads();
@@ -881,13 +901,13 @@
         }
         {
             uint32_t *mine = hsh.tabs + (size_t)k * kSvcTabStride;
-            for (uint32_t i = tid; i < pf.tableSize; i += kThreads) __hip_atomic_store(&mine[i], tbl[i], QZ_RLX_AGENT);
+            for (uint32_t i = tid; i < pf.tableSize; i += kThr) __hip_atomic_store(&mine[i], tbl[i], QZ_RLX_AGENT);
             asm volatile("s_waitcnt vmcnt(0)" ::: "memory");
             __syncthreads();
             if (tid == 0u) __hip_atomic_store(&hsh.tabFlags[k], hsh.epoch, QZ_RLX_AGENT);
         }
         if (!wait_for(hsh.tabFlags)) return QZSTD_HIP_NSEQ_ERROR;
-        for (uint32_t i = tid; i < pf.tableSize; i += kThreads) {
+        for (uint32_t i = tid; i < pf.tableSize; i += kThr) {
             uint32_t m = 0u;
             for (uint32_t j = 0; j < k; j++) m = umax(m, hsh.tabs[(size_t)j * kSvcTabStride + i]);
             tbl[i] = m;
@@ -915,17 +935,17 @@
         if (tid == 0u) __hip_atomic_store(&hsh.linkFlags[k], hsh.epoch, QZ_RLX_AGENT);
         if (!wait_for(hsh.linkFlags)) return QZSTD_HIP_NSEQ_ERROR;
         constexpr uint32_t kCh = 16u / kEL;
-        for (uint32_t p0 = a0 + tid; p0 < b0; p0 += kCh * (uint32_t)kThreads) {
+        for (uint32_t p0 = a0 + tid; p0 < b0; p0 += kCh * (uint32_t)kThr) {
             uint32_t e[kEL][kCh];
 #pragma unroll
-            for (uint32_t i = 0; i < kCh; i++) { const uint32_t pp = p0 + i * (uint32_t)kThreads; e[0][i] = pp < b0 ? __hip_atomic_load(&p1B[pp], QZ_RLX_AGENT) : 0u; }
+            for (uint32_t i = 0; i < kCh; i++) { const uint32_t pp = p0 + i * (uint32_t)kThr; e[0][i] = pp < b0 ? __hip_atomic_load(&p1B[pp], QZ_RLX_AGENT) : 0u; }
 #pragma unroll
             for (uint32_t d = 1; d < kEL; d++)
 #pragma unroll
                 for (uint32_t i = 0; i < kCh; i++) e[d][i] = e[d - 1u][i] ? __hip_atomic_load(&p1B[(e[d - 1u][i] >> kTagBits) - 1u], QZ_RLX_AGENT) : 0u;
 #pragma unroll
             for (uint32_t i = 0; i < kCh; i++) {
-                const uint32_t pp = p0 + i * (uint32_t)kThreads;
+                const uint32_t pp = p0 + i * (uint32_t)kThr;
                 if (pp < b0) {
                     u64 *w = reinterpret_cast<u64 *>(chainB + (size_t)pp * kEQ);
 #pragma unroll
@@ -937,11 +957,11 @@
         __syncthreads();
         if (tid == 0u) __hip_atomic_store(&hsh.flags[k], hsh.epoch, QZ_RLX_AGENT);
         if (!wait_for(hsh.flags)) return QZSTD_HIP_NSEQ_ERROR;
-        for (uint32_t i = tid; i < kTile; i += kThreads) nearTab[i] = 0xFFFFFFFFu;
-        for (uint32_t i = tid; i < kLagT * kWin * kSrecWords + kLagT * kPvStride + QZSTD_HIP_LDS_CTRL / 4u; i += kThreads) srec[i] = 0u;
+        for (uint32_t i = tid; i < kTile; i += kThr) nearTab[i] = 0xFFFFFFFFu;
+        for (uint32_t i = tid; i < kLagT * kWin * kSrecWords + kLagT * kPvStride + QZSTD_HIP_LDS_CTRL / 4u; i += kThr) srec[i] = 0u;
     } else if (CHAIN && itBegin != 0u) {
         constexpr uint32_t kGroup = 4096u;
-        static_assert(kGroup * 8u <= kRing, "two words per position of a group in the ring's LDS");
+        static_assert(!CHAIN || kGroup * 8u <= kRing, "two words per position of a group in the ring's LDS");
         uint32_t *hist = ring32;
         uint32_t *link = ring32 + kGroup;
         const uint32_t nGroups = (histEnd + kGroup - 1u) / kGroup;
@@ -1007,17 +1027,17 @@
         }
         constexpr uint32_t kChase = 32u / kEL;
         const uint32_t chaseFrom = hsh.flags ? histEnd - histEnd / hsh.item : 0u;
-        for (uint32_t p0 = chaseFrom + tid; p0 < histEnd && !QZ_ABLATED(512u); p0 += kChase * (uint32_t)kThreads) {
+        for (uint32_t p0 = chaseFrom + tid; p0 < histEnd && !QZ_ABLATED(512u); p0 += kChase * (uint32_t)kThr) {
             uint32_t e[kEL][kChase];
 #pragma unroll
-            for (uint32_t i = 0; i < kChase; i++) { const uint32_t pp = p0 + i * (uint32_t)kThreads; e[0][i] = pp < histEnd ? p1B[pp] : 0u; }
+            for (uint32_t i = 0; i < kChase; i++) { const uint32_t pp = p0 + i * (uint32_t)kThr; e[0][i] = pp < histEnd ? p1B[pp] : 0u; }
 #pragma unroll
             for (uint32_t d = 1; d < kEL; d++)
 #pragma unroll
                 for (uint32_t i = 0; i < kChase; i++) e[d][i] = e[d - 1u][i] ? p1B[(e[d - 1u][i] >> kTagBits) - 1u] : 0u;
 #pragma unroll
             for (uint32_t i = 0; i < kChase; i++) {
-                const uint32_t pp = p0 + i * (uint32_t)kThreads;
+                const uint32_t pp = p0 + i * (uint32_t)kThr;
                 if (pp < histEnd) {
                     if (hsh.flags) {
                         u64 *w = reinterpret_cast<u64 *>(chainB + (size_t)pp * kEQ);
@@ -1049,8 +1069,8 @@
             if (rdfirst(turnCtr[2]) == 0u) return QZSTD_HIP_NSEQ_ERROR;
         }
         __syncthreads();
-        for (uint32_t i = tid; i < kTile; i += kThreads) nearTab[i] = 0xFFFFFFFFu;
-        for (uint32_t i = tid; i < kLagT * kWin * kSrecWords + kLagT * kPvStride + QZSTD_HIP_LDS_CTRL / 4u; i += kThreads) srec[i] = 0u;
+        for (uint32_t i = tid; i < kTile; i += kThr) nearTab[i] = 0xFFFFFFFFu;
+        for (uint32_t i = tid; i < kLagT * kWin * kSrecWords + kLagT * kPvStride + QZSTD_HIP_LDS_CTRL / 4u; i += kThr) srec[i] = 0u;
     }
     {
         const uint32_t hiMaskH = pf.hashBytes >= 8 ? 0xFFFFFFFFu : ((1u << (8u * (pf.hashBytes - 4u))) - 1u);
@@ -1059,7 +1079,7 @@
             const uint32_t o2 = fo + 2u * kStep;
             if (o2 < hi) { fa2 = g128[o2 >> 4]; if (o2 < hashEnd) fb2 = g128[(o2 >> 4) + 1u]; }
             if (fo >= lo) {
-                const uint32_t r = ring_dw(fo) << 2;
+                const uint32_t r = ring_dw<S::kRing>(fo) << 2;
                 ring128[r >> 4] = fa0;
                 if (r < kMirror) ring128[(kRing + r) >> 4] = fa0;
             }
@@ -1085,7 +1105,7 @@
         }
         if (itBegin != 0u && TURNS && !CHAIN && tid == 0u) *turnCtr = itBegin * (uint32_t)kMatchWaves;
         if (itBegin == 0u)
-            for (uint32_t o = hi + tid * 16u; o < kTile + kLook; o += kThreads * 16u) {
+            for (uint32_t o = hi + tid * 16u; o < kTile + kLook; o += kThr * 16u) {
                 ring128[o >> 4] = make_uint4(0u, 0u, 0u, 0u);
                 if (o < kMirror) ring128[(kRing + o) >> 4] = make_uint4(0u, 0u, 0u, 0u);
             }
@@ -1176,7 +1196,7 @@
     uint32_t offH[kLagT], lenH[kLagT];
 #pragma unroll
     for (uint32_t i = 0; i < kLagT; i++) offH[i] = lenH[i] = 0u;
-    uint32_t rp = ring_dw((itBegin << kTileLog) + tid) << 2 | (tid & 3u);
+    uint32_t rp = ring_dw<S::kRing>((itBegin << kTileLog) + tid) << 2 | (tid & 3u);
 #ifdef QZ_DEBUG_DUMP
     u64 dI1 = 0, dW1 = 0, dI2 = 0, dW2 = 0, tP = __builtin_amdgcn_s_memtime();
     u64 dC[6] = { 0, 0, 0, 0, 0, 0 }, tC = 0;
@@ -1240,7 +1260,7 @@
         if (refill) fresh = g128[fpos >> 4];
         if (!DEFER && it >= kLagT + firstTile && !QZ_ABLATED(8u))
             emit_window<REP>(pf, src, srec + ((it % kLagT) * kWin + wave) * kSrecWords, pv + (it % kLagT) * kPvStride + 64u * wave,
-                             offH[kLagT - 1u], lenH[kLagT - 1u], t0 - kLagT * kTile + 64u * wave, ring_back(rp, kLagT * kTile), lane, out, blk.seqCap,
+                             offH[kLagT - 1u], lenH[kLagT - 1u], t0 - kLagT * kTile + 64u * wave, ring_back<S::kRing>(rp, kLagT * kTile), lane, out, blk.seqCap,
                              REP ? srec[(it % kLagT) * kWin * kSrecWords] : 0u, blk.mark);
         QZ_PRIO(1);
         uint32_t slot = 0, nslot = 0, slotL = 0, oldL = 0, tagL = 0;
@@ -1280,7 +1300,7 @@
         if (CHAIN && DEFER && wave == 0u && it + 1u < nTiles)
             chain_insert_tile(pf, src, tbl, ((it + 1u) & 1u) ? P1odd : nearTab, (it + 1u) << kTileLog, n, nh, lane, args.orderedLds != 0u);
         if (refill) {
-            const uint32_t o = ring_dw(fpos) << 2;
+            const uint32_t o = ring_dw<S::kRing>(fpos) << 2;
             ring128[o >> 4] = fresh;
             if (o < kMirror) ring128[(kRing + o) >> 4] = fresh;
         }
@@ -1351,7 +1371,7 @@
                             far[g] = p - q[g] > src.nearLimit;
                             m[g] = l != 0u && walked + (uint32_t)(kk + g) < pf.chainDepth && (l & kTagMask) == tag && (pf.window == 0u || p - q[g] <= pf.window) &&
                                    !QZ_ABLATED(2u) && !(QZ_ABLATED(64u) && far[g]);
-                            rq[g] = ring_back(rp, p - q[g]);
+                            rq[g] = ring_back<S::kRing>(rp, p - q[g]);
                         }
                         bool any = false;
 #pragma unroll
@@ -1362,9 +1382,9 @@
                             for (int g = 0; g < kG; g++) {
                                 m[g] = m[g] && cl < cap;
                                 v[g] = 0u;
-                                if (m[g]) v[g] = rd32_r(src, q[g] + cl - 3u, ring_fwd(rq[g], cl - 3u), far[g]);
+                                if (m[g]) v[g] = rd32_r(src, q[g] + cl - 3u, ring_fwd<S::kRing>(rq[g], cl - 3u), far[g]);
                             }
-                            const uint32_t pw = rd32_r(src, p + cl - 3u, ring_fwd(rp, cl - 3u), false);
+                            const uint32_t pw = rd32_r(src, p + cl - 3u, ring_fwd<S::kRing>(rp, cl - 3u), false);
 #pragma unroll
                             for (int g = 0; g < kG; g++) m[g] = m[g] && v[g] == pw;
                         }
@@ -1380,7 +1400,7 @@
                         for (int g = 0; g < kG; g++) {
                             if (m[g] && cl < cap) {
                                 uint32_t l = head_cmp(oa, Q[g], q[g] & 3u);
-                                if (l == 16u && cap > 16u) l += chunk_len(src, p + 16u, ring_fwd(rp, 16u), p - q[g], far[g]);
+                                if (l == 16u && cap > 16u) l += chunk_len(src, p + 16u, ring_fwd<S::kRing>(rp, 16u), p - q[g], far[g]);
                                 l = umin(l, cap);
                                 const int gn = (int)(4u * l) - (int)(31u - (uint32_t)__builtin_clz(p - q[g] + 1u));
                                 if (l >= 4u && (cl == 0u || gn > bg)) { cl = l; off = p - q[g]; bg = gn; }
@@ -1431,34 +1451,34 @@
             if (QZ_ABLATED(64u) && q1 != kNone && p - q1 > src.nearLimit) q1 = kNone;
             uint32_t l1 = 0, l2 = 0, l3 = 0;
             const bool far1 = q1 != kNone && p - q1 > src.nearLimit;
-            if (q1 != kNone) l1 = head_len(src, oa, q1, ring_back(rp, p - q1), far1);
+            if (q1 != kNone) l1 = head_len(src, oa, q1, ring_back<S::kRing>(rp, p - q1), far1);
             uint32_t q3 = kNone;
             if (HAS_LONG && validL && oldL != 0u && (oldL & kTagMask) == tagL && !QZ_ABLATED(2u)) q3 = (oldL >> kTagBits) - 1u;
             const bool far3 = q3 != kNone && p - q3 > src.nearLimit;
-            if (q3 != kNone) l3 = head_len(src, oa, q3, ring_back(rp, p - q3), far3);
+            if (q3 != kNone) l3 = head_len(src, oa, q3, ring_back<S::kRing>(rp, p - q3), far3);
             if (pf.nearTab && (en >> stampShift) == (stamp >> stampShift) && (en & kTagMask) == tag) {
                 const uint32_t q = t0 + ((en >> kTagBits) & (kTile - 1u));
                 if (q < p && !QZ_ABLATED(2u | 256u)) q2 = q;
             }
-            if (q2 != kNone) l2 = head_len(src, oa, q2, ring_back(rp, p - q2), false);
+            if (q2 != kNone) l2 = head_len(src, oa, q2, ring_back<S::kRing>(rp, p - q2), false);
             bool need1 = l1 == 16u && cap > 16u, need2 = l2 == 16u && cap > 16u, need3 = HAS_LONG && l3 == 16u && cap > 16u;
             if (QZ_ABLATED(128u)) need1 = need2 = need3 = false;
             QZ_PRIO(1);
             if (need1 || need2 || need3) {
-                const uint32_t rp16 = ring_fwd(rp, 16u);
+                const uint32_t rp16 = ring_fwd<S::kRing>(rp, 16u);
                 uint32_t P[9], pa[8];
                 load_dw_r<9>(src, p + 16u, rp16, false, P);
 #pragma unroll
                 for (int i = 0; i < 8; i++) pa[i] = __builtin_amdgcn_alignbyte(P[i + 1], P[i], p & 3u);
-                if (need1) { const uint32_t l = tail_len(src, pa, q1 + 16u, ring_back(rp16, p - q1), far1); l1 = 16u + l; need1 = l == 32u && 48u < cap; }
-                if (HAS_LONG && need3) { const uint32_t l = tail_len(src, pa, q3 + 16u, ring_back(rp16, p - q3), far3); l3 = 16u + l; need3 = l == 32u && 48u < cap; }
-                if (need2) { const uint32_t l = tail_len(src, pa, q2 + 16u, ring_back(rp16, p - q2), false); l2 = 16u + l; need2 = l == 32u && 48u < cap; }
+                if (need1) { const uint32_t l = tail_len(src, pa, q1 + 16u, ring_back<S::kRing>(rp16, p - q1), far1); l1 = 16u + l; need1 = l == 32u && 48u < cap; }
+                if (HAS_LONG && need3) { const uint32_t l = tail_len(src, pa, q3 + 16u, ring_back<S::kRing>(rp16, p - q3), far3); l3 = 16u + l; need3 = l == 32u && 48u < cap; }
+                if (need2) { const uint32_t l = tail_len(src, pa, q2 + 16u, ring_back<S::kRing>(rp16, p - q2), false); l2 = 16u + l; need2 = l == 32u && 48u < cap; }
             }
             while (need1 || need2 || need3) {
                 const int which = need1 ? 1 : (need3 ? 3 : 2);
                 const uint32_t q = which == 1 ? q1 : (which == 3 ? q3 : q2);
                 const uint32_t L = which == 1 ? l1 : (which == 3 ? l3 : l2);
-                const uint32_t l = chunk_len(src, p + L, ring_fwd(rp, L), p - q, which == 1 ? far1 : (which == 3 ? far3 : false));
+                const uint32_t l = chunk_len(src, p + L, ring_fwd<S::kRing>(rp, L), p - q, which == 1 ? far1 : (which == 3 ? far3 : false));
                 const bool more = l == 32u && L + 32u < cap;
                 if (which == 1) { l1 = L + l; need1 = more; }
                 else if (which == 3) { l3 = L + l; need3 = more; }
@@ -1477,7 +1497,7 @@
         for (uint32_t i = kLagT - 1u; i > 0u; i--) { offH[i] = offH[i - 1u]; lenH[i] = lenH[i - 1u]; }
         offH[0] = off;
         lenH[0] = cl;
-        rp = ring_fwd(rp, kTile);
+        rp = ring_fwd<S::kRing>(rp, kTile);
         QZ_LAP(dI2)
         if (DEFER && !CHAIN) QZ_BARRIER_LDS(); else __syncthreads();
         QZ_LAP(dW2)
@@ -1497,7 +1517,7 @@
         constexpr uint32_t kSegLog = 12u, kSeg = 1u << kSegLog, kMaxSegs = QZSTD_HIP_BLOCK_MAX >> kSegLog;
         static_assert(kMaxSegs <= 64u, "one lane per segment in the prefix step");
         constexpr uint32_t kNoAnchor = 0xFFFFFFFFu;
-        uint32_t *segCnt = srec, *segEndA = srec + kMaxSegs;
+        uint32_t *segCnt = SMALL ? nearTab : srec, *segEndA = segCnt + kMaxSegs;
         const uint32_t firstSeg = blk.parseFrom >> kSegLog, nSegs = (nh + kSeg - 1u) >> kSegLog;
 #ifdef QZ_DEBUG_DUMP
         const u64 tD0 = __builtin_amdgcn_s_memtime();
@@ -1706,11 +1726,11 @@
     return 0u;
 }
 
-template <bool HAS_LONG, bool REP, bool CHAIN, bool TURNS, bool NEAR>
-__global__ __launch_bounds__(kThreads) QZ_OCCUPANCY void qzstd_find_sequences_kernel(LaunchArgs args)
+template <bool HAS_LONG, bool REP, bool CHAIN, bool TURNS, bool NEAR, bool SMALL = false>
+__global__ __launch_bounds__(SMALL ? kSmallThreads : kThreads) __attribute__((amdgpu_waves_per_eu(SMALL ? 6 : QZ_WAVES_PER_EU))) void qzstd_find_sequences_kernel(LaunchArgs args)
 {
     const qzstd_hip_block_t blk = args.blocks[blockIdx.x];
-    const uint32_t count = qz_item<HAS_LONG, REP, CHAIN, TURNS, NEAR, true>(args, blk, args.src + blk.srcOff, args.seqs + blk.seqOff,
+    const uint32_t count = qz_item<HAS_LONG, REP, CHAIN, TURNS, NEAR, true, SMALL>(args, blk, args.src + blk.srcOff, args.seqs + blk.seqOff,
                                                               CHAIN ? args.chain + (size_t)blockIdx.x * args.chainStride : nullptr,
                                                               reinterpret_cast<uint32_t *>(args.chain + (size_t)blockIdx.x * args.chainStride + args.chainEntries),
                                                               HistShare{ nullptr, 0u, 0u, 0u, 0u, nullptr, nullptr, nullptr });
@@ -2066,7 +2086,9 @@
     X(true, false, false, false, last), X(true, true, false, false, last)
 #define QZ_K(L, R, C, T, N) reinterpret_cast<const void *>(qzstd_find_sequences_kernel<L, R, C, T, N>)
 #define QZ_W(L, R, C, T, M) reinterpret_cast<const void *>(qzstd_service_worker<L, R, C, T, M>)
-const void *const kLaunchKernels[16] = { QZ_SEARCHES(QZ_K, false), QZ_SEARCHES(QZ_K, true) };
+const void *const kLaunchKernels[18] = { QZ_SEARCHES(QZ_K, false), QZ_SEARCHES(QZ_K, true),
+                                         reinterpret_cast<const void *>(qzstd_find_sequences_kernel<false, false, false, false, false, true>),
+                                         reinterpret_cast<const void *>(qzstd_find_sequences_kernel<false, false, false, true, false, true>) };
 const void *const kWorkers[8] = { QZ_SEARCHES(QZ_W, false) };
 #undef QZ_K
 #undef QZ_W
@@ -2077,6 +2099,14 @@
     const int search = p.chainDepth ? 2 : (p.longSize ? 3 : (p.subTileLog ? 1 : 0));
     return (nearK ? 8 : 0) + 2 * search + (p.repWin ? 1 : 0);
 }
+
+int launch_variant_index(const qzstd_hip_profile_t &p, uint32_t maxBlockLen)
+{
+    const bool nearK = maxBlockLen <= QZ_RING;
+    if (!nearK && !p.chainDepth && !p.longSize && !p.repWin) return 16 + (p.subTileLog ? 1 : 0);
+    return variant_index(p, nearK);
+}
+int launch_threads(int launchVariant) { return launchVariant >= 16 ? kSmallThreads : kThreads; }
 
 }
 
@@ -2136,7 +2166,7 @@
         a.prof.lazy > 4 || (a.prof.subTileLog != 0u && a.prof.subTileLog != 6u) || (a.prof.segLog != 0u && (a.prof.segLog < kTileLog || a.prof.segLog > 17u)) ||
         (a.prof.chainDepth && (a.prof.subTileLog != 6u || a.prof.longSize || a.prof.nearTab)) || (a.prof.longSize && a.prof.subTileLog))
         return fail_msg("qzstd_hip_find_sequences: unsupported profile");
-    const size_t lds = qzstd_hip_lds_bytes(level, maxBlockLen);
+    const size_t lds = qzstd_hip_launch_lds_bytes(level, maxBlockLen, 0);
     if (lds == 0) return fail_msg("qzstd_hip_find_sequences: LDS budget exceeded");
     QZ_SET_DEVICE(device);
     bool big = lds + qzstd_hip_lds_bytes(1, QZSTD_HIP_BLOCK_MAX) > kLdsPerCu;
@@ -2197,8 +2227,9 @@
 #else
     const size_t ldsLaunch = lds;
 #endif
-    const dim3 grid(nBlocks), wg(kThreads);
-    const void *kernel = kLaunchKernels[variant_index(a.prof, maxBlockLen <= kRing)];
+    const int variant = launch_variant_index(a.prof, maxBlockLen);
+    const void *kernel = kLaunchKernels[variant];
+    const dim3 grid(nBlocks), wg(launch_threads(variant));
     void *kargs[1] = { &a };
     if (!a.prof.chainDepth && ((a.prof.tableSize & (a.prof.tableSize - 1u)) != 0u || (a.prof.longSize & (a.prof.longSize - 1u)) != 0u || a.prof.hashBytes > 7u))
         return fail_msg("qzstd_hip_find_sequences: unsupported profile (tables below the chain levels are powers of two, hashBytes <= 7)");
@@ -2231,6 +2262,27 @@
     int n = 0;
     QZ_CHECK(hipOccupancyMaxActiveBlocksPerMultiprocessor(&n, k, kThreads, lds), "hipOccupancyMaxActiveBlocksPerMultiprocessor");
     return n;
+}
+
+int qzstd_hip_launch_residency(int device, int level, uint32_t maxBlockLen, unsigned long out[4])
+{
+    qzstd_hip_profile_t p;
+    if (!out || qzstd_hip_profile_for_level(level, maxBlockLen, &p)) return fail_msg("qzstd_hip_launch_residency: bad level");
+    const size_t lds = qzstd_hip_launch_lds_bytes(level, maxBlockLen, 0);
+    if (lds == 0) return fail_msg("qzstd_hip_launch_residency: LDS budget exceeded");
+    QZ_SET_DEVICE(device);
+    const int variant = launch_variant_index(p, maxBlockLen);
+    const void *k = kLaunchKernels[variant];
+    (void)hipFuncSetAttribute(k, hipFuncAttributeMaxDynamicSharedMemorySize, (int)lds);
+    int n = 0;
+    hipFuncAttributes fa;
+    QZ_CHECK(hipOccupancyMaxActiveBlocksPerMultiprocessor(&n, k, launch_threads(variant), lds), "hipOccupancyMaxActiveBlocksPerMultiprocessor");
+    QZ_CHECK(hipFuncGetAttributes(&fa, k), "hipFuncGetAttributes");
+    out[0] = (unsigned long)n;
+    out[1] = (unsigned long)fa.numRegs;
+    out[2] = (unsigned long)fa.localSizeBytes;
+    out[3] = (unsigned long)lds;
+    return 0;
 }
 
 }
diff --git a/qat-zstd-plugin_amd/csrc/qzstd_profile.c b/qat-zstd-plugin_amd/csrc/qzstd_profile.c
--- a/qat-zstd-plugin_amd/csrc/qzstd_profile.c
+++ b/qat-zstd-plugin_amd/csrc/qzstd_profile.c
@@ -1,4 +1,6 @@
 #include "qzstd_hip.h"
+
+size_t qzstd_hip_launch_lds_bytes(int level, uint32_t maxBlockLen, int flags);
 
 #include <string.h>
 
@@ -59,19 +61,31 @@
     return (size_t)nBlocks * (((size_t)maxBlockLen + 511u) & ~(size_t)511u) * (4u * QZSTD_HIP_CHAIN_ENTRY_LINKS + 4u);
 }
 
+static size_t lds_need(const qzstd_hip_profile_t *p, size_t ring, int parseLds)
+{
+    const size_t lag = 2u;
+    const size_t need = ring + QZSTD_HIP_RING_MIRROR
+           + 4u * p->tableSize
+           + 4u * p->longSize
+           + (4u << p->tileLog)
+           + (parseLds ? lag * ((4u << p->tileLog) + 32u) : 0u)
+           + (parseLds ? lag * ((1u << p->tileLog) >> 6) * 32u : 0u)
+           + (p->chainDepth ? (4u << p->tileLog) : 0u)
+           + QZSTD_HIP_LDS_BASE + QZSTD_HIP_LDS_CTRL + QZSTD_HIP_LDS_SVC;
+    return need <= QZSTD_HIP_LDS_MAX ? need : 0;
+}
+
 size_t qzstd_hip_lds_bytes(int level, uint32_t maxBlockLen)
 {
     qzstd_hip_profile_t p;
-    size_t need;
-    const size_t lag = 2u;
     if (maxBlockLen > QZSTD_HIP_BLOCK_MAX || qzstd_hip_profile_for_level(level, maxBlockLen, &p)) return 0;
-    need = (size_t)QZ_RING + QZSTD_HIP_RING_MIRROR
-           + 4u * p.tableSize
-           + 4u * p.longSize
-           + (4u << p.tileLog)
-           + lag * ((4u << p.tileLog) + 32u)
-           + lag * ((1u << p.tileLog) >> 6) * 32u
-           + (p.chainDepth ? (4u << p.tileLog) : 0u)
-           + QZSTD_HIP_LDS_BASE + QZSTD_HIP_LDS_CTRL + QZSTD_HIP_LDS_SVC;
-    return need <= QZSTD_HIP_LDS_MAX ? need : 0;
+    return lds_need(&p, QZ_RING, 1);
 }
+
+size_t qzstd_hip_launch_lds_bytes(int level, uint32_t maxBlockLen, int flags)
+{
+    qzstd_hip_profile_t p;
+    if (maxBlockLen > QZSTD_HIP_BLOCK_MAX || qzstd_hip_profile_for_level(level | flags, maxBlockLen, &p)) return 0;
+    if (!p.chainDepth && !p.longSize && !p.repWin && maxBlockLen > QZ_RING) return lds_need(&p, QZ_RING_SMALL, 0);
+    return lds_need(&p, QZ_RING, 1);
+}
```
